# Liozou/CrystalEnergyGrids.jl

Hardware: AMD Instinct MI355X
Metric: grid-points/sec (higher is better)
Workload: dtype f64; 1 GPU; CHA_1.4_3b4eeb96 tiled 2x2x3 (11664 atoms) x 256^3 grid, Ar probe LJ + real-space Ewald; grid_points=16777216, framework_atoms=11664, lattice_images=37460, mode=fused, algo=culled, parallelism=x-slab sharding over 1 GPU(s)

## Files before the change

### crystalenergygrids.jl_amd/ceg_hip/_abi.py

```python
from __future__ import annotations

import ctypes as C
import os
import sys
from pathlib import Path

import numpy as np

RULE_DTYPE = np.dtype([('kind', '<i4'), ('_pad', '<i4'), ('p', '<f8', (3,)), ('shift', '<f8')],
                      align=True)
assert RULE_DTYPE.itemsize == 40

PKG_DIR = Path(__file__).resolve().parent.parent
REPO_DIR = PKG_DIR.parent
LIB_PATH = PKG_DIR / "csrc" / "libceg_hip.so"

class GridHeader(C.Structure):
    _fields_ = [("spacing", C.c_double), ("dims", C.c_int32 * 3), ("has_mat", C.c_int32),
                ("size", C.c_double * 3), ("shift", C.c_double * 3), ("delta", C.c_double * 3), ("unitcell", C.c_double * 3),
                ("num_unitcell", C.c_int32 * 3), ("_pad", C.c_int32), ("ewald_precision", C.c_double), ("mat", C.c_double * 9)]


class SweepParams(C.Structure):
    _fields_ = [("seed", C.c_uint64), ("first_step", C.c_uint64), ("stream_id", C.c_void_p), ("temperature", C.c_void_p),
                ("dmax", C.c_void_p), ("thetamax", C.c_void_p), ("p_rotation", C.c_void_p), ("bead", C.c_void_p)]


SWEEP_STATS_DTYPE = np.dtype([('translation_trials', '<i8'), ('translation_accepted', '<i8'), ('rotation_trials', '<i8'),
                              ('rotation_accepted', '<i8'), ('blocked', '<i8'), ('delta', '<f8')], align=True)
SWEEP_RECORD_DTYPE = np.dtype([('molecule', '<i4'), ('kind', '<i4'), ('accepted', '<i4'), ('_pad', '<i4'), ('u', '<f8'),
                               ('rows', '<f8', (2, 4)), ('positions', '<f8', (16, 3))], align=True)
assert SWEEP_STATS_DTYPE.itemsize == 48 and SWEEP_RECORD_DTYPE.itemsize == 472

GCMC_MAX_SPECIES = 8


class GcmcParams(C.Structure):
    _fields_ = [("seed", C.c_uint64), ("first_step", C.c_uint64), ("stream_id", C.c_void_p), ("temperature", C.c_void_p),
                ("dmax", C.c_void_p), ("thetamax", C.c_void_p), ("nspecies", C.c_int32), ("_pad", C.c_int32), ("species", C.c_void_p),
                ("molecule_species", C.c_void_p), ("max_molecules", C.c_void_p), ("molecule_species_out", C.c_void_p)]


GCMC_SPECIES_DTYPE = np.dtype([('m', '<i4'), ('bead', '<i4'), ('kinds', '<i4', (16,)), ('model', '<f8', (16, 3)), ('cumulative', '<f8', (5,)),
                               ('phiPV_div_k', '<f8'), ('self_reciprocal', '<f8'), ('tail_framework', '<f8'),
                               ('tail_cross', '<f8', (GCMC_MAX_SPECIES,))], align=True)
GCMC_STATS_DTYPE = np.dtype([('trials', '<i8', (7,)), ('accepted', '<i8', (7,)), ('blocked', '<i8'), ('capacity', '<i8'), ('spent', '<i8'),
                             ('delta_moves', '<f8'), ('delta_swaps', '<f8'), ('count', '<i4', (GCMC_MAX_SPECIES,)), ('nmol', '<i4'),
                             ('_pad', '<i4')], align=True)
GCMC_RECORD_DTYPE = np.dtype([('species', '<i4'), ('molecule', '<i4'), ('kind', '<i4'), ('accepted', '<i4'), ('n_species', '<i4'),
                              ('flags', '<i4'), ('u', '<f8'), ('tc', '<f8'), ('rows', '<f8', (2, 4)), ('positions', '<f8', (16, 3))], align=True)
assert (C.sizeof(GcmcParams), GCMC_SPECIES_DTYPE.itemsize, GCMC_STATS_DTYPE.itemsize, GCMC_RECORD_DTYPE.itemsize) == (88, 584, 192, 488)

c_double_p = C.POINTER(C.c_double)
c_float_p = C.POINTER(C.c_float)
c_int32_p = C.POINTER(C.c_int32)
c_int64_p = C.POINTER(C.c_int64)

PROTOTYPES = {
    "ceg_abi_version": (C.c_int, []),
    "ceg_device_count": (C.c_int, []),
    "ceg_last_error": (C.c_char_p, []),
    "ceg_grid_vdw": (C.c_int, [
        c_double_p, c_int64_p, C.c_int64, c_double_p, c_double_p,
        C.c_int32, C.c_double, C.c_double,
        C.c_void_p, c_int32_p, C.c_int32,
        c_int32_p, c_double_p, c_double_p, c_double_p,
        C.c_double, C.c_double, c_float_p, C.c_int32]),
    "ceg_grid_coulomb": (C.c_int, [
        c_double_p, c_double_p, C.c_int64, c_double_p, c_double_p,
        C.c_int32, C.c_double, C.c_double, C.c_double,
        c_int32_p, c_double_p, c_double_p, c_double_p,
        C.c_double, C.c_double, c_float_p, C.c_int32]),
    "ceg_grid_vdw_device": (C.c_int, [
        c_double_p, c_int64_p, C.c_int64, c_double_p, c_double_p,
        C.c_int32, C.c_double, C.c_double,
        C.c_void_p, c_int32_p, C.c_int32,
        c_int32_p, c_double_p, c_double_p, c_double_p,
        C.c_double, C.c_double, C.c_void_p, C.c_int32, C.c_int32]),
    "ceg_grid_coulomb_device": (C.c_int, [
        c_double_p, c_double_p, C.c_int64, c_double_p, c_double_p,
        C.c_int32, C.c_double, C.c_double, C.c_double,
        c_int32_p, c_double_p, c_double_p, c_double_p,
        C.c_double, C.c_double, C.c_void_p, C.c_int32, C.c_int32]),
    "ceg_grid_vdw_file": (C.c_int, [
        c_double_p, c_int64_p, C.c_int64, c_double_p, c_double_p,
        C.c_int32, C.c_double, C.c_double,
        C.c_void_p, c_int32_p, C.c_int32,
        c_int32_p, c_double_p, c_double_p, c_double_p,
        C.c_double, C.c_double, c_float_p, C.c_int32,
        C.c_char_p, C.c_char_p, C.c_int64, C.c_char_p, C.c_int64]),
    "ceg_grid_coulomb_file": (C.c_int, [
        c_double_p, c_double_p, C.c_int64, c_double_p, c_double_p,
        C.c_int32, C.c_double, C.c_double, C.c_double,
        c_int32_p, c_double_p, c_double_p, c_double_p,
        C.c_double, C.c_double, c_float_p, C.c_int32,
        C.c_char_p, C.c_char_p, C.c_int64, C.c_char_p, C.c_int64]),
    "ceg_release_cached_buffers": (C.c_int, []),
    "ceg_host_grid_alloc": (c_float_p, [c_int32_p]),
    "ceg_host_grid_free": (C.c_int, [c_float_p]),
    "ceg_plan_create": (C.c_int, [
        C.POINTER(C.c_void_p), C.c_int32,
        c_double_p, c_int64_p, c_double_p, C.c_int64,
        c_double_p, c_double_p, C.c_int32, C.c_double, C.c_double,
        C.c_void_p, c_int32_p, C.c_int32, C.c_double,
        c_int32_p, c_double_p, c_double_p, c_double_p]),
    "ceg_plan_destroy": (C.c_int, [C.c_void_p]),
    "ceg_image_cache_stats": (C.c_int, [c_int64_p, c_int64_p, c_int64_p]),
    "ceg_plan_can_cull": (C.c_int, [C.c_void_p]),
    "ceg_plan_num_images": (C.c_int64, [C.c_void_p]),
    "ceg_plan_copy_images": (C.c_int, [C.c_void_p, c_double_p, c_int32_p, c_int32_p, c_int32_p, c_int32_p]),
    "ceg_plan_build_vdw": (C.c_int, [
        C.c_void_p, C.c_double, C.c_double, C.c_int32, C.c_int32,
        C.c_void_p, C.c_int64, C.c_int32, C.c_int32, C.c_void_p]),
    "ceg_plan_build_coulomb": (C.c_int, [
        C.c_void_p, C.c_double, C.c_double, C.c_int32, C.c_int32,
        C.c_void_p, C.c_int64, C.c_int32, C.c_int32, C.c_void_p]),
    "ceg_plan_build_fused": (C.c_int, [
        C.c_void_p, C.c_double, C.c_double, C.c_double, C.c_double,
        C.c_int32, C.c_int32, C.c_void_p, C.c_void_p, C.c_int64, C.c_int32,
        C.c_int32, C.c_void_p]),
    "ceg_plan_create_multi": (C.c_int, [
        C.POINTER(C.c_void_p), C.c_int32,
        c_double_p, c_int64_p, c_double_p, C.c_int64,
        c_double_p, c_double_p, C.c_int32, C.c_double, C.c_double,
        C.c_int32, C.POINTER(C.c_void_p), C.POINTER(C.c_void_p), C.c_int32, C.c_double,
        c_int32_p, c_double_p, c_double_p, c_double_p]),
    "ceg_plan_num_probes": (C.c_int, [C.c_void_p]),
    "ceg_grids_multi": (C.c_int, [
        c_double_p, c_int64_p, c_double_p, C.c_int64, c_double_p, c_double_p, C.c_int32, C.c_double, C.c_double,
        C.c_int32, C.POINTER(C.c_void_p), C.POINTER(C.c_void_p), C.c_int32, C.c_double,
        c_int32_p, c_double_p, c_double_p, c_double_p,
        C.c_double, C.c_double, C.c_double, C.c_double, C.POINTER(C.c_void_p), c_float_p, C.c_int32]),
    "ceg_plan_build_multi": (C.c_int, [
        C.c_void_p, C.c_double, C.c_double, C.c_double, C.c_double,
        C.c_int32, C.c_int32, C.POINTER(C.c_void_p), C.c_void_p, C.c_int64, C.c_int32, C.c_void_p]),
    "ceg_plan_eval_points": (C.c_int, [
        C.c_void_p, C.c_int32, C.c_int32, c_double_p, C.c_int64, c_double_p]),
    "ceg_interp_create": (C.c_int, [
        C.POINTER(C.c_void_p), C.c_int32, C.c_void_p, C.c_int32,
        c_int32_p, c_double_p, c_double_p, c_double_p, c_double_p, C.c_int32]),
    "ceg_interp_create_from_file": (C.c_int, [C.POINTER(C.c_void_p), C.c_int32, C.c_char_p, C.c_int32, C.c_double, c_double_p, c_double_p, C.c_void_p]),
    "ceg_interp_set_higherorder": (C.c_int, [C.c_void_p, C.c_int32]),
    "ceg_interp_destroy": (C.c_int, [C.c_void_p]),
    "ceg_interp_points": (C.c_int, [C.c_void_p, c_double_p, C.c_int64, c_double_p]),
    "ceg_interp_points_device": (C.c_int, [C.c_void_p, C.c_void_p, C.c_int64, C.c_void_p, C.c_void_p]),
    "ceg_scale_grid_device": (C.c_int, [C.c_void_p, C.c_int64, C.c_double, C.c_int32, C.c_void_p]),
    "ceg_recip_create": (C.c_int, [
        C.POINTER(C.c_void_p), C.c_int32, c_int32_p, c_double_p, c_double_p, c_double_p, C.c_int64,
        c_int32_p, c_double_p]),
    "ceg_recip_destroy": (C.c_int, [C.c_void_p]),
    "ceg_recip_layout": (C.c_int, [c_int32_p, C.c_int64, c_int32_p, c_int32_p, c_int32_p, C.c_void_p, C.c_void_p]),
    "ceg_recip_energy": (C.c_int, [C.c_void_p, c_double_p, c_double_p, C.c_int32, C.c_int64, C.c_double, C.c_double, c_double_p]),
    "ceg_block_from_grid": (C.c_int, [C.c_int32, C.c_void_p, C.c_int32, c_int32_p, C.c_double, C.c_void_p]),
    "ceg_block_spheres": (C.c_int, [C.c_int32, c_int32_p, c_double_p, c_double_p, c_double_p, c_double_p, C.c_int32, C.c_double,
                                    c_double_p, c_double_p, C.c_int32, C.c_void_p]),
    "ceg_recip_set_structure_factor": (C.c_int, [C.c_void_p, c_double_p, c_double_p]),
    "ceg_pairs_create": (C.c_int, [C.POINTER(C.c_void_p), C.c_int32, c_double_p, c_double_p, C.c_double, C.c_void_p, c_int32_p,
                                   C.c_int32, C.c_double]),
    "ceg_pairs_destroy": (C.c_int, [C.c_void_p]),
    "ceg_pairs_set_atoms": (C.c_int, [C.c_void_p, c_double_p, c_int32_p, c_int32_p, C.c_int64]),
    "ceg_pairs_energy": (C.c_int, [C.c_void_p, c_double_p, c_int32_p, C.c_int32, C.c_int64, C.c_int32, c_double_p]),
    "ceg_pairs_energy_device": (C.c_int, [C.c_void_p, C.c_void_p, c_int32_p, C.c_int32, C.c_int64, C.c_int32, C.c_void_p, C.c_void_p]),
    "ceg_pairs_neighbour_cells": (C.c_int, [C.c_void_p, c_int32_p]),
    "ceg_mc_create": (C.c_int, [C.POINTER(C.c_void_p), C.c_int32, C.POINTER(C.c_void_p), C.c_void_p, c_double_p, C.c_int32, c_double_p,
                                c_double_p, C.c_double, C.c_void_p, c_int32_p, C.c_double, c_int32_p, c_double_p, c_double_p, c_double_p,
                                C.c_int64, c_int32_p, c_double_p]),
    "ceg_mc_destroy": (C.c_int, [C.c_void_p]),
    "ceg_mc_set_guests": (C.c_int, [C.c_void_p, c_double_p, c_int32_p, c_int32_p, C.c_int32]),
    "ceg_mc_trial": (C.c_int, [C.c_void_p, C.c_int32, c_double_p, C.c_int64, c_double_p]),
    "ceg_mc_trial_device": (C.c_int, [C.c_void_p, C.c_int32, C.c_void_p, C.c_int64, C.c_void_p, C.c_void_p]),
    "ceg_mc_trial_insert_device": (C.c_int, [C.c_void_p, c_int32_p, C.c_int32, C.c_void_p, C.c_int64, C.c_void_p, C.c_void_p]),
    "ceg_mc_accept": (C.c_int, [C.c_void_p, C.c_int32, c_double_p]),
    "ceg_mc_get_state": (C.c_int, [C.c_void_p, c_double_p, c_double_p, c_double_p]),
    "ceg_mc_neighbour_cells": (C.c_int, [C.c_void_p, c_int32_p, c_int32_p]),
    "ceg_mc_trial_insert": (C.c_int, [C.c_void_p, c_int32_p, C.c_int32, c_double_p, C.c_int64, c_double_p]),
    "ceg_mc_insert": (C.c_int, [C.c_void_p, c_int32_p, C.c_int32, c_double_p, c_int32_p]),
    "ceg_mc_remove": (C.c_int, [C.c_void_p, C.c_int32, c_int32_p]),
    "ceg_mc_group_create": (C.c_int, [C.POINTER(C.c_void_p), C.POINTER(C.c_void_p), C.c_int32]),
    "ceg_mc_group_destroy": (C.c_int, [C.c_void_p]),
    "ceg_mc_group_trial": (C.c_int, [C.c_void_p, c_int32_p, c_int32_p, c_int32_p, C.c_int32, c_double_p, c_double_p]),
    "ceg_mc_group_accept": (C.c_int, [C.c_void_p, c_int32_p, c_double_p]),
    "ceg_mc_group_sweep": (C.c_int, [C.c_void_p, C.c_void_p, C.c_int64, C.c_void_p, C.c_void_p]),
    "ceg_mc_group_sweep_gcmc": (C.c_int, [C.c_void_p, C.c_void_p, C.c_int64, C.c_void_p, C.c_void_p]),
    "ceg_energy_grid": (C.c_int, [C.POINTER(C.c_void_p), C.c_void_p, C.c_void_p, c_double_p, c_double_p, C.c_int32,
                                  c_double_p, C.c_int32, c_double_p, c_int32_p,
                                  C.c_void_p, c_int32_p, c_double_p, c_double_p, c_double_p, c_double_p,
                                  C.c_double, C.c_double, C.c_void_p, C.c_int32, C.c_void_p]),
    "ceg_energy_grid_reduced": (C.c_int, [C.POINTER(C.c_void_p), C.c_void_p, C.c_void_p, c_double_p, c_double_p, C.c_int32,
                                          c_double_p, C.c_int32, c_double_p, c_int32_p,
                                          C.c_void_p, c_int32_p, c_double_p, c_double_p, c_double_p, c_double_p,
                                          C.c_double, C.c_double, c_double_p, C.c_int32, c_double_p,
                                          C.c_void_p, C.c_void_p, C.c_void_p, C.c_int32, C.c_void_p]),
    "ceg_recip_energy_device": (C.c_int, [C.c_void_p, C.c_void_p, c_double_p, C.c_int32, C.c_int64, C.c_double, C.c_double,
                                          C.c_void_p, C.c_void_p]),
}

ALGO_AUTO, ALGO_BRUTEFORCE, ALGO_CULLED = 0, 1, 2
EGRID_MAX_TEMPS = 8


class CegError(RuntimeError):

    def __init__(self, code: int, msg: str):
        super().__init__(f"libceg_hip error {code}: {msg}")
        self.code = code


_lib = None


def load_library(path: os.PathLike | None = None) -> C.CDLL:
    global _lib
    if _lib is not None and path is None:
        return _lib
    p = Path(path) if path is not None else Path(os.environ.get("CEG_HIP_LIB", LIB_PATH))
    if not p.exists():
        raise ImportError(
            f"{p} is missing: build it with `python -c 'import __graft_entry__ as g; g.build()'` "
            "(hipcc --offload-arch=gfx950).  There is no CPU fallback for the grid build.")
    if "torch" not in sys.modules and not os.environ.get("CEG_HIP_NO_TORCH"):
        try:
            import torch
        except ImportError:
            pass
    lib = C.CDLL(str(p))
    for name, (restype, argtypes) in PROTOTYPES.items():
        fn = getattr(lib, name)
        fn.restype = restype
        fn.argtypes = argtypes
    if lib.ceg_abi_version() != 1:
        raise ImportError("libceg_hip.so ABI version mismatch")
    if path is None:
        _lib = lib
    return lib


def check(lib: C.CDLL, code: int) -> None:
    if code != 0:
        raise CegError(code, (lib.ceg_last_error() or b"").decode())


def dptr(a: np.ndarray):
    assert a.dtype == np.float64 and a.flags.c_contiguous
    return a.ctypes.data_as(c_double_p)


def i32ptr(a: np.ndarray):
    assert a.dtype == np.int32 and a.flags.c_contiguous
    return a.ctypes.data_as(c_int32_p)


def i64ptr(a: np.ndarray):
    assert a.dtype == np.int64 and a.flags.c_contiguous
    return a.ctypes.data_as(c_int64_p)


def fptr(a: np.ndarray):
    assert a.dtype == np.float32
    return a.ctypes.data_as(c_float_p)
```

### crystalenergygrids.jl_amd/ceg_hip/plan.py

```python
from __future__ import annotations

import ctypes as C
from typing import Optional

import numpy as np

from . import _abi
from .hostmirror.coordinates import GridCoordinatesSetup
from .grids import _grid_args, _matT, coulomb_scaling, vdw_scaling
from .hostmirror.probes import ProbeSystem


class _PlainBuilds:

    def build_vdw(self, d_out: int, channel_stride: int, i_begin: int, i_end: int, i_origin: int = 0,
                  algo: int = _abi.ALGO_AUTO, stream: int = 0) -> None:
        lam, thr = vdw_scaling()
        _abi.check(self._lib, self._lib.ceg_plan_build_vdw(self._h, lam, thr, i_begin, i_end, d_out, channel_stride,
                                                           i_origin, algo, stream))

    def build_coulomb(self, d_out: int, channel_stride: int, i_begin: int, i_end: int, i_origin: int = 0,
                      algo: int = _abi.ALGO_AUTO, stream: int = 0) -> None:
        lam, thr = coulomb_scaling()
        _abi.check(self._lib, self._lib.ceg_plan_build_coulomb(self._h, lam, thr, i_begin, i_end, d_out,
                                                               channel_stride, i_origin, algo, stream))

    def build_fused(self, d_vdw: int, d_coulomb: int, channel_stride: int, i_begin: int, i_end: int,
                    i_origin: int = 0, algo: int = _abi.ALGO_AUTO, stream: int = 0) -> None:
        lv, tv = vdw_scaling()
        lc, tc = coulomb_scaling()
        _abi.check(self._lib, self._lib.ceg_plan_build_fused(self._h, lv, tv, lc, tc, i_begin, i_end, d_vdw,
                                                             d_coulomb, channel_stride, i_origin, algo, stream))

    def eval_points(self, which: str, points, algo: int = _abi.ALGO_AUTO) -> np.ndarray:
        pts = np.ascontiguousarray(points, dtype=np.float64).reshape(-1, 3)
        out = np.empty((len(pts), 8), dtype=np.float64)
        w = {"vdw": 0, "coulomb": 1}[which]
        _abi.check(self._lib, self._lib.ceg_plan_eval_points(self._h, w, algo, _abi.dptr(pts), len(pts), _abi.dptr(out)))
        return out


class GridPlan(_PlainBuilds):
    def __init__(self, cset: GridCoordinatesSetup, vdw: Optional[ProbeSystem] = None,
                 coulomb: Optional[ProbeSystem] = None, alpha: float = 0.0, device: int = 0):
        if vdw is None and coulomb is None:
            raise ValueError("GridPlan needs a VdW probe and/or a Coulomb probe")
        ref = vdw if vdw is not None else coulomb
        if vdw is not None and coulomb is not None:
            if vdw.positions.shape != coulomb.positions.shape or not np.array_equal(vdw.positions, coulomb.positions):
                raise ValueError("VdW and Coulomb probes must share the same framework")
        self._lib = _abi.load_library()
        self.cset = cset
        self.device = device
        self.has_vdw = vdw is not None
        self.has_coulomb = coulomb is not None
        pos = np.ascontiguousarray(ref.positions, dtype=np.float64)
        mat, invmat = _matT(ref.mat), _matT(ref.invmat)
        ortho, safemin2 = ref.periodic_setup()
        dims, size, shift, delta = _grid_args(cset)
        kinds_p = rules_p = offs_p = None
        nkinds = 0
        keep = [pos, mat, invmat, dims, size, shift, delta]
        if vdw is not None:
            ff = vdw.forcefield
            ff.check_vdw_grid(vdw.probe, np.unique(vdw.atomkinds))
            rules, offsets = ff.rule_table(vdw.probe)
            kinds = np.ascontiguousarray(vdw.atomkinds, dtype=np.int64)
            kinds_p, rules_p, offs_p, nkinds = _abi.i64ptr(kinds), rules.ctypes.data, _abi.i32ptr(offsets), ff.nkinds
            keep += [rules, offsets, kinds]
        q_p = None
        if coulomb is not None:
            q = np.ascontiguousarray(coulomb.charges, dtype=np.float64)
            q_p = _abi.dptr(q)
            keep.append(q)
        handle = C.c_void_p()
        rc = self._lib.ceg_plan_create(C.byref(handle), device, _abi.dptr(pos), kinds_p, q_p, len(pos),
                                       _abi.dptr(mat), _abi.dptr(invmat), int(ortho), safemin2, ref.cutoff2,
                                       rules_p, offs_p, nkinds, float(alpha),
                                       _abi.i32ptr(dims), _abi.dptr(size), _abi.dptr(shift), _abi.dptr(delta))
        _abi.check(self._lib, rc)
        self._h = handle
        self.npoints = cset.npoints
        self.plane = self.npoints[1] * self.npoints[2]

    @property
    def can_cull(self) -> bool:
        return bool(self._lib.ceg_plan_can_cull(self._h))

    @property
    def num_images(self) -> int:
        return int(self._lib.ceg_plan_num_images(self._h))

    def close(self) -> None:
        if getattr(self, "_h", None):
            self._lib.ceg_plan_destroy(self._h)
            self._h = None

    def __del__(self):
        try:
            self.close()
        except Exception:
            pass


class MultiGridPlan(_PlainBuilds):
    MAX_PROBES = 4

    def __init__(self, cset: GridCoordinatesSetup, probes, coulomb: Optional[ProbeSystem] = None, alpha: float = 0.0,
                 device: int = 0):
        probes = list(probes)
        if not 1 <= len(probes) <= self.MAX_PROBES:
            raise ValueError(f"1..{self.MAX_PROBES} probes per multi-probe plan")
        ref = probes[0]
        for other in probes[1:] + ([coulomb] if coulomb is not None else []):
            if other.positions.shape != ref.positions.shape or not np.array_equal(other.positions, ref.positions):
                raise ValueError("all probes of a multi-probe plan must share the same framework")
        for other in probes[1:]:
            if not np.array_equal(other.atomkinds, ref.atomkinds) or other.cutoff2 != ref.cutoff2:
                raise ValueError("all probes of a multi-probe plan must share atom kinds and cutoff")
        self._lib = _abi.load_library()
        self.cset, self.device = cset, device
        self.nprobes = len(probes)
        self.has_coulomb = coulomb is not None
        pos = np.ascontiguousarray(ref.positions, dtype=np.float64)
        mat, invmat = _matT(ref.mat), _matT(ref.invmat)
        ortho, safemin2 = ref.periodic_setup()
        dims, size, shift, delta = _grid_args(cset)
        kinds = np.ascontiguousarray(ref.atomkinds, dtype=np.int64)
        tables = []
        for pr in probes:
            pr.forcefield.check_vdw_grid(pr.probe, np.unique(pr.atomkinds))
            tables.append(pr.forcefield.rule_table(pr.probe))
        rules_pp = (C.c_void_p * self.nprobes)(*[t[0].ctypes.data for t in tables])
        offs_pp = (C.c_void_p * self.nprobes)(*[t[1].ctypes.data for t in tables])
        q = np.ascontiguousarray(coulomb.charges, dtype=np.float64) if coulomb is not None else None
        handle = C.c_void_p()
        rc = self._lib.ceg_plan_create_multi(C.byref(handle), device, _abi.dptr(pos), _abi.i64ptr(kinds), _abi.dptr(q) if q is not None else None,
                                             len(pos), _abi.dptr(mat), _abi.dptr(invmat), int(ortho), safemin2, ref.cutoff2,
                                             self.nprobes, rules_pp, offs_pp, ref.forcefield.nkinds, float(alpha),
                                             _abi.i32ptr(dims), _abi.dptr(size), _abi.dptr(shift), _abi.dptr(delta))
        _abi.check(self._lib, rc)
        self._h = handle
        self.npoints = cset.npoints
        self.plane = self.npoints[1] * self.npoints[2]

    @property
    def num_images(self) -> int:
        return int(self._lib.ceg_plan_num_images(self._h))

    def close(self) -> None:
        if getattr(self, "_h", None):
            self._lib.ceg_plan_destroy(self._h)
            self._h = None

    def __del__(self):
        try:
            self.close()
        except Exception:
            pass

    def build(self, d_vdw, d_coulomb: int, channel_stride: int, i_begin: int, i_end: int, i_origin: int = 0, stream: int = 0) -> None:
        d_vdw = list(d_vdw) + [0] * (self.nprobes - len(d_vdw))
        ptrs = (C.c_void_p * self.nprobes)(*[int(x) if x else None for x in d_vdw])
        lv, tv = vdw_scaling()
        lc, tc = coulomb_scaling()
        _abi.check(self._lib, self._lib.ceg_plan_build_multi(self._h, lv, tv, lc, tc, i_begin, i_end, ptrs, int(d_coulomb) if d_coulomb else None,
                                                             channel_stride, i_origin, stream))
```

### crystalenergygrids.jl_amd/csrc/ceg_api.hip

```cpp
#include "ceg_internal.h"
#include "ceg_host.h"

#include <algorithm>
#include <atomic>
#include <chrono>
#include <cmath>
#include <cstdarg>
#include <cstdio>
#include <cstring>
#include <limits>
#include <map>
#include <memory>
#include <mutex>
#include <unordered_map>
#include <string>
#include <vector>

using namespace ceg;
using ceg_host::check_common;
using ceg_host::DeviceGuard;
using ceg_host::fail;

static thread_local std::string g_err = "";

int ceg_host::fail(int code, const char* fmt, ...)
{
    char buf[512];
    va_list ap;
    va_start(ap, fmt);
    vsnprintf(buf, sizeof buf, fmt, ap);
    va_end(ap);
    g_err = buf;
    return code;
}

extern "C" void ceg_set_last_error_(const char* msg) { g_err = msg ? msg : ""; }

extern "C" int ceg_abi_version(void) { return CEG_ABI_VERSION; }

extern "C" const char* ceg_last_error(void) { return g_err.c_str(); }

extern "C" int ceg_device_count(void)
{
    int n = 0;
    if (hipGetDeviceCount(&n) != hipSuccess) {
        (void)hipGetLastError();
        return 0;
    }
    return n;
}

struct ceg_plan {
    int device = 0;
    Geom g{};
    int64_t natoms = 0;
    bool has_rules = false, has_charge = false;
    bool can_cull = false;
    std::vector<double> h_pos, h_charge;
    std::vector<int32_t> h_kind;
    std::vector<DevRule> h_rules;
    std::vector<int32_t> h_offset;
    std::vector<int32_t> h_offset_union;
    int32_t nkinds = 0;
    double4* d_atoms = nullptr;
    int32_t* d_kind = nullptr;
    DevRule* d_rules = nullptr;
    int32_t* d_offset = nullptr;
    double4* d_images = nullptr;
    int32_t* d_imgkind = nullptr;
    int32_t* d_imgatom = nullptr;
    int32_t* d_binstart = nullptr;
    std::shared_ptr<void> images;
    ImageBins ib{};
    bool images_built = false;
    bool images_from_cache = false;
    PlanConst* d_pc = nullptr;
    double* d_erfcx = nullptr;
    double* d_exp2 = nullptr;
    int vdwk = 0;
    bool single_buck = false;
    double bk[4] = {0, 0, 0, 0};
    double* d_bk2 = nullptr;
    double r_exact2 = CEG_R_EXACT2;
    std::vector<FastVdw> h_fast;
    FastVdw* d_fast = nullptr;
    bool fast_ewald = false;
    bool ew2 = false;
    double* d_ew2 = nullptr;
    struct ProbeTab {
        std::vector<DevRule> rules;
        std::vector<int32_t> offset;
        std::vector<FastVdw> fast;
        DevRule* d_rules = nullptr;
        int32_t* d_offset = nullptr;
        FastVdw* d_fast = nullptr;
        PlanConst* d_pc = nullptr;
        int vdwk = 0;
        bool single_buck = false;
        double bk[4] = {0, 0, 0, 0};
        double* d_bk2 = nullptr;
        int32_t* d_imgkind = nullptr;
    };
    int nprobes = 0;
    std::vector<ProbeTab> probes;
};

namespace {

inline void matvec(const double* m, const double v[3], double o[3])
{
    for (int i = 0; i < 3; ++i) o[i] = m[i] * v[0] + m[i + 3] * v[1] + m[i + 6] * v[2];
}

void perpendicular_widths(const double* m, double w[3])
{
    const double* a = m;
    const double* b = m + 3;
    const double* c = m + 6;
    auto cross = [](const double* u, const double* v, double* o) {
        o[0] = u[1] * v[2] - u[2] * v[1];
        o[1] = u[2] * v[0] - u[0] * v[2];
        o[2] = u[0] * v[1] - u[1] * v[0];
    };
    auto norm = [](const double* u) { return std::sqrt(u[0] * u[0] + u[1] * u[1] + u[2] * u[2]); };
    double axb[3], bxc[3], cxa[3];
    cross(a, b, axb);
    cross(b, c, bxc);
    cross(c, a, cxa);
    const double vol = std::fabs(a[0] * bxc[0] + a[1] * bxc[1] + a[2] * bxc[2]);
    w[0] = vol / norm(bxc);
    w[1] = vol / norm(cxa);
    w[2] = vol / norm(axb);
}

int convert_rules(ceg_plan* p, const ceg_rule_t* rules, const int32_t* rule_offset, int32_t nkinds)
{
    std::vector<char> present(nkinds, 0);
    for (int64_t a = 0; a < p->natoms; ++a) present[p->h_kind[a]] = 1;
    p->h_offset.assign(nkinds + 1, 0);
    p->h_rules.clear();
    for (int32_t k = 0; k < nkinds; ++k) {
        p->h_offset[k] = (int32_t)p->h_rules.size();
        for (int32_t t = rule_offset[k]; t < rule_offset[k + 1]; ++t) {
            const ceg_rule_t& r = rules[t];
            DevRule d{};
            d.kind = r.kind;
            d.shift = r.shift;
            switch (r.kind) {
            case CEG_NOINTERACTION:
            case CEG_COULOMB_EWALD_DIRECT:
                continue;
            case CEG_LENNARDJONES:
                d.p0 = r.p[0];
                d.p1 = r.p[1] * r.p[1];
                break;
            case CEG_BUCKINGHAM:
                d.p0 = r.p[0];
                d.p1 = r.p[1];
                d.p2 = r.p[2];
                break;
            case CEG_HARDSPHERE: {
                const double rr = r.p[0] + r.p[1];
                d.p0 = rr * rr;
                break;
            }
            default:
                if (present[k])
                    return fail(CEG_ERR_RULE,
                                "interaction kind %d (force-field index %d) is not valid in a VdW grid "
                                "(src/interactions.jl:442-467)", r.kind, k + 1);
                continue;
            }
            p->h_rules.push_back(d);
        }
    }
    p->h_offset[nkinds] = (int32_t)p->h_rules.size();
    p->nkinds = nkinds;
    p->h_fast.assign(nkinds, FastVdw{});
    bool all_lj = true, all_fast = true;
    double hs_max2 = 0.0;
    for (int32_t k = 0; k < nkinds; ++k) {
        const int32_t b = p->h_offset[k], e = p->h_offset[k + 1];
        FastVdw f{};
        int nlj = 0, nbuck = 0, nhs = 0, nother = 0;
        for (int32_t t = b; t < e; ++t) {
            const DevRule& r = p->h_rules[t];
            if (r.kind == CEG_LENNARDJONES) { ++nlj; f.p0 = 4.0 * r.p0; f.p1 = r.p1; f.p2 = r.p1 * r.p1 * r.p1; f.shift += r.shift; }
            else if (r.kind == CEG_BUCKINGHAM) { ++nbuck; f.p0 = r.p0; f.p1 = r.p1; f.p2 = r.p2; f.shift += r.shift; }
            else if (r.kind == CEG_HARDSPHERE) { ++nhs; f.shift += r.shift; if (present[k]) hs_max2 = std::max(hs_max2, r.p0); }
            else ++nother;
        }
        if (e == b) f.cls = 0;
        else if (nlj == 1 && nbuck == 0 && nhs == 0 && nother == 0) f.cls = 1;
        else if (nbuck == 1 && nlj == 0 && nother == 0) f.cls = 2;
        else f.cls = 3;
        p->h_fast[k] = f;
        if (!present[k]) continue;
        if (f.cls > 1) all_lj = false;
        if (f.cls > 2) all_fast = false;
    }
    p->vdwk = all_lj ? 1 : (all_fast ? 2 : 0);
    if (p->vdwk == 2) {
        bool first = true, same = true;
        for (int32_t k = 0; k < nkinds && same; ++k) {
            const FastVdw& f = p->h_fast[k];
            if (!present[k] || f.cls == 0) continue;
            if (f.cls != 2) { same = false; break; }
            if (first) { p->bk[0] = f.p0; p->bk[1] = f.p1; p->bk[2] = f.p2; p->bk[3] = f.shift; first = false; }
            else same = f.p0 == p->bk[0] && f.p1 == p->bk[1] && f.p2 == p->bk[2] && f.shift == p->bk[3];
        }
        p->single_buck = same && !first && p->bk[1] > 0.0 && p->bk[2] != 0.0 && std::isfinite(1.0 / p->bk[2]);
    }
    p->r_exact2 = std::max(CEG_R_EXACT2, hs_max2 * (1.0 + 1e-9) + 1e-9);
    if (p->r_exact2 >= p->g.cutoff2) p->vdwk = 0, p->r_exact2 = CEG_R_EXACT2;
    return CEG_OK;
}

struct BlockCache {
    std::mutex m;
    std::map<std::pair<int, size_t>, std::vector<void*>> idle;
    std::unordered_map<void*, std::pair<int, size_t>> owner;
    size_t idle_bytes = 0;
};
BlockCache g_blocks;
constexpr size_t BLOCK_CACHE_LIMIT = 256ull << 20;

hipError_t cached_malloc(void** out, size_t bytes)
{
    int dev = 0;
    if (hipError_t e = hipGetDevice(&dev); e != hipSuccess) return e;
    size_t cls = 512;
    while (cls < bytes) cls <<= 1;
    std::lock_guard<std::mutex> lock(g_blocks.m);
    auto& list = g_blocks.idle[{dev, cls}];
    if (!list.empty()) {
        *out = list.back();
        list.pop_back();
        g_blocks.idle_bytes -= cls;
        return hipSuccess;
    }
    if (hipError_t e = hipMalloc(out, cls); e != hipSuccess) return e;
    g_blocks.owner[*out] = {dev, cls};
    return hipSuccess;
}

void cached_free(void* ptr)
{
    if (!ptr) return;
    std::lock_guard<std::mutex> lock(g_blocks.m);
    auto it = g_blocks.owner.find(ptr);
    if (it == g_blocks.owner.end()) { (void)hipFree(ptr); return; }
    const size_t cls = it->second.second;
    if (g_blocks.idle_bytes + cls > BLOCK_CACHE_LIMIT) {
        g_blocks.owner.erase(it);
        (void)hipFree(ptr);
        return;
    }
    g_blocks.idle[it->second].push_back(ptr);
    g_blocks.idle_bytes += cls;
}

void block_cache_release()
{
    std::lock_guard<std::mutex> lock(g_blocks.m);
    int prev = -1;
    (void)hipGetDevice(&prev);
    for (auto& kv : g_blocks.idle) {
        if (hipSetDevice(kv.first.first) != hipSuccess) continue;
        for (void* ptr : kv.second) {
            g_blocks.owner.erase(ptr);
            (void)hipFree(ptr);
        }
        kv.second.clear();
    }
    g_blocks.idle_bytes = 0;
    if (prev >= 0) (void)hipSetDevice(prev);
}

}

namespace ceg_host {
hipError_t pool_malloc(void** out, size_t bytes) { return cached_malloc(out, bytes); }
void pool_free(void* ptr) { cached_free(ptr); }
}

namespace ceg {
struct ImgBox {
    double mat[9], invmat[9];
    double lo[3], hi[3], bin[3];
    int32_t nb[3];
    int32_t has_rules, has_charge, vdw_only;
    int32_t nkinds;
    uint64_t hasbits[16];
};
hipError_t build_images_device(const ImgBox& B, const double4* d_atoms, const int32_t* d_kind, const int32_t* d_has, int64_t natoms,
                               double4** out_xyzq, int32_t** out_kind, int32_t** out_atom, int32_t** out_binstart, int64_t* out_n);
}

namespace {

struct UploadStaging {
    char* h = nullptr;
    size_t cap = 0, used = 0;
    bool pending = false;
};
constexpr size_t UPLOAD_STAGING_BYTES = 4u << 20, UPLOAD_STAGED_MAX = 1u << 20;
struct StagingPool {
    std::mutex m;
    std::vector<char*> idle;
};
StagingPool g_staging_pool;
thread_local UploadStaging* g_staging = nullptr;

struct StagingLease {
    UploadStaging st;
    UploadStaging* outer;
    StagingLease() : outer(g_staging)
    {
        if (!std::getenv("CEG_HIP_SYNC_UPLOADS")) {
            {
                std::lock_guard<std::mutex> lock(g_staging_pool.m);
                if (!g_staging_pool.idle.empty()) { st.h = g_staging_pool.idle.back(); g_staging_pool.idle.pop_back(); }
            }
            if (!st.h && hipHostMalloc((void**)&st.h, UPLOAD_STAGING_BYTES, hipHostMallocPortable) != hipSuccess) { st.h = nullptr; (void)hipGetLastError(); }
            if (st.h) st.cap = UPLOAD_STAGING_BYTES;
        }
        g_staging = &st;
    }
    ~StagingLease()
    {
        if (st.pending) (void)hipStreamSynchronize(nullptr);
        g_staging = outer;
        if (st.h) {
            std::lock_guard<std::mutex> lock(g_staging_pool.m);
            if (g_staging_pool.idle.size() < 8) g_staging_pool.idle.push_back(st.h);
            else (void)hipHostFree(st.h);
        }
    }
};

inline hipError_t flush_uploads()
{
    UploadStaging* st = g_staging;
    if (!st || !st->pending) return hipSuccess;
    st->pending = false;
    st->used = 0;
    return hipStreamSynchronize(nullptr);
}

template <class T>
int upload(T** dst, const T* src, size_t n)
{
    *dst = nullptr;
    if (n == 0) n = 1;
    HIP_TRY(cached_malloc((void**)dst, n * sizeof(T)));
    if (!src) return CEG_OK;
    const size_t bytes = n * sizeof(T);
    UploadStaging* st = g_staging;
    if (st && st->h && bytes <= UPLOAD_STAGED_MAX) {
        if (st->used + bytes > st->cap) HIP_TRY(flush_uploads());
        memcpy(st->h + st->used, src, bytes);
        HIP_TRY(hipMemcpyAsync(*dst, st->h + st->used, bytes, hipMemcpyHostToDevice, nullptr));
        st->used += (bytes + 255) & ~(size_t)255;
        st->pending = true;
        return CEG_OK;
    }
    HIP_TRY(hipMemcpy(*dst, src, bytes, hipMemcpyHostToDevice));
    return CEG_OK;
}

struct ImageSet {
    int device = 0;
    uint64_t key[2] = {0, 0};
    int64_t natoms = 0;
    double cutoff2 = 0.0;
    double lo[3] = {0, 0, 0}, hi[3] = {0, 0, 0};
    double4* d_images = nullptr;
    int32_t* d_imgkind = nullptr;
    int32_t* d_imgatom = nullptr;
    int32_t* d_binstart = nullptr;
    ImageBins ib{};
    size_t bytes = 0;
    ~ImageSet()
    {
        DeviceGuard guard(device);
        (void)hipDeviceSynchronize();
        for (void* ptr : {(void*)d_images, (void*)d_imgkind, (void*)d_imgatom, (void*)d_binstart}) cached_free(ptr);
    }
};
std::mutex g_image_mutex;
std::vector<std::shared_ptr<ImageSet>>& g_image_cache = *new std::vector<std::shared_ptr<ImageSet>>();
std::atomic<long> g_image_hits{0}, g_image_misses{0};

struct Hash128 {
    uint64_t a = 0x243F6A8885A308D3ull, b = 0x13198A2E03707344ull;
    void word(uint64_t w)
    {
        a = (a ^ w) * 0x9E3779B97F4A7C15ull; a ^= a >> 29;
        b = (b + w) * 0xC2B2AE3D27D4EB4Full; b ^= b >> 31; b += a;
    }
    void bytes(const void* ptr, size_t n)
    {
        const unsigned char* c = static_cast<const unsigned char*>(ptr);
        size_t i = 0;
        for (; i + 8 <= n; i += 8) { uint64_t w; memcpy(&w, c + i, 8); word(w); }
        uint64_t w = 0;
        if (i < n) memcpy(&w, c + i, n - i);
        word(w ^ ((uint64_t)n << 56));
    }
    template <class T> void pod(const T& v) { bytes(&v, sizeof v); }
};

int image_cache_capacity()
{
    if (const char* e = std::getenv("CEG_HIP_IMAGE_CACHE")) return std::max(0, atoi(e));
    return 6;
}

void image_cache_release()
{
    std::lock_guard<std::mutex> lock(g_image_mutex);
    g_image_cache.clear();
}

#ifndef CEG_BIN_Z
#define CEG_BIN_Z 1.5
#endif
int build_images(ceg_plan* p)
{
    const Geom& g = p->g;
    const double cutoff = std::sqrt(g.cutoff2);
    const double margin = cutoff * (1.0 + 1e-6) + 1e-6;
    double lo[3], hi[3];
    for (int a = 0; a < 3; ++a) {
        lo[a] = g.shift[a] - margin;
        hi[a] = g.shift[a] + g.size[a] + margin;
    }
    double target[3] = {4.5, 4.5, CEG_BIN_Z};
    if (const char* e = std::getenv("CEG_HIP_BIN_XY")) target[0] = target[1] = std::max(0.5, atof(e));
    if (const char* e = std::getenv("CEG_HIP_BIN_Z")) target[2] = std::max(0.25, atof(e));
    int nb[3];
    double bin[3];
    for (int a = 0; a < 3; ++a) {
        nb[a] = std::max(1, (int)std::floor((hi[a] - lo[a]) / target[a]));
        bin[a] = (hi[a] - lo[a]) / nb[a];
    }
    const std::vector<int32_t>& off = p->nprobes > 0 ? p->h_offset_union : p->h_offset;
    auto kind_has_rule = [&](int32_t k) { return k >= 0 && k + 1 < (int32_t)off.size() && off[k + 1] > off[k]; };
    Hash128 hk;
    std::shared_ptr<ImageSet> hit;
    const int cap = image_cache_capacity();
    if (cap > 0) {
        hk.pod(p->device); hk.pod(p->natoms);
        hk.bytes(g.mat, sizeof g.mat); hk.bytes(g.invmat, sizeof g.invmat);
        hk.bytes(lo, sizeof lo); hk.bytes(hi, sizeof hi); hk.bytes(target, sizeof target);
        hk.bytes(p->h_pos.data(), p->h_pos.size() * sizeof(double));
        const int32_t mode = (p->has_rules ? 1 : 0) | (p->has_charge ? 2 : 0);
        hk.pod(mode);
        if (p->has_charge) hk.bytes(p->h_charge.data(), p->h_charge.size() * sizeof(double));
        if (p->has_rules)
            for (int64_t a = 0; a < p->natoms; ++a) {
                const int32_t k = p->h_kind[a];
                hk.pod((int32_t)(k < 0 ? -1 : (k | (kind_has_rule(k) ? (1 << 25) : 0))));
            }
        std::lock_guard<std::mutex> lock(g_image_mutex);
        for (size_t t = 0; t < g_image_cache.size(); ++t) {
            const std::shared_ptr<ImageSet> c = g_image_cache[t];
            if (c->device == p->device && c->key[0] == hk.a && c->key[1] == hk.b && c->natoms == p->natoms && c->cutoff2 == g.cutoff2 &&
                memcmp(c->lo, lo, sizeof lo) == 0 && memcmp(c->hi, hi, sizeof hi) == 0) {
                hit = c;
                std::rotate(g_image_cache.begin() + t, g_image_cache.begin() + t + 1, g_image_cache.end());
                break;
            }
        }
    }
    if (hit) {
        g_image_hits.fetch_add(1);
        p->images = hit;
        const ImageSet& c = *hit;
        p->d_images = c.d_images; p->d_imgkind = c.d_imgkind; p->d_imgatom = c.d_imgatom; p->d_binstart = c.d_binstart;
        p->ib = c.ib;
        p->ib.kind = p->has_rules ? p->d_imgkind : nullptr;
        p->ib.atoms = p->d_atoms;
        p->images_built = true;
        p->images_from_cache = true;
        return CEG_OK;
    }
    if (cap > 0) g_image_misses.fetch_add(1);
    if (!std::getenv("CEG_HIP_IMAGES_ON_HOST")) {
        ceg::ImgBox B{};
        memcpy(B.mat, g.mat, sizeof B.mat);
        memcpy(B.invmat, g.invmat, sizeof B.invmat);
        for (int a = 0; a < 3; ++a) { B.lo[a] = lo[a]; B.hi[a] = hi[a]; B.bin[a] = bin[a]; B.nb[a] = nb[a]; }
        B.has_rules = p->has_rules ? 1 : 0;
        B.has_charge = p->has_charge ? 1 : 0;
        B.vdw_only = (p->has_rules && !p->has_charge) ? 1 : 0;
        B.nkinds = p->nkinds;
        int32_t* d_has = nullptr;
        if (p->has_rules && p->nkinds <= 1024) {
            for (int32_t k = 0; k < p->nkinds; ++k)
                if (kind_has_rule(k)) B.hasbits[k >> 6] |= 1ull << (k & 63);
        } else if (p->has_rules) {
            std::vector<int32_t> has((size_t)std::max(p->nkinds, 1), 0);
            for (int32_t k = 0; k < p->nkinds; ++k) has[k] = kind_has_rule(k) ? 1 : 0;
            if (int rc = upload(&d_has, has.data(), has.size())) return rc;
        }
        auto set = std::make_shared<ImageSet>();
        set->device = p->device;
        set->key[0] = hk.a; set->key[1] = hk.b;
        set->natoms = p->natoms; set->cutoff2 = g.cutoff2;
        memcpy(set->lo, lo, sizeof lo); memcpy(set->hi, hi, sizeof hi);
        int64_t n = 0;
        const hipError_t e = ceg::build_images_device(B, p->d_atoms, p->has_rules ? p->d_kind : nullptr, d_has, p->natoms, &set->d_images, &set->d_imgkind,
                                                      &set->d_imgatom, &set->d_binstart, &n);
        if (d_has) cached_free(d_has);
        if (e != hipSuccess) return fail(CEG_ERR_HIP, "building the lattice-image list on the device failed: %s", hipGetErrorString(e));
        set->bytes = (size_t)n * (sizeof(double4) + 2 * sizeof(int32_t)) + (size_t)(nb[0] * nb[1] * nb[2] + 1) * sizeof(int32_t);
        p->images = set;
        p->d_images = set->d_images; p->d_imgkind = set->d_imgkind; p->d_imgatom = set->d_imgatom; p->d_binstart = set->d_binstart;
        ImageBins& ib = p->ib;
        ib.xyzq = p->d_images;
        ib.kind = p->has_rules ? p->d_imgkind : nullptr;
        ib.atom = p->d_imgatom;
        ib.atoms = p->d_atoms;
        ib.bin_start = p->d_binstart;
        for (int a = 0; a < 3; ++a) {
            ib.lo[a] = lo[a];
            ib.bin[a] = bin[a];
            ib.inv_bin[a] = 1.0 / bin[a];
            ib.nb[a] = nb[a];
        }
        ib.nimages = (int32_t)n;
        p->images_built = true;
        set->ib = ib;
        if (cap > 0) {
            std::lock_guard<std::mutex> lock(g_image_mutex);
            g_image_cache.push_back(set);
            while ((int)g_image_cache.size() > cap) g_image_cache.erase(g_image_cache.begin());
        }
        return CEG_OK;
    }
    struct Img { double x, y, z, q; int32_t kind; int32_t bin; int32_t atom; };
    std::vector<Img> imgs;
    imgs.reserve((size_t)p->natoms * 8);
    const double* M = g.mat;
    const double* I = g.invmat;
    for (int64_t a = 0; a < p->natoms; ++a) {
        if (p->has_rules && !p->has_charge) {
            if (!kind_has_rule(p->h_kind[a])) continue;
        }
        const double pa[3] = {p->h_pos[3 * a], p->h_pos[3 * a + 1], p->h_pos[3 * a + 2]};
        double fmin[3] = {1e300, 1e300, 1e300}, fmax[3] = {-1e300, -1e300, -1e300};
        for (int c = 0; c < 8; ++c) {
            const double d[3] = {((c & 1) ? hi[0] : lo[0]) - pa[0], ((c & 2) ? hi[1] : lo[1]) - pa[1],
                                 ((c & 4) ? hi[2] : lo[2]) - pa[2]};
            double f[3];
            matvec(I, d, f);
            for (int q = 0; q < 3; ++q) {
                fmin[q] = std::min(fmin[q], f[q]);
                fmax[q] = std::max(fmax[q], f[q]);
            }
        }
        int n0[3], n1[3];
        for (int q = 0; q < 3; ++q) {
            n0[q] = (int)std::ceil(fmin[q] - 1e-9);
            n1[q] = (int)std::floor(fmax[q] + 1e-9);
        }
        for (int nx = n0[0]; nx <= n1[0]; ++nx)
            for (int ny = n0[1]; ny <= n1[1]; ++ny)
                for (int nz = n0[2]; nz <= n1[2]; ++nz) {
                    const double P[3] = {pa[0] + (nx * M[0] + ny * M[3] + nz * M[6]),
                                         pa[1] + (nx * M[1] + ny * M[4] + nz * M[7]),
                                         pa[2] + (nx * M[2] + ny * M[5] + nz * M[8])};
                    if (P[0] < lo[0] || P[0] > hi[0] || P[1] < lo[1] || P[1] > hi[1] || P[2] < lo[2] ||
                        P[2] > hi[2])
                        continue;
                    int b[3];
                    for (int q = 0; q < 3; ++q) {
                        b[q] = (int)std::floor((P[q] - lo[q]) / bin[q]);
                        b[q] = std::min(std::max(b[q], 0), nb[q] - 1);
                    }
                    Img im;
                    im.x = P[0]; im.y = P[1]; im.z = P[2];
                    im.q = p->has_charge ? p->h_charge[a] : 0.0;
                    im.kind = -1;
                    if (p->has_rules) {
                        const int32_t k = p->h_kind[a];
                        im.kind = k < 0 ? -1 : (k | (kind_has_rule(k) ? (1 << 25) : 0));
                    }
                    im.bin = (b[0] * nb[1] + b[1]) * nb[2] + b[2];
                    im.atom = (int32_t)a;
                    imgs.push_back(im);
                }
    }
    if (imgs.size() > 0x7ffffff0ull) return fail(CEG_ERR_UNSUPPORTED, "too many lattice images");
    const size_t nbins = (size_t)nb[0] * nb[1] * nb[2];
    std::vector<int32_t> start(nbins + 1, 0);
    for (const Img& im : imgs) start[im.bin + 1]++;
    for (size_t b = 0; b < nbins; ++b) start[b + 1] += start[b];
    std::vector<int32_t> cursor(start.begin(), start.end() - 1);
    std::vector<double4> xyzq(imgs.size());
    std::vector<int32_t> kind(imgs.size());
    std::vector<int32_t> atom(imgs.size());
    for (const Img& im : imgs) {
        const int32_t s = cursor[im.bin]++;
        xyzq[s] = make_double4(im.x, im.y, im.z, im.q);
        kind[s] = im.kind;
        atom[s] = im.atom;
    }
    auto set = std::make_shared<ImageSet>();
    set->device = p->device;
    set->key[0] = hk.a; set->key[1] = hk.b;
    set->natoms = p->natoms; set->cutoff2 = g.cutoff2;
    memcpy(set->lo, lo, sizeof lo); memcpy(set->hi, hi, sizeof hi);
    if (int rc = upload(&set->d_images, xyzq.data(), xyzq.size())) return rc;
    if (int rc = upload(&set->d_imgkind, kind.data(), kind.size())) return rc;
    if (int rc = upload(&set->d_imgatom, atom.data(), atom.size())) return rc;
    if (int rc = upload(&set->d_binstart, start.data(), start.size())) return rc;
    set->bytes = xyzq.size() * sizeof(double4) + (kind.size() + atom.size() + start.size()) * sizeof(int32_t);
    p->images = set;
    p->d_images = set->d_images; p->d_imgkind = set->d_imgkind; p->d_imgatom = set->d_imgatom; p->d_binstart = set->d_binstart;
    ImageBins& ib = p->ib;
    ib.xyzq = p->d_images;
    ib.kind = p->has_rules ? p->d_imgkind : nullptr;
    ib.atom = p->d_imgatom;
    ib.atoms = p->d_atoms;
    ib.bin_start = p->d_binstart;
    for (int a = 0; a < 3; ++a) {
        ib.lo[a] = lo[a];
        ib.bin[a] = bin[a];
        ib.inv_bin[a] = 1.0 / bin[a];
        ib.nb[a] = nb[a];
    }
    ib.nimages = (int32_t)imgs.size();
    p->images_built = true;
    set->ib = ib;
    if (cap > 0) {
        std::lock_guard<std::mutex> lock(g_image_mutex);
        g_image_cache.push_back(set);
        while ((int)g_image_cache.size() > cap) g_image_cache.erase(g_image_cache.begin());
    }
    return CEG_OK;
}

bool build_ewald_tables_uncached(double alpha, double cutoff2, std::vector<double>& tab, std::vector<double>& exp2_tab,
                                 double* inv_h_out, double* mx0_inv_h_out);

bool build_ewald_tables(double alpha, double cutoff2, std::vector<double>& tab, std::vector<double>& exp2_tab,
                        double* inv_h_out, double* mx0_inv_h_out)
{
    struct Memo { bool valid = false, ok = false; double alpha = 0, cutoff2 = 0, inv_h = 0, mx0 = 0; std::vector<double> tab, e2; };
    static std::mutex m;
    static Memo memo;
    std::lock_guard<std::mutex> lock(m);
    if (!(memo.valid && memo.alpha == alpha && memo.cutoff2 == cutoff2)) {
        memo.tab.clear(); memo.e2.clear();
        memo.ok = build_ewald_tables_uncached(alpha, cutoff2, memo.tab, memo.e2, &memo.inv_h, &memo.mx0);
        memo.alpha = alpha; memo.cutoff2 = cutoff2; memo.valid = true;
    }
    tab = memo.tab; exp2_tab = memo.e2; *inv_h_out = memo.inv_h; *mx0_inv_h_out = memo.mx0;
    return memo.ok;
}

bool build_ewald_tables_uncached(double alpha, double cutoff2, std::vector<double>& tab, std::vector<double>& exp2_tab,
                                 double* inv_h_out, double* mx0_inv_h_out)
{
    const int N = CEG_ERFCX_TAB_N;
    const long double x0 = (long double)alpha * std::sqrt((long double)CEG_R_EXACT2) * (1.0L - 1e-6L);
    const long double x1 = (long double)alpha * std::sqrt((long double)cutoff2 * (1.0L + 2e-9L)) * (1.0L + 1e-6L);
    if (!(x1 > x0) || x1 > 5.0L * (1.0L - 1e-9L)) return false;
    const long double h = (x1 - x0) / N;
    auto erfcx = [](long double x) { return expl(x * x) * erfcl(x); };
    tab.assign((size_t)N * 6, 0.0);
    const long double PI = 3.14159265358979323846264338327950288L;
    long double node[6];
    for (int k = 0; k < 6; ++k) node[k] = 0.5L + 0.5L * cosl(PI * (k + 0.5L) / 6.0L);
    double worst = 0.0;
    for (int i = 0; i < N; ++i) {
        const long double lo = x0 + i * h;
        long double V[6][7];
        for (int r = 0; r < 6; ++r) {
            long double pw = 1.0L;
            for (int c = 0; c < 6; ++c) { V[r][c] = pw; pw *= node[r]; }
            V[r][6] = erfcx(lo + node[r] * h);
        }
        for (int c = 0; c < 6; ++c) {
            int piv = c;
            for (int r = c + 1; r < 6; ++r) if (fabsl(V[r][c]) > fabsl(V[piv][c])) piv = r;
            for (int q = 0; q < 7; ++q) std::swap(V[c][q], V[piv][q]);
            const long double d = V[c][c];
            for (int q = 0; q < 7; ++q) V[c][q] /= d;
            for (int r = 0; r < 6; ++r) if (r != c) {
                const long double f = V[r][c];
                for (int q = 0; q < 7; ++q) V[r][q] -= f * V[c][q];
            }
        }
        for (int c = 0; c < 6; ++c) tab[(size_t)i * 6 + c] = (double)V[c][6];
        for (int t = 0; t <= 8; ++t) {
            const double sl = t / 8.0;
            double pv = tab[(size_t)i * 6 + 5];
            for (int c = 4; c >= 0; --c) pv = pv * sl + tab[(size_t)i * 6 + c];
            const long double ref = erfcx(lo + (long double)sl * h);
            worst = std::max(worst, (double)fabsl(((long double)pv - ref) / ref));
        }
    }
    if (!(worst < 1e-14)) return false;
    exp2_tab.resize(64);
    for (int j = 0; j < 64; ++j) exp2_tab[j] = (double)exp2l((long double)j / 64.0L);
    *inv_h_out = (double)(1.0L / h);
    *mx0_inv_h_out = (double)(-x0 / h);
    return true;
}

bool build_ew2_table_uncached(double alpha, double r_exact2, double cutoff2, std::vector<double>& tab, int32_t* base_out,
                              int32_t* ni_out, double* worst_out, int which = 0, double bkA = 0.0, double bkC = 0.0)
{
    const int SHIFT = which == 0 ? CEG_EW2_SHIFT : CEG_BK2_SHIFT, ni_max = which == 0 ? CEG_EW2_NI_MAX : CEG_BK2_NI_MAX;
    auto key_of = [SHIFT](double s) { uint64_t b; memcpy(&b, &s, 8); return (int32_t)((uint32_t)(b >> 32) >> SHIFT); };
    if (!(alpha > 0.0) || !(r_exact2 >= 1.0) || !(cutoff2 > r_exact2)) return false;
    const int32_t base = key_of(r_exact2), last = key_of(cutoff2 * (1.0 + 4e-9) + 4e-9);
    const int32_t ni = last - base + 1;
    if (ni < 1 || ni > ni_max) return false;
    const long double a = alpha, ka = 2.0L * a / sqrtl(3.14159265358979323846264338327950288L);
    auto B0 = [&](long double s) { const long double r = sqrtl(s); return which == 0 ? erfcl(a * r) / r : (long double)bkA * expl(-a * r); };
    auto Cf = [&](long double s) { return ka * expl(-a * a * s); };
    const int nf = which == 0 ? 2 : 1, stride = which == 0 ? CEG_EW2_STRIDE : CEG_BK2_STRIDE;
    const int ND = which == 0 ? 7 : CEG_BK2_ND;
    const long double PI = 3.14159265358979323846264338327950288L;
    long double node[8];
    for (int k = 0; k < ND; ++k) node[k] = cosl(PI * (k + 0.5L) / (long double)ND);
    tab.assign((size_t)ni * stride, 0.0);
    double worst = 0.0;
    for (int32_t i = 0; i < ni; ++i) {
        const uint64_t lo_bits = (uint64_t)(uint32_t)((base + i) << SHIFT) << 32;
        const uint64_t mid_bits = lo_bits | ((uint64_t)1 << (32 + SHIFT - 1));
        const uint64_t hi_bits = (uint64_t)(uint32_t)((base + i + 1) << SHIFT) << 32;
        double s_lo, s_mid, s_hi;
        memcpy(&s_lo, &lo_bits, 8); memcpy(&s_mid, &mid_bits, 8); memcpy(&s_hi, &hi_bits, 8);
        const long double hh = 0.5L * ((long double)s_hi - (long double)s_lo);
        for (int f = 0; f < nf; ++f) {
            long double V[8][9];
            for (int r = 0; r < ND; ++r) {
                long double pw = 1.0L;
                for (int c = 0; c < ND; ++c) { V[r][c] = pw; pw *= node[r]; }
                const long double s = (long double)s_mid + node[r] * hh;
                V[r][ND] = f == 0 ? B0(s) : Cf(s);
            }
            for (int c = 0; c < ND; ++c) {
                int piv = c;
                for (int r = c + 1; r < ND; ++r) if (fabsl(V[r][c]) > fabsl(V[piv][c])) piv = r;
                for (int q = 0; q <= ND; ++q) std::swap(V[c][q], V[piv][q]);
                const long double d = V[c][c];
                for (int q = 0; q <= ND; ++q) V[c][q] /= d;
                for (int r = 0; r < ND; ++r) if (r != c) {
                    const long double g = V[r][c];
                    for (int q = 0; q <= ND; ++q) V[r][q] -= g * V[c][q];
                }
            }
            long double cu[8], ct[8] = {0, 0, 0, 0, 0, 0, 0, 0};
            long double sc = 1.0L;
            for (int c = 0; c < ND; ++c) { cu[c] = V[c][ND] * sc; sc /= hh; }
            for (int c = 0; c < ND; ++c) {
                long double binom = 1.0L;
                for (int k = 0; k <= c; ++k) {
                    ct[k] += cu[c] * binom * powl(-hh, c - k);
                    binom = binom * (c - k) / (k + 1);
                }
            }
            double* co = &tab[(size_t)i * stride + ND * f];
            for (int c = 0; c < ND; ++c) co[c] = (double)ct[c];
            for (int q = 0; q <= 16; ++q) {
                const double t = (double)(((long double)q / 16.0L) * 2.0L * hh * (1.0L - 1e-12L));
                double pv = co[ND - 1];
                for (int c = ND - 2; c >= 0; --c) pv = __builtin_fma(pv, t, co[c]);
                const long double s = (long double)s_lo + (long double)t;
                const long double ref = f == 0 ? B0(s) : Cf(s);
                const long double scale = which == 0 ? fabsl(ref) : fabsl(ref) + fabsl((long double)bkC) / (s * s * s);
                worst = std::max(worst, (double)fabsl(((long double)pv - ref) / scale));
            }
        }
    }
    *base_out = base; *ni_out = ni; *worst_out = worst;
    return worst < 5e-11;
}

bool build_ew2_table(double alpha, double r_exact2, double cutoff2, std::vector<double>& tab, int32_t* base_out, int32_t* ni_out)
{
    struct Memo { bool valid = false, ok = false; double alpha = 0, r_exact2 = 0, cutoff2 = 0; int32_t base = 0, ni = 0; std::vector<double> tab; };
    static std::mutex m;
    static Memo memo;
    std::lock_guard<std::mutex> lock(m);
    if (!(memo.valid && memo.alpha == alpha && memo.r_exact2 == r_exact2 && memo.cutoff2 == cutoff2)) {
        memo.tab.clear();
        double worst = 0.0;
        memo.ok = build_ew2_table_uncached(alpha, r_exact2, cutoff2, memo.tab, &memo.base, &memo.ni, &worst);
        memo.alpha = alpha; memo.r_exact2 = r_exact2; memo.cutoff2 = cutoff2; memo.valid = true;
        if (std::getenv("CEG_HIP_TRACE"))
            fprintf(stderr, "[ceg_hip] r^2-indexed Ewald table: %d intervals, worst relative error %.2e -> %s\n", memo.ni, worst,
                    memo.ok ? "used" : "not used");
    }
    tab = memo.tab; *base_out = memo.base; *ni_out = memo.ni;
    return memo.ok;
}

bool build_bk2_table(double A, double B, double C, double r_exact2, double cutoff2, std::vector<double>& tab, int32_t* base_out, int32_t* ni_out)
{
    struct Memo { bool valid = false, ok = false; double A = 0, B = 0, C = 0, r_exact2 = 0, cutoff2 = 0; int32_t base = 0, ni = 0; std::vector<double> tab; };
    static std::mutex m;
    static Memo memo;
    std::lock_guard<std::mutex> lock(m);
    if (!(memo.valid && memo.A == A && memo.B == B && memo.C == C && memo.r_exact2 == r_exact2 && memo.cutoff2 == cutoff2)) {
        memo.tab.clear();
        double worst = 0.0;
        memo.ok = build_ew2_table_uncached(B, r_exact2, cutoff2, memo.tab, &memo.base, &memo.ni, &worst, 1, A, C) && worst < CEG_BK2_TOL;
        memo.A = A; memo.B = B; memo.C = C; memo.r_exact2 = r_exact2; memo.cutoff2 = cutoff2; memo.valid = true;
        if (std::getenv("CEG_HIP_TRACE"))
            fprintf(stderr, "[ceg_hip] r^2-indexed Buckingham table: %d intervals, worst error %.2e of the pair energy -> %s\n", memo.ni, worst,
                    memo.ok ? "used" : "not used");
    }
    tab = memo.tab; *base_out = memo.base; *ni_out = memo.ni;
    return memo.ok;
}

}

int ceg_host::check_common(const double* pos, int64_t natoms, const double* mat, const double* invmat,
                           const int32_t* dims, const double* size, const double* shift, const double* delta)
{
    if (!pos && natoms > 0) return fail(CEG_ERR_INVALID, "pos is NULL");
    if (natoms < 0) return fail(CEG_ERR_INVALID, "natoms < 0");
    if (!mat || !invmat || !dims || !size || !shift || !delta)
        return fail(CEG_ERR_INVALID, "NULL geometry argument");
    for (int a = 0; a < 3; ++a)
        if (dims[a] < 1) return fail(CEG_ERR_INVALID, "dims[%d] = %d < 1", a, dims[a]);
    return CEG_OK;
}

__global__ void k_probe_image_flags(const int32_t* __restrict__ kind_union, const int32_t* __restrict__ has, int32_t nkinds, int32_t* __restrict__ out, int64_t n)
{
    const int64_t i = (int64_t)blockIdx.x * blockDim.x + threadIdx.x;
    if (i >= n) return;
    const int32_t kw = kind_union[i];
    if (kw < 0) { out[i] = kw; return; }
    const int32_t k = kw & ((1 << 24) - 1);
    out[i] = k | ((k < nkinds && has[k]) ? (1 << 25) : 0);
}

static int probe_image_flags(const int32_t* d_union, const int32_t* d_has, int32_t nkinds, int32_t* d_out, int64_t n)
{
    if (n <= 0) return CEG_OK;
    hipLaunchKernelGGL(k_probe_image_flags, dim3((unsigned)((n + 255) / 256)), dim3(256), 0, nullptr, d_union, d_has, nkinds, d_out, n);
    return hipGetLastError() == hipSuccess ? CEG_OK : fail(CEG_ERR_HIP, "image-flag kernel launch failed");
}

static int create_impl(ceg_plan_t** plan, int32_t device,
                       const double* pos, const int64_t* atomkind, const double* charge,
                       int64_t natoms,
                       const double mat[9], const double invmat[9],
                       int32_t ortho, double safemin2, double cutoff2,
                       const ceg_rule_t* rules, const int32_t* rule_offset, int32_t nkinds,
                       int32_t nprobes, const ceg_rule_t* const* mrules, const int32_t* const* moffset,
                       double alpha,
                       const int32_t dims[3], const double size[3], const double shift[3],
                       const double delta[3])
{
    if (!plan) return fail(CEG_ERR_INVALID, "plan is NULL");
    *plan = nullptr;
    if (int rc = check_common(pos, natoms, mat, invmat, dims, size, shift, delta)) return rc;
    if (nprobes < 0 || nprobes > CEG_MAX_PROBES) return fail(CEG_ERR_INVALID, "nprobes = %d outside 1..%d", nprobes, CEG_MAX_PROBES);
    if (nprobes > 0) {
        if (!mrules || !moffset || !atomkind || nkinds <= 0) return fail(CEG_ERR_INVALID, "rule tables / atomkind missing");
        for (int q = 0; q < nprobes; ++q)
            if (!mrules[q] || !moffset[q]) return fail(CEG_ERR_INVALID, "rule table of probe %d is NULL", q);
        rules = mrules[0];
        rule_offset = moffset[0];
    }
    const bool trace = std::getenv("CEG_HIP_TRACE") != nullptr;
    const auto t0 = std::chrono::steady_clock::now();
    auto stamp = [&](const char* what) {
        if (trace)
            fprintf(stderr, "[ceg plan] %-28s %8.3f ms\n", what,
                    std::chrono::duration<double, std::milli>(std::chrono::steady_clock::now() - t0).count());
    };
    const int ndev = ceg_device_count();
    if (ndev <= 0) return fail(CEG_ERR_NO_DEVICE, "no HIP device available (this library has no CPU path)");
    if (device < 0 || device >= ndev) return fail(CEG_ERR_NO_DEVICE, "device %d not present (%d devices)", device, ndev);
    const bool has_rules = rules && rule_offset && atomkind && nkinds > 0;
    if (!has_rules && !charge) return fail(CEG_ERR_INVALID, "plan needs rules+atomkind and/or charges");

    ceg_plan* p = new ceg_plan();
    p->device = device;
    p->natoms = natoms;
    p->has_rules = has_rules;
    p->has_charge = charge != nullptr;
    Geom& g = p->g;
    memcpy(g.mat, mat, sizeof g.mat);
    memcpy(g.invmat, invmat, sizeof g.invmat);
    for (int a = 0; a < 3; ++a) {
        g.size[a] = size[a];
        g.shift[a] = shift[a];
        g.delta[a] = delta[a];
        g.dims[a] = dims[a];
    }
    g.ortho = ortho ? 1 : 0;
    g.safemin2 = safemin2;
    g.cutoff2 = cutoff2;
    g.alpha = alpha;
    g.diag = (mat[1] == 0 && mat[2] == 0 && mat[3] == 0 && mat[5] == 0 && mat[6] == 0 && mat[7] == 0) ? 1 : 0;

    p->h_pos.assign(pos, pos + 3 * natoms);
    if (charge) p->h_charge.assign(charge, charge + natoms);
    p->h_kind.assign(natoms, -1);
    if (has_rules) {
        for (int64_t a = 0; a < natoms; ++a) {
            const int64_t k = atomkind[a];
            if (k < 1 || k > nkinds) {
                delete p;
                return fail(CEG_ERR_INVALID, "atomkind[%lld] = %lld outside 1..%d", (long long)a, (long long)k, nkinds);
            }
            p->h_kind[a] = (int32_t)(k - 1);
        }
        if (int rc = convert_rules(p, rules, rule_offset, nkinds)) {
            delete p;
            return rc;
        }
        if (nprobes > 0) {
            p->nprobes = nprobes;
            p->probes.resize(nprobes);
            std::vector<int32_t> any(nkinds, 0);
            double r_exact2 = CEG_R_EXACT2;
            for (int q = 0; q < nprobes; ++q) {
                if (q > 0)
                    if (int rc = convert_rules(p, mrules[q], moffset[q], nkinds)) { delete p; return rc; }
                ceg_plan::ProbeTab& t = p->probes[q];
                t.rules = p->h_rules; t.offset = p->h_offset; t.fast = p->h_fast;
                t.vdwk = p->vdwk; t.single_buck = p->single_buck;
                for (int c = 0; c < 4; ++c) t.bk[c] = p->bk[c];
                r_exact2 = std::max(r_exact2, p->r_exact2);
                for (int32_t k = 0; k < nkinds; ++k) any[k] |= (t.offset[k + 1] > t.offset[k]) ? 1 : 0;
            }
            p->r_exact2 = r_exact2;
            if (!(r_exact2 < p->g.cutoff2)) {
                delete p;
                return fail(CEG_ERR_UNSUPPORTED, "a hard sphere of one of the probes reaches the cutoff: build that grid with a plan of its own");
            }
            p->h_rules = p->probes[0].rules; p->h_fast = p->probes[0].fast;
            p->vdwk = p->probes[0].vdwk; p->single_buck = p->probes[0].single_buck;
            for (int c = 0; c < 4; ++c) p->bk[c] = p->probes[0].bk[c];
            p->h_offset_union.assign(nkinds + 1, 0);
            for (int32_t k = 0; k < nkinds; ++k) p->h_offset_union[k + 1] = p->h_offset_union[k] + any[k];
            p->h_offset = p->probes[0].offset;
        }
    }
    double w[3];
    perpendicular_widths(g.mat, w);
    const double cutoff = std::sqrt(cutoff2);
    p->can_cull = std::isfinite(cutoff2) && cutoff2 > 0 &&
                  std::min(w[0], std::min(w[1], w[2])) >= 2.0 * cutoff * (1.0 - 1e-12);

    stamp("host: rules, geometry");
    DeviceGuard guard(device);
    if (!guard.ok) {
        delete p;
        return fail(CEG_ERR_HIP, "hipSetDevice(%d) failed", device);
    }
    StagingLease lease;
    std::vector<double4> xyzq((size_t)natoms);
    for (int64_t a = 0; a < natoms; ++a)
        xyzq[a] = make_double4(pos[3 * a], pos[3 * a + 1], pos[3 * a + 2], charge ? charge[a] : 0.0);
    int rc = upload(&p->d_atoms, xyzq.data(), xyzq.size());
    if (!rc) rc = upload(&p->d_kind, p->h_kind.data(), p->h_kind.size());
    if (!rc) rc = upload(&p->d_rules, p->h_rules.data(), p->h_rules.size());
    if (!rc) {
        if (p->h_offset.empty()) p->h_offset.assign(1, 0);
        rc = upload(&p->d_offset, p->h_offset.data(), p->h_offset.size());
    }
    stamp("atom / rule tables uploaded");
    if (!rc && p->can_cull) rc = build_images(p);
    stamp(p->images_from_cache ? "images: cache hit" : "images built + uploaded");
    if (!rc && p->can_cull) {
        PlanConst hc{};
        hc.g = p->g;
        hc.ib = p->ib;
        hc.rt = RuleTable{p->d_rules, p->d_offset, p->nkinds};
        hc.alpha2 = alpha * alpha;
        hc.r_exact2 = p->r_exact2;
        {
            const double hx = 1.5 * size[0] / dims[0], hy = 1.5 * size[1] / dims[1], hz = 1.5 * size[2] / dims[2];
            const double reach = std::sqrt(cutoff2 * (1.0 + 1e-9) + 1e-9) + std::sqrt(hx * hx + hy * hy + hz * hz);
            bool all = true;
            for (int k = 0; k < 3; ++k) {
                const double rown = std::sqrt(invmat[k] * invmat[k] + invmat[k + 3] * invmat[k + 3] + invmat[k + 6] * invmat[k + 6]);
                const double ek = std::fabs(invmat[k]) * hx + std::fabs(invmat[k + 3]) * hy + std::fabs(invmat[k + 6]) * hz + 1e-9;
                if (!(rown * reach + ek < 0.5 - 1e-6)) all = false;
            }
            hc.all_simple = all ? 1 : 0;
        }
        if (p->h_fast.empty()) p->h_fast.assign(1, FastVdw{});
        rc = upload(&p->d_fast, p->h_fast.data(), p->h_fast.size());
        hc.fastvdw = p->d_fast;
        p->fast_ewald = false;
        bool any_vdwk2 = p->vdwk == 2;
        for (const auto& t : p->probes) any_vdwk2 = any_vdwk2 || t.vdwk == 2;
        if (!rc && ((p->has_charge && std::isfinite(alpha) && alpha > 0) || any_vdwk2)) {
            std::vector<double> tab, e2;
            double inv_h = 0, mx0 = 0;
            const bool want_ewald = p->has_charge && std::isfinite(alpha) && alpha > 0;
            const bool ok = build_ewald_tables(want_ewald ? alpha : 0.25, cutoff2, tab, e2, &inv_h, &mx0);
            if (!ok && p->vdwk == 2) p->vdwk = 0;
            if (!ok)
                for (auto& t : p->probes)
                    if (t.vdwk == 2) t.vdwk = 0;
            if (ok) {
                rc = upload(&p->d_erfcx, tab.data(), tab.size());
                if (!rc) rc = upload(&p->d_exp2, e2.data(), e2.size());
                hc.erfcx_tab = p->d_erfcx;
                hc.exp2_tab = p->d_exp2;
                hc.erfcx_inv_h = inv_h;
                hc.erfcx_mx0_inv_h = mx0;
                p->fast_ewald = want_ewald;
            }
            hc.ew_k3 = 2.0 * alpha * alpha / 3.0;
            hc.ew_k15 = 4.0 * (alpha * alpha) * (alpha * alpha) / 15.0;
            if (ok && want_ewald && !rc && !std::getenv("CEG_HIP_NO_EW2")) {
                std::vector<double> t2;
                int32_t base = 0, ni = 0;
                if (build_ew2_table(alpha, p->r_exact2, cutoff2, t2, &base, &ni)) {
                    rc = upload(&p->d_ew2, t2.data(), t2.size());
                    hc.ew2_tab = p->d_ew2;
                    hc.ew2_ni = ni;
                    hc.ew2_base = base;
                    p->ew2 = !rc;
                }
            }
        }
        auto setup_bk2 = [&](int& vdwk, bool single_buck, const double bk[4], double** d_tab, PlanConst& target) {
            if (rc || vdwk != 2 || !single_buck || std::getenv("CEG_HIP_NO_BK2")) return;
            std::vector<double> tb;
            int32_t base = 0, ni = 0;
            if (!build_bk2_table(bk[0] / bk[2], bk[1], 1.0, p->r_exact2, cutoff2, tb, &base, &ni)) return;
            rc = upload(d_tab, tb.data(), tb.size());
            target.bk2_tab = *d_tab;
            target.bk2_ni = ni;
            target.bk2_base = base;
            const double B = bk[1], C = bk[2];
            target.bk_B = B; target.bk_C = C; target.bk_invC = 1.0 / C; target.bk_nshift = -bk[3] / C;
            target.bk_c1 = -B / 6.0; target.bk_c2 = -B / 48.0; target.bk_c3 = B * B / 3.0; target.bk_c4 = -B / 160.0;
            target.bk_s1 = 1.0 / (6.0 * C); target.bk_s2 = -1.0 / (48.0 * C); target.bk_s3 = 1.0 / (480.0 * C);
            if (!rc) vdwk = 3;
        };
        if (p->nprobes == 0) setup_bk2(p->vdwk, p->single_buck, p->bk, &p->d_bk2, hc);
        if (!rc && p->nprobes > 0) {
            hc.nprobes = p->nprobes;
            for (int q = 0; q < p->nprobes && !rc; ++q) {
                ceg_plan::ProbeTab& t = p->probes[q];
                rc = upload(&t.d_rules, t.rules.data(), t.rules.size());
                if (!rc) rc = upload(&t.d_offset, t.offset.data(), t.offset.size());
                if (!rc) rc = upload(&t.d_fast, t.fast.data(), t.fast.size());
                hc.rtm[q] = RuleTable{t.d_rules, t.d_offset, p->nkinds};
                hc.fastm[q] = t.d_fast;
            }
            for (int q = 0; q < p->nprobes && !rc; ++q) {
                ceg_plan::ProbeTab& t = p->probes[q];
                PlanConst hq = hc;
                hq.rt = hc.rtm[q];
                hq.fastvdw = hc.fastm[q];
                setup_bk2(t.vdwk, t.single_buck, t.bk, &t.d_bk2, hq);
                if (!rc && p->nprobes > 1) {
                    std::vector<int32_t> has((size_t)p->nkinds);
                    for (int32_t k = 0; k < p->nkinds; ++k) has[k] = t.offset[k + 1] > t.offset[k] ? 1 : 0;
                    int32_t* d_has = nullptr;
                    rc = upload(&d_has, has.data(), has.size());
                    if (!rc) {
                        void* raw = nullptr;
                        const int64_t n = p->ib.nimages;
                        if (cached_malloc(&raw, sizeof(int32_t) * (size_t)std::max<int64_t>(n, 1)) != hipSuccess) rc = fail(CEG_ERR_HIP, "hipMalloc failed");
                        else {
                            t.d_imgkind = (int32_t*)raw;
                            rc = probe_image_flags(p->d_imgkind, d_has, p->nkinds, t.d_imgkind, n);
                        }
                    }
                    if (d_has) { (void)hipDeviceSynchronize(); cached_free(d_has); }
                    hq.ib.kind = t.d_imgkind;
                }
                if (!rc) rc = upload(&t.d_pc, &hq, 1);
                if (q == 0) { p->vdwk = t.vdwk; }
            }
            hc.rt = hc.rtm[0];
            hc.fastvdw = hc.fastm[0];
        }
        if (!rc) rc = upload(&p->d_pc, &hc, 1);
    } else if (!rc && p->nprobes > 0) {
        rc = fail(CEG_ERR_UNSUPPORTED, "multi-probe plans need every perpendicular cell width >= 2*cutoff (what a ProbeSystem guarantees)");
    }
    if (flush_uploads() != hipSuccess && !rc) rc = fail(CEG_ERR_HIP, "uploading the plan's tables failed");
    stamp("function tables, constants");
    if (rc) {
        ceg_plan_destroy(p);
        return rc;
    }
    *plan = p;
    return CEG_OK;
}

extern "C" int ceg_plan_create(ceg_plan_t** plan, int32_t device,
                               const double* pos, const int64_t* atomkind, const double* charge,
                               int64_t natoms,
                               const double mat[9], const double invmat[9],
                               int32_t ortho, double safemin2, double cutoff2,
                               const ceg_rule_t* rules, const int32_t* rule_offset, int32_t nkinds,
                               double alpha,
                               const int32_t dims[3], const double size[3], const double shift[3],
                               const double delta[3])
{
    return create_impl(plan, device, pos, atomkind, charge, natoms, mat, invmat, ortho, safemin2, cutoff2, rules, rule_offset, nkinds, 0,
                       nullptr, nullptr, alpha, dims, size, shift, delta);
}

extern "C" int ceg_plan_create_multi(ceg_plan_t** plan, int32_t device, const double* pos, const int64_t* atomkind, const double* charge,
                                     int64_t natoms, const double mat[9], const double invmat[9], int32_t ortho, double safemin2,
                                     double cutoff2, int32_t nprobes, const ceg_rule_t* const* rules,
                                     const int32_t* const* rule_offset, int32_t nkinds, double alpha, const int32_t dims[3],
                                     const double size[3], const double shift[3], const double delta[3])
{
    if (nprobes < 1) return fail(CEG_ERR_INVALID, "nprobes = %d < 1", nprobes);
    return create_impl(plan, device, pos, atomkind, charge, natoms, mat, invmat, ortho, safemin2, cutoff2, nullptr, nullptr, nkinds, nprobes,
                       rules, rule_offset, alpha, dims, size, shift, delta);
}

extern "C" int ceg_plan_num_probes(const ceg_plan_t* p) { return p ? p->nprobes : 0; }

extern "C" int ceg_plan_destroy(ceg_plan_t* p)
{
    if (!p) return CEG_OK;
    DeviceGuard guard(p->device);
    (void)hipDeviceSynchronize();
    p->images.reset();
    for (void* ptr : {(void*)p->d_atoms, (void*)p->d_kind, (void*)p->d_rules, (void*)p->d_offset, (void*)p->d_pc, (void*)p->d_erfcx,
                      (void*)p->d_exp2, (void*)p->d_fast, (void*)p->d_ew2, (void*)p->d_bk2})
        cached_free(ptr);
    for (auto& t : p->probes)
        for (void* ptr : {(void*)t.d_rules, (void*)t.d_offset, (void*)t.d_fast, (void*)t.d_pc, (void*)t.d_bk2, (void*)t.d_imgkind}) cached_free(ptr);
    delete p;
    return CEG_OK;
}

extern "C" int ceg_image_cache_stats(int64_t* hits, int64_t* misses, int64_t* entries)
{
    std::lock_guard<std::mutex> lock(g_image_mutex);
    if (hits) *hits = g_image_hits.load();
    if (misses) *misses = g_image_misses.load();
    if (entries) *entries = (int64_t)g_image_cache.size();
    return CEG_OK;
}

extern "C" int ceg_plan_can_cull(const ceg_plan_t* p) { return (p && p->can_cull) ? 1 : 0; }

extern "C" int64_t ceg_plan_num_images(const ceg_plan_t* p) { return (p && p->images_built) ? p->ib.nimages : 0; }

extern "C" int ceg_plan_copy_images(const ceg_plan_t* p, double* xyzq, int32_t* kind, int32_t* atom, int32_t* bin_start, int32_t nb[3])
{
    if (!p || !p->images_built) return fail(CEG_ERR_INVALID, "the plan has no image list");
    DeviceGuard guard(p->device);
    if (!guard.ok) return fail(CEG_ERR_HIP, "hipSetDevice(%d) failed", p->device);
    const size_t n = (size_t)p->ib.nimages;
    const size_t nbins = (size_t)p->ib.nb[0] * p->ib.nb[1] * p->ib.nb[2];
    if (nb) for (int a = 0; a < 3; ++a) nb[a] = p->ib.nb[a];
    bool ok = hipDeviceSynchronize() == hipSuccess;
    if (ok && xyzq && n) ok = hipMemcpy(xyzq, p->d_images, n * sizeof(double4), hipMemcpyDeviceToHost) == hipSuccess;
    if (ok && kind && n && p->d_imgkind) ok = hipMemcpy(kind, p->d_imgkind, n * sizeof(int32_t), hipMemcpyDeviceToHost) == hipSuccess;
    if (ok && atom && n) ok = hipMemcpy(atom, p->d_imgatom, n * sizeof(int32_t), hipMemcpyDeviceToHost) == hipSuccess;
    if (ok && bin_start) ok = hipMemcpy(bin_start, p->d_binstart, (nbins + 1) * sizeof(int32_t), hipMemcpyDeviceToHost) == hipSuccess;
    return ok ? CEG_OK : fail(CEG_ERR_HIP, "copying the image list failed");
}

namespace {

int resolve_algo(const ceg_plan* p, int32_t algo, bool* culled)
{
    switch (algo) {
    case CEG_ALGO_AUTO: *culled = p->can_cull; return CEG_OK;
    case CEG_ALGO_BRUTEFORCE: *culled = false; return CEG_OK;
    case CEG_ALGO_CULLED:
        if (!p->can_cull)
            return fail(CEG_ERR_UNSUPPORTED,
                        "culled algorithm needs every perpendicular cell width >= 2*cutoff");
        *culled = true;
        return CEG_OK;
    default: return fail(CEG_ERR_INVALID, "unknown algo %d", algo);
    }
}

int run(ceg_plan* p, int mode, const Output& out, const Points& pts, bool culled, hipStream_t stream)
{
    if (mode != MODE_COULOMB && !p->has_rules) return fail(CEG_ERR_INVALID, "plan was created without rules");
    if (mode != MODE_VDW && !p->has_charge) return fail(CEG_ERR_INVALID, "plan was created without charges");
    RuleTable rt{p->d_rules, p->d_offset, p->nkinds};
    hipError_t e;
    if (culled) {
        const bool probe0 = p->nprobes > 0 && mode != MODE_COULOMB;
        e = launch_culled(mode, probe0 ? p->probes[0].d_pc : p->d_pc, p->g, probe0 ? p->probes[0].vdwk : p->vdwk,
                          p->ew2 ? 2 : (p->fast_ewald ? 1 : 0), out, pts, stream);
    } else {
        AtomTable at{p->d_atoms, p->has_rules ? p->d_kind : nullptr, p->natoms};
        e = launch_bruteforce(mode, p->g, at, rt, out, pts, stream);
    }
    if (e != hipSuccess) return fail(CEG_ERR_HIP, "kernel launch failed: %s", hipGetErrorString(e));
    return CEG_OK;
}

int build_common(ceg_plan* p, int mode, double lv, double tv, double lc, double tc, int32_t i_begin,
                 int32_t i_end, float* d_v, float* d_c, int64_t channel_stride, int32_t i_origin,
                 int32_t algo, void* stream)
{
    if (!p) return fail(CEG_ERR_INVALID, "plan is NULL");
    if (i_begin < 0 || i_end > p->g.dims[0] + 1 || i_begin > i_end)
        return fail(CEG_ERR_INVALID, "bad x-plane range [%d,%d) for dims[0]+1 = %d", i_begin, i_end, p->g.dims[0] + 1);
    if (i_origin > i_begin) return fail(CEG_ERR_INVALID, "i_origin %d > i_begin %d", i_origin, i_begin);
    if ((mode != MODE_COULOMB && !d_v) || (mode != MODE_VDW && !d_c)) return fail(CEG_ERR_INVALID, "output pointer is NULL");
    const int64_t plane = (int64_t)(p->g.dims[1] + 1) * (p->g.dims[2] + 1);
    if (channel_stride < (int64_t)(i_end - i_origin) * plane)
        return fail(CEG_ERR_INVALID, "channel_stride %lld too small", (long long)channel_stride);
    bool culled;
    if (int rc = resolve_algo(p, algo, &culled)) return rc;
    Output out{};
    out.vdw = d_v;
    out.coulomb = d_c;
    out.channel_stride = channel_stride;
    out.i_origin = i_origin;
    out.i_begin = i_begin;
    out.i_end = i_end;
    out.lambda_vdw = lv;
    out.thr_vdw = tv;
    out.lambda_coulomb = lc;
    out.thr_coulomb = tc;
    DeviceGuard guard(p->device);
    if (!guard.ok) return fail(CEG_ERR_HIP, "hipSetDevice(%d) failed", p->device);
    return run(p, mode, out, Points{nullptr, 0}, culled, (hipStream_t)stream);
}

}

extern "C" int ceg_plan_build_vdw(ceg_plan_t* plan, double lambda, double threshold, int32_t i_begin,
                                  int32_t i_end, float* d_out, int64_t channel_stride, int32_t i_origin,
                                  int32_t algo, void* stream)
{
    return build_common(plan, MODE_VDW, lambda, threshold, 0, 0, i_begin, i_end, d_out, nullptr, channel_stride,
                        i_origin, algo, stream);
}

extern "C" int ceg_plan_build_coulomb(ceg_plan_t* plan, double lambda, double threshold, int32_t i_begin,
                                      int32_t i_end, float* d_out, int64_t channel_stride, int32_t i_origin,
                                      int32_t algo, void* stream)
{
    return build_common(plan, MODE_COULOMB, 0, 0, lambda, threshold, i_begin, i_end, nullptr, d_out,
                        channel_stride, i_origin, algo, stream);
}

extern "C" int ceg_plan_build_fused(ceg_plan_t* plan, double lambda_vdw, double threshold_vdw,
                                    double lambda_coulomb, double threshold_coulomb, int32_t i_begin,
                                    int32_t i_end, float* d_out_vdw, float* d_out_coulomb,
                                    int64_t channel_stride, int32_t i_origin, int32_t algo, void* stream)
{
    return build_common(plan, MODE_FUSED, lambda_vdw, threshold_vdw, lambda_coulomb, threshold_coulomb, i_begin,
                        i_end, d_out_vdw, d_out_coulomb, channel_stride, i_origin, algo, stream);
}

extern "C" int ceg_plan_build_multi(ceg_plan_t* p, double lambda_vdw, double threshold_vdw, double lambda_coulomb, double threshold_coulomb,
                                    int32_t i_begin, int32_t i_end, float* const* d_out_vdw, float* d_out_coulomb,
                                    int64_t channel_stride, int32_t i_origin, void* stream)
{
    if (!p) return fail(CEG_ERR_INVALID, "plan is NULL");
    if (p->nprobes < 1) return fail(CEG_ERR_INVALID, "not a multi-probe plan (ceg_plan_create_multi)");
    if (i_begin < 0 || i_end > p->g.dims[0] + 1 || i_begin > i_end)
        return fail(CEG_ERR_INVALID, "bad x-plane range [%d,%d) for dims[0]+1 = %d", i_begin, i_end, p->g.dims[0] + 1);
    if (i_origin > i_begin) return fail(CEG_ERR_INVALID, "i_origin %d > i_begin %d", i_origin, i_begin);
    const int64_t plane = (int64_t)(p->g.dims[1] + 1) * (p->g.dims[2] + 1);
    if (channel_stride < (int64_t)(i_end - i_origin) * plane) return fail(CEG_ERR_INVALID, "channel_stride %lld too small", (long long)channel_stride);
    if (d_out_coulomb && !p->has_charge) return fail(CEG_ERR_INVALID, "plan was created without charges");
    std::vector<int> req;
    for (int q = 0; q < p->nprobes; ++q)
        if (d_out_vdw && d_out_vdw[q]) req.push_back(q);
    if (req.empty() && !d_out_coulomb) return CEG_OK;
    Output base{};
    base.channel_stride = channel_stride;
    base.i_origin = i_origin;
    base.i_begin = i_begin;
    base.i_end = i_end;
    base.lambda_vdw = lambda_vdw;
    base.thr_vdw = threshold_vdw;
    base.lambda_coulomb = lambda_coulomb;
    base.thr_coulomb = threshold_coulomb;
    DeviceGuard guard(p->device);
    if (!guard.ok) return fail(CEG_ERR_HIP, "hipSetDevice(%d) failed", p->device);
    hipStream_t st = (hipStream_t)stream;
    hipError_t e = hipSuccess;
    const int ewk = p->ew2 ? 2 : (p->fast_ewald ? 1 : 0);
    auto single = [&](int mode, int q) {
        Output o = base;
        o.vdw = q >= 0 ? d_out_vdw[q] : nullptr;
        o.coulomb = mode != MODE_VDW ? d_out_coulomb : nullptr;
        return launch_culled(mode, q >= 0 ? p->probes[q].d_pc : p->d_pc, p->g, q >= 0 ? p->probes[q].vdwk : 1, ewk, o, Points{nullptr, 0}, st);
    };
    auto multi = [&](int mode, const int* idx, int np) {
        Output o = base;
        for (int t = 0; t < np; ++t) { o.vdwm[t] = d_out_vdw[idx[t]]; o.probe_idx[t] = idx[t]; }
        o.coulomb = mode == MODE_FUSED ? d_out_coulomb : nullptr;
        return launch_culled_multi(mode, np, p->d_pc, p->g, o, st);
    };
    std::vector<int> lj, other;
    for (int q : req) (p->probes[q].vdwk == 1 ? lj : other).push_back(q);
    if (d_out_coulomb) {
        int fused_np = CEG_MAX_PROBES_FUSED;
        if (const char* env = std::getenv("CEG_HIP_MULTI_FUSED_NP")) fused_np = std::max(0, std::min(CEG_MAX_PROBES_FUSED, atoi(env)));
        if (!p->ew2 && p->nprobes > 1) fused_np = 0;
        if (fused_np >= 2 && lj.size() >= 2) {
            e = multi(MODE_FUSED, &lj[0], 2);
            lj.erase(lj.begin(), lj.begin() + 2);
        } else if (fused_np >= 1 && !other.empty()) {
            e = single(MODE_FUSED, other[0]);
            other.erase(other.begin());
        } else if (fused_np >= 1 && !lj.empty()) {
            e = single(MODE_FUSED, lj[0]);
            lj.erase(lj.begin());
        } else {
            e = single(MODE_COULOMB, -1);
        }
    }
    size_t at = 0;
    while (e == hipSuccess && at < lj.size()) {
        const int n = (int)std::min<size_t>(CEG_MAX_PROBES, lj.size() - at);
        e = n == 1 ? single(MODE_VDW, lj[at]) : multi(MODE_VDW, &lj[at], n);
        at += (size_t)n;
    }
    for (size_t t = 0; e == hipSuccess && t < other.size(); ++t) e = single(MODE_VDW, other[t]);
    if (e != hipSuccess) return fail(CEG_ERR_HIP, "kernel launch failed: %s", hipGetErrorString(e));
    return CEG_OK;
}

extern "C" int ceg_plan_eval_points(ceg_plan_t* p, int32_t which, int32_t algo, const double* points,
                                    int64_t npoints, double* out)
{
    if (!p) return fail(CEG_ERR_INVALID, "plan is NULL");
    if (npoints < 0 || (npoints > 0 && (!points || !out))) return fail(CEG_ERR_INVALID, "bad points/out");
    if (which != 0 && which != 1) return fail(CEG_ERR_INVALID, "which must be 0 (vdw) or 1 (coulomb)");
    if (npoints == 0) return CEG_OK;
    bool culled;
    if (int rc = resolve_algo(p, algo, &culled)) return rc;
    if (culled) {
        bool inside = true;
        for (int64_t q = 0; q < npoints && inside; ++q)
            for (int a = 0; a < 3; ++a) {
                const double x = points[3 * q + a];
                if (!(x >= p->g.shift[a] - 1e-9 && x <= p->g.shift[a] + p->g.size[a] + 1e-9)) inside = false;
            }
        if (!inside) {
            if (algo == CEG_ALGO_CULLED)
                return fail(CEG_ERR_UNSUPPORTED, "culled evaluation needs points inside the grid bounding box");
            culled = false;
        }
    }
    DeviceGuard guard(p->device);
    if (!guard.ok) return fail(CEG_ERR_HIP, "hipSetDevice(%d) failed", p->device);
    double* d_pts = nullptr;
    double* d_out = nullptr;
    HIP_TRY(hipMalloc((void**)&d_pts, sizeof(double) * 3 * npoints));
    if (hipMalloc((void**)&d_out, sizeof(double) * 8 * npoints) != hipSuccess) {
        (void)hipFree(d_pts);
        return fail(CEG_ERR_HIP, "hipMalloc failed");
    }
    int rc = CEG_OK;
    if (hipMemcpy(d_pts, points, sizeof(double) * 3 * npoints, hipMemcpyHostToDevice) != hipSuccess)
        rc = fail(CEG_ERR_HIP, "hipMemcpy H2D failed");
    if (!rc) {
        Output o{};
        if (which == 0) o.raw_vdw = d_out; else o.raw_coulomb = d_out;
        rc = run(p, which == 0 ? MODE_VDW : MODE_COULOMB, o, Points{d_pts, npoints}, culled, nullptr);
    }
    if (!rc && hipDeviceSynchronize() != hipSuccess) rc = fail(CEG_ERR_HIP, "kernel execution failed: %s", hipGetErrorString(hipGetLastError()));
    if (!rc && hipMemcpy(out, d_out, sizeof(double) * 8 * npoints, hipMemcpyDeviceToHost) != hipSuccess)
        rc = fail(CEG_ERR_HIP, "hipMemcpy D2H failed");
    (void)hipFree(d_pts);
    (void)hipFree(d_out);
    return rc;
}

extern "C" int ceg_release_cached_buffers(void)
{
    ceg_host::oneshot_pools_release();
    image_cache_release();
    block_cache_release();
    return CEG_OK;
}
```

### crystalenergygrids.jl_amd/csrc/ceg_internal.h

```cpp
#pragma once

#include <hip/hip_runtime.h>
#include <stdint.h>

#include "../../include/ceg_hip.h"

namespace ceg {

enum Mode : int { MODE_VDW = 0, MODE_COULOMB = 1, MODE_FUSED = 2 };

struct DevRule {
    int32_t kind;
    int32_t _pad;
    double  p0, p1, p2;
    double  shift;
};

struct Geom {
    double mat[9];
    double invmat[9];
    double size[3];
    double shift[3];
    double delta[3];
    int32_t dims[3];
    int32_t ortho;
    double safemin2;
    double cutoff2;
    double alpha;
    int32_t diag;
    int32_t _pad;
};


struct Output {
    float*  vdw;
    float*  coulomb;
    double* raw_vdw;
    double* raw_coulomb;
    int64_t channel_stride;
    int32_t i_origin;
    int32_t i_begin, i_end;
    double  lambda_vdw, thr_vdw;
    double  lambda_coulomb, thr_coulomb;
    float*  vdwm[CEG_MAX_PROBES];
    int32_t probe_idx[CEG_MAX_PROBES];
};

struct Points {
    const double* xyz;
    int64_t n;
};

struct AtomTable {
    const double4* xyzq;
    const int32_t* kind;
    int64_t n;
};

struct RuleTable {
    const DevRule* rules;
    const int32_t* offset;
    int32_t nkinds;
};

struct ImageBins {
    const double4* xyzq;
    const int32_t* kind;
    const int32_t* atom;
    const double4* atoms;
    const int32_t* bin_start;
    double lo[3];
    double inv_bin[3];
    double bin[3];
    int32_t nb[3];
    int32_t nimages;
};

struct FastVdw {
    double p0, p1, p2, shift;
    int32_t cls;
    int32_t _pad;
};

struct PlanConst {
    Geom g;
    ImageBins ib;
    RuleTable rt;
    const FastVdw* fastvdw;
    double r_exact2;
    const double* erfcx_tab;
    const double* exp2_tab;
    double erfcx_inv_h;
    double erfcx_mx0_inv_h;
    double alpha2;
    const double* ew2_tab;
    int32_t ew2_ni;
    int32_t ew2_base;
    double ew_k3, ew_k15;
    const double* bk2_tab;
    int32_t bk2_ni, bk2_base;
    double bk_B, bk_C, bk_invC;
    double bk_nshift, bk_c1, bk_c2, bk_c3, bk_c4;
    double bk_s1, bk_s2, bk_s3;
    int32_t all_simple;
    int32_t nprobes;
    RuleTable rtm[CEG_MAX_PROBES];
    const FastVdw* fastm[CEG_MAX_PROBES];
};

constexpr int CEG_ERFCX_TAB_N = 128;
#ifndef CEG_R_EXACT2_VALUE
#define CEG_R_EXACT2_VALUE 4.0
#endif
constexpr double CEG_R_EXACT2 = CEG_R_EXACT2_VALUE;

constexpr int CEG_EW2_LOGM = 5;
constexpr int CEG_EW2_SHIFT = 20 - CEG_EW2_LOGM;
constexpr int CEG_EW2_STRIDE = 14;
#ifndef CEG_EW2_LDS_STRIDE
#define CEG_EW2_LDS_STRIDE 14
#endif
constexpr int CEG_EW2_NI_MAX = 176;
constexpr int CEG_BK2_ND = 8;
constexpr int CEG_BK2_STRIDE = 10;
constexpr int CEG_BK2_LOGM = CEG_EW2_LOGM;
constexpr int CEG_BK2_SHIFT = 20 - CEG_BK2_LOGM;
constexpr int CEG_BK2_NI_MAX = CEG_EW2_NI_MAX;
constexpr double CEG_BK2_TOL = 2e-14;

hipError_t launch_bruteforce(int mode, const Geom& g, const AtomTable& atoms, const RuleTable& rt,
                             const Output& out, const Points& pts, hipStream_t stream);
hipError_t launch_culled(int mode, const PlanConst* d_pc, const Geom& g, int vdwk, int ewk,
                         const Output& out, const Points& pts, hipStream_t stream);
constexpr int CEG_MAX_PROBES_FUSED = 2;
hipError_t launch_culled_multi(int mode, int np, const PlanConst* d_pc, const Geom& g, const Output& out, hipStream_t stream);

}
```

### crystalenergygrids.jl_amd/csrc/ceg_kernels.hip

```cpp
#include <type_traits>

#include "ceg_internal.h"
#include "ceg_math.h"
#include "ceg_minimage.h"

namespace ceg {

struct Accum {
    double v, d1x, d1y, d1z, d2xy, d2xz, d2yz, d3;
};

__device__ __forceinline__ void accum_zero(Accum& a)
{
    a.v = a.d1x = a.d1y = a.d1z = a.d2xy = a.d2xz = a.d2yz = a.d3 = 0.0;
}

__device__ __forceinline__ void accum_add(Accum& a, double v, double p1, double p2, double p3,
                                          double dx, double dy, double dz)
{
    a.v += v;
    a.d1x += p1 * dx;
    a.d1y += p1 * dy;
    a.d1z += p1 * dz;
    const double d13 = dx * dz;
    a.d2xy += p2 * (dx * dy);
    a.d2xz += p2 * d13;
    a.d2yz += p2 * (dy * dz);
    a.d3 += p3 * d13 * dy;
}

__device__ __forceinline__ double grid_coord(int i, double size, int dims, double shift)
{
#pragma clang fp contract(off)
    return __dadd_rn(__ddiv_rn(__dmul_rn((double)i, size), (double)dims), shift);
}

__device__ __attribute__((noinline)) double exp_out_of_line(double x) { return exp(x); }

template <bool LJONLY = false, bool COLD = false>
__device__ __forceinline__ void vdw_terms(const DevRule* __restrict__ rules, int rb, int re, double r2,
                                          double& v_out, double& p1_out, double& p2_out, double& p3_out)
{
    double v = 0.0, p1 = 0.0, p2 = 0.0, p3 = 0.0;
    for (int t = rb; t < re; ++t) {
        const int kind = rules[t].kind;
        const double q0 = rules[t].p0, q1 = rules[t].p1, q2 = rules[t].p2, sh = rules[t].shift;
        double tv, t1 = 0.0, t2 = 0.0, t3 = 0.0;
        if (LJONLY || kind == CEG_LENNARDJONES) {
            const double inv = 1.0 / r2;
            const double s = q1 * inv;
            const double x6 = s * s * s;
            const double inv2 = inv * inv;
            tv = 4.0 * q0 * x6 * (x6 - 1.0);
            t1 = 24.0 * q0 * (x6 * (1.0 - 2.0 * x6)) * inv;
            t2 = 96.0 * q0 * (x6 * (7.0 * x6 - 2.0)) * inv2;
            t3 = 384.0 * q0 * (x6 * (5.0 - 28.0 * x6)) * (inv2 * inv2);
        } else if (kind == CEG_BUCKINGHAM) {
            const double A = q0, B = q1, C = q2;
            const double r4 = r2 * r2;
            const double r = sqrt(r2);
            const double r6 = r4 * r2;
            const double x6 = C / r6;
            const double xe = A * (COLD ? exp_out_of_line(-B * r) : exp(-B * r));
            tv = xe - x6;
            t1 = -B * xe / r + 6.0 * x6 / r2;
            t2 = -48.0 * x6 / r4 + B * xe * (1.0 + B * r) / (r2 * r);
            t3 = -(3.0 * B * r + B * B * r2 + 3.0) * B * xe * r / r6 + 480.0 * C / (r6 * r6);
        } else {
            tv = (r2 < q0) ? __builtin_huge_val() : 0.0;
        }
        v += tv - sh;
        p1 += t1;
        p2 += t2;
        p3 += t3;
    }
    v_out = v; p1_out = p1; p2_out = p2; p3_out = p3;
}

__device__ __forceinline__ void ewald_terms(double alpha, double charge, double r2,
                                            double& v, double& p1, double& p2, double& p3)
{
    const double inv_sqrtpi = 0.56418958354775628695;
    const double r = sqrt(r2);
    const double r3 = r2 * r;
    const double r5 = r3 * r2;
    const double r2a2 = r2 * (alpha * alpha);
    const double er2a2 = 2.0 * alpha * r * exp(-r2a2) * inv_sqrtpi;
    const double erfar = erfc(alpha * r);
    v = charge * erfar / r;
    p1 = -charge * (er2a2 + erfar) / r3;
    p2 = charge * (er2a2 * (3.0 + 2.0 * r2a2) + 3.0 * erfar) / r5;
    p3 = charge * (-er2a2 * (15.0 + 10.0 * r2a2 + 4.0 * (r2a2 * r2a2)) - 15.0 * erfar) / (r5 * r2);
}

__device__ __forceinline__ void ewald_terms_poly(double alpha, double charge, double r2,
                                                 double& v, double& p1, double& p2, double& p3)
{
    const double inv_sqrtpi = 0.56418958354775628695;
    const double r = sqrt(r2);
    const double r3 = r2 * r;
    const double r5 = r3 * r2;
    const double r2a2 = r2 * (alpha * alpha);
    const double E = fast_exp_neg(-r2a2);
    const double er2a2 = 2.0 * alpha * r * E * inv_sqrtpi;
    const double erfar = E * erfcx_poly(alpha * r);
    v = charge * erfar / r;
    p1 = -charge * (er2a2 + erfar) / r3;
    p2 = charge * (er2a2 * (3.0 + 2.0 * r2a2) + 3.0 * erfar) / r5;
    p3 = charge * (-er2a2 * (15.0 + 10.0 * r2a2 + 4.0 * (r2a2 * r2a2)) - 15.0 * erfar) / (r5 * r2);
}

__device__ __attribute__((noinline)) double4 ewald_terms_poly_call(double alpha, double charge, double r2)
{
    double v, p1, p2, p3;
    ewald_terms_poly(alpha, charge, r2, v, p1, p2, p3);
    return make_double4(v, p1, p2, p3);
}
__device__ __attribute__((noinline)) double4 lj_terms_call(const DevRule* __restrict__ rules, int rb, int re, double r2)
{
    double v, p1, p2, p3;
    vdw_terms<true, true>(rules, rb, re, r2, v, p1, p2, p3);
    return make_double4(v, p1, p2, p3);
}

__device__ __forceinline__ double clamp_julia(double x, double lo, double hi)
{
    return (x > hi) ? hi : ((x < lo) ? lo : x);
}

__device__ __forceinline__ void store_gridpoint(float* __restrict__ out, int64_t idx, int64_t cs,
                                                const double* delta, double lambda, double thr, Accum a)
{
#pragma clang fp contract(off)
    if (a.v > thr) {
        a.v = 2.0 * thr;
        a.d1x = clamp_julia(a.d1x, -thr, thr);
        a.d1y = clamp_julia(a.d1y, -thr, thr);
        a.d1z = clamp_julia(a.d1z, -thr, thr);
        a.d2xy = a.d2xz = a.d2yz = 0.0;
        a.d3 = 0.0;
    }
    const double D1 = delta[0], D2 = delta[1], D3 = delta[2];
    out[idx] = (float)__dmul_rn(a.v, lambda);
    out[idx + cs] = (float)__dmul_rn(__dmul_rn(a.d1x, D1), lambda);
    out[idx + 2 * cs] = (float)__dmul_rn(__dmul_rn(a.d1y, D2), lambda);
    out[idx + 3 * cs] = (float)__dmul_rn(__dmul_rn(a.d1z, D3), lambda);
    out[idx + 4 * cs] = (float)__dmul_rn(__dmul_rn(a.d2xy, __dmul_rn(D1, D2)), lambda);
    out[idx + 5 * cs] = (float)__dmul_rn(__dmul_rn(a.d2xz, __dmul_rn(D1, D3)), lambda);
    out[idx + 6 * cs] = (float)__dmul_rn(__dmul_rn(a.d2yz, __dmul_rn(D2, D3)), lambda);
    out[idx + 7 * cs] = (float)__dmul_rn(__dmul_rn(a.d3, __dmul_rn(__dmul_rn(D1, D2), D3)), lambda);
}

__device__ __forceinline__ void gridpoint8(float r[8], const double* delta, double lambda, double thr, Accum a)
{
#pragma clang fp contract(off)
    if (a.v > thr) {
        a.v = 2.0 * thr;
        a.d1x = clamp_julia(a.d1x, -thr, thr);
        a.d1y = clamp_julia(a.d1y, -thr, thr);
        a.d1z = clamp_julia(a.d1z, -thr, thr);
        a.d2xy = a.d2xz = a.d2yz = 0.0;
        a.d3 = 0.0;
    }
    const double D1 = delta[0], D2 = delta[1], D3 = delta[2];
    r[0] = (float)__dmul_rn(a.v, lambda);
    r[1] = (float)__dmul_rn(__dmul_rn(a.d1x, D1), lambda);
    r[2] = (float)__dmul_rn(__dmul_rn(a.d1y, D2), lambda);
    r[3] = (float)__dmul_rn(__dmul_rn(a.d1z, D3), lambda);
    r[4] = (float)__dmul_rn(__dmul_rn(a.d2xy, __dmul_rn(D1, D2)), lambda);
    r[5] = (float)__dmul_rn(__dmul_rn(a.d2xz, __dmul_rn(D1, D3)), lambda);
    r[6] = (float)__dmul_rn(__dmul_rn(a.d2yz, __dmul_rn(D2, D3)), lambda);
    r[7] = (float)__dmul_rn(__dmul_rn(a.d3, __dmul_rn(__dmul_rn(D1, D2), D3)), lambda);
}

typedef float ceg_v4f __attribute__((ext_vector_type(4)));
__device__ __forceinline__ void store_float4_unaligned(float* dst, float4 v)
{
    const ceg_v4f u = {v.x, v.y, v.z, v.w};
    asm volatile("global_store_dwordx4 %0, %1, off" : : "v"(dst), "v"(u) : "memory");
}

__device__ __forceinline__ void store_raw(double* __restrict__ out, int64_t p, const Accum& a)
{
    double* o = out + 8 * p;
    o[0] = a.v;  o[1] = a.d1x;  o[2] = a.d1y;  o[3] = a.d1z;
    o[4] = a.d2xy;  o[5] = a.d2xz;  o[6] = a.d2yz;  o[7] = a.d3;
}

template <int MODE>
__device__ __forceinline__ void write_results(const Geom& g, const Output& out, bool points_mode,
                                              int64_t pidx, int i, int j, int k,
                                              Accum av, Accum ac, double smallest_d2)
{
    if (MODE != MODE_VDW) {
        ac.v = (smallest_d2 < 1.0) ? __builtin_huge_val() : ac.v;
    }
    if (points_mode) {
        if (MODE != MODE_COULOMB && out.raw_vdw) store_raw(out.raw_vdw, pidx, av);
        if (MODE != MODE_VDW && out.raw_coulomb) store_raw(out.raw_coulomb, pidx, ac);
        return;
    }
    const int64_t nz = g.dims[2] + 1, ny = g.dims[1] + 1;
    const int64_t idx = (int64_t)k + nz * ((int64_t)j + ny * (int64_t)(i - out.i_origin));
    if (MODE != MODE_COULOMB && out.vdw)
        store_gridpoint(out.vdw, idx, out.channel_stride, g.delta, out.lambda_vdw, out.thr_vdw, av);
    if (MODE != MODE_VDW && out.coulomb)
        store_gridpoint(out.coulomb, idx, out.channel_stride, g.delta, out.lambda_coulomb, out.thr_coulomb, ac);
}

__device__ __forceinline__ double periodic_distance2_literal(const Geom& g, double& dx, double& dy, double& dz)
{
    return periodic_distance2_literal_m(g.mat, g.invmat, g.ortho, g.safemin2, dx, dy, dz);
}

template <int MODE, bool POINTS>
__global__ __launch_bounds__(256) void k_bruteforce(Geom g, AtomTable atoms, RuleTable rt, Output out,
                                                     Points pts, int64_t total)
{
    __shared__ double4 s_xyzq[256];
    __shared__ int32_t s_kind[256];

    const int tid = threadIdx.x;
    const int64_t t = (int64_t)blockIdx.x * 256 + tid;
    const bool valid = t < total;
    int i = 0, j = 0, k = 0;
    double px, py, pz;
    if (POINTS) {
        const int64_t tt = valid ? t : 0;
        px = pts.xyz[3 * tt]; py = pts.xyz[3 * tt + 1]; pz = pts.xyz[3 * tt + 2];
    } else {
        const int64_t nz = g.dims[2] + 1, ny = g.dims[1] + 1;
        const int64_t tt = valid ? t : 0;
        k = (int)(tt % nz);
        j = (int)((tt / nz) % ny);
        i = out.i_begin + (int)(tt / (nz * ny));
        px = grid_coord(i, g.size[0], g.dims[0], g.shift[0]);
        py = grid_coord(j, g.size[1], g.dims[1], g.shift[1]);
        pz = grid_coord(k, g.size[2], g.dims[2], g.shift[2]);
    }

    Accum av, ac;
    accum_zero(av);
    accum_zero(ac);
    double smallest_d2 = __builtin_huge_val();

    for (int64_t base = 0; base < atoms.n; base += 256) {
        __syncthreads();
        const int64_t a = base + tid;
        if (a < atoms.n) {
            s_xyzq[tid] = atoms.xyzq[a];
            s_kind[tid] = atoms.kind ? atoms.kind[a] : -1;
        }
        __syncthreads();
        const int m = (int)((atoms.n - base < 256) ? (atoms.n - base) : 256);
        for (int q = 0; q < m; ++q) {
            const double4 A = s_xyzq[q];
            double dx = px - A.x, dy = py - A.y, dz = pz - A.z;
            const double d2 = periodic_distance2_literal(g, dx, dy, dz);
            if (d2 >= g.cutoff2) continue;
            if (MODE != MODE_COULOMB) {
                const int kd = __builtin_amdgcn_readfirstlane(s_kind[q]);
                if (kd >= 0) {
                    const int rb = rt.offset[kd], re = rt.offset[kd + 1];
                    if (re > rb) {
                        double v, p1, p2, p3;
                        vdw_terms(rt.rules, rb, re, d2, v, p1, p2, p3);
                        accum_add(av, v, p1, p2, p3, dx, dy, dz);
                    }
                }
            }
            if (MODE != MODE_VDW) {
                smallest_d2 = fmin(smallest_d2, d2);
                double v, p1, p2, p3;
                ewald_terms(g.alpha, A.w, d2, v, p1, p2, p3);
                accum_add(ac, v, p1, p2, p3, dx, dy, dz);
            }
        }
    }
    if (valid) write_results<MODE>(g, out, POINTS, t, i, j, k, av, ac, smallest_d2);
}

#ifndef CEG_WAVES_FUSED_BUCK
#define CEG_WAVES_FUSED_BUCK CEG_WAVES
#endif
#ifndef CEG_WAVES_FUSED_LJ
#define CEG_WAVES_FUSED_LJ CEG_WAVES
#endif
#ifndef CEG_WAVES_VDW_LJ
#define CEG_WAVES_VDW_LJ CEG_WAVES
#endif
#ifndef CEG_WAVES_VDW_BUCK
#define CEG_WAVES_VDW_BUCK CEG_WAVES
#endif
#ifndef CEG_WAVES_COULOMB
#define CEG_WAVES_COULOMB CEG_WAVES
#endif
#ifndef CEG_WAVES
#define CEG_WAVES 4
#endif
#ifndef CEG_WG
#define CEG_WG 256
#endif
#ifndef CEG_WAVES_MULTI_FUSED
#define CEG_WAVES_MULTI_FUSED 4
#endif
#ifndef CEG_WAVES_MULTI_VDW
#define CEG_WAVES_MULTI_VDW 4
#endif
#ifndef CEG_NW_MULTI_FUSED
#define CEG_NW_MULTI_FUSED 8
#endif
constexpr int culled_waves(int mode, int vdwk, int ewk, int np = 1)
{
    return np > 1 ? (mode == 2 ? CEG_WAVES_MULTI_FUSED : (np == 2 ? CEG_WAVES_MULTI_VDW : 3))
           : (mode == 2 && vdwk >= 2 && ewk) ? CEG_WAVES_FUSED_BUCK
           : (mode == 2 && vdwk == 1 && ewk) ? CEG_WAVES_FUSED_LJ
           : (mode == 0 && vdwk == 1)      ? CEG_WAVES_VDW_LJ
           : (mode == 0 && vdwk >= 2)      ? CEG_WAVES_VDW_BUCK
           : (mode == 1 && ewk)            ? CEG_WAVES_COULOMB
                                           : CEG_WAVES;
}
#ifndef CEG_NW_EW2
#define CEG_NW_EW2 8
#endif
constexpr int culled_nw(int mode, int vdwk, int ewk, int np = 1)
{
    return np > 1 ? (mode == 2 ? CEG_NW_MULTI_FUSED : CEG_WG / 64)
                  : ((mode != 0 && ewk == 2) || (mode != 1 && vdwk == 3)) ? CEG_NW_EW2 : CEG_WG / 64;
}
[[maybe_unused]] constexpr double R_EXACT2 = CEG_R_EXACT2;
static_assert(ERFCX_TAB_N == CEG_ERFCX_TAB_N, "table size mismatch");
constexpr int META_SIMPLE = 1 << 24;
constexpr int META_HASVDW = 1 << 25;
constexpr int META_BUCK = 1 << 26;
constexpr int META_KINDMASK = (1 << 24) - 1;

struct __attribute__((aligned(16))) Quad { double x, y, z, w; };
struct __attribute__((aligned(16))) CandRec {
    Quad xyzq;
    Quad lj;
    int32_t meta;
    int32_t atom;
    int32_t _pad[2];
};

template <int MODE, bool FASTEW, bool LJSLOW, bool EWSCALED, bool BKSCALED, int NP, bool DOV = true, bool DOC = true, typename Rec>
__device__ __forceinline__ void slow_pairs(const PlanConst* __restrict__ pc, unsigned long long cands, int lane,
                                           double px, double py, double pz,
                                           const Rec* s_rec,
                                           const unsigned long long* s_odd,
                                           Accum* avm, const int32_t* probe_idx, Accum& ac, double& smallest_d2)
{
    Accum& av = avm[0];
    const Geom& g = pc->g;
    while (cands != 0ull) {
        const int q = __builtin_ctzll(cands);
        cands &= cands - 1ull;
        const unsigned long long lanes = s_odd[q];
        if (!((lanes >> lane) & 1ull)) continue;
        const int mt = s_rec[q].meta;
        const double4 O = pc->ib.atoms[s_rec[q].atom];
        double dx = px - O.x, dy = py - O.y, dz = pz - O.z;
        const double r2 = periodic_distance2_literal(g, dx, dy, dz);
        if (r2 >= g.cutoff2) continue;
        if constexpr (NP > 1) {
            if (DOV && (mt & META_HASVDW)) {
                const int kd = mt & META_KINDMASK;
#pragma unroll
                for (int p = 0; p < NP; ++p) {
                    const RuleTable& rtp = pc->rtm[probe_idx[p]];
                    const int rb = rtp.offset[kd], re = rtp.offset[kd + 1];
                    if (re == rb) continue;
                    const double4 T = lj_terms_call(rtp.rules, rb, re, r2);
                    accum_add(avm[p], T.x, T.y * (-1.0 / 6.0), T.z * (1.0 / 48.0), T.w * (-1.0 / 480.0), dx, dy, dz);
                }
            }
        } else if (MODE != MODE_COULOMB && (mt & META_HASVDW)) {
            const int kd = mt & META_KINDMASK;
            double v, p1, p2, p3;
            vdw_terms<LJSLOW, true>(pc->rt.rules, pc->rt.offset[kd], pc->rt.offset[kd + 1], r2, v, p1, p2, p3);
            if (LJSLOW) {
                p1 *= -1.0 / 6.0; p2 *= 1.0 / 48.0; p3 *= -1.0 / 480.0;
            }
            if (BKSCALED) {
                v *= pc->bk_invC; p1 *= pc->bk_s1; p2 *= pc->bk_s2; p3 *= pc->bk_s3;
            }
            accum_add(av, v, p1, p2, p3, dx, dy, dz);
        }
        if (MODE != MODE_VDW && DOC) {
            smallest_d2 = fmin(smallest_d2, r2);
            double v, p1, p2, p3;
            if constexpr (NP > 1) {
                const double4 T = ewald_terms_poly_call(g.alpha, O.w, r2);
                v = T.x; p1 = T.y; p2 = T.z; p3 = T.w;
            } else if (FASTEW)
                ewald_terms_poly(g.alpha, O.w, r2, v, p1, p2, p3);
            else
                ewald_terms(g.alpha, O.w, r2, v, p1, p2, p3);
            if (EWSCALED) {
                p2 *= 1.0 / 3.0; p3 *= 1.0 / 15.0;
            }
            accum_add(ac, v, p1, p2, p3, dx, dy, dz);
        }
    }
}

__device__ __forceinline__ int mad_u24(int a, int b, int c)
{
    int r;
    asm("v_mad_u32_u24 %0, %1, %2, %3" : "=v"(r) : "v"(a), "v"(b), "s"(c));
    return r;
}

__device__ __forceinline__ double uniform(double x)
{
    int lo = __double2loint(x), hi = __double2hiint(x);
    asm("" : "+v"(lo));
    asm("" : "+v"(hi));
    return __hiloint2double(__builtin_amdgcn_readfirstlane(hi), __builtin_amdgcn_readfirstlane(lo));
}

__device__ __forceinline__ double wave_min(double x)
{
#pragma unroll
    for (int o = 32; o > 0; o >>= 1) x = fmin(x, __shfl_xor(x, o));
    return x;
}
__device__ __forceinline__ double wave_max(double x)
{
#pragma unroll
    for (int o = 32; o > 0; o >>= 1) x = fmax(x, __shfl_xor(x, o));
    return x;
}

static_assert(sizeof(CandRec) == 80, "candidate record layout");
struct __attribute__((aligned(16))) CandRecS {
    Quad xyzq;
    int32_t meta;
    int32_t atom;
    int32_t _pad[2];
};
static_assert(sizeof(CandRecS) == 48, "candidate record layout");
template <int NP>
struct __attribute__((aligned(16))) CandRecM {
    Quad xyzq;
    double ljm[3 * NP + (NP & 1)];
    int32_t meta;
    int32_t atom;
    int32_t _pad[2];
};
static_assert(sizeof(CandRecM<2>) == 96 && sizeof(CandRecM<3>) == 128 && sizeof(CandRecM<4>) == 144, "candidate record layout");
template <int NP> __device__ __forceinline__ Quad lj_record(const CandRecM<NP>& r, int p) { return Quad{r.ljm[3 * p], 0.0, r.ljm[3 * p + 1], r.ljm[3 * p + 2]}; }
__device__ __forceinline__ Quad lj_record(const CandRec& r, int) { return r.lj; }
__device__ __forceinline__ Quad lj_record(const CandRecS&, int) { return Quad{0.0, 0.0, 0.0, 0.0}; }
template <int NP> __device__ __forceinline__ void set_lj_record(CandRecM<NP>& r, int p, Quad q) { r.ljm[3 * p] = q.x; r.ljm[3 * p + 1] = q.z; r.ljm[3 * p + 2] = q.w; }
__device__ __forceinline__ void set_lj_record(CandRec& r, int, Quad q) { r.lj = q; }
__device__ __forceinline__ void set_lj_record(CandRecS&, int, Quad) {}

template <int MODE, bool POINTS, int VDWK, int EWK, int NP = 1>
__global__ __launch_bounds__(64 * culled_nw(MODE, VDWK, EWK, NP), culled_waves(MODE, VDWK, EWK, NP)) void k_culled(const PlanConst* __restrict__ pc, Output out, Points pts,
                                                              int tiles_j, int tiles_k, int64_t ntiles)
{
    static_assert(NP >= 1 && NP <= CEG_MAX_PROBES && (NP == 1 || (VDWK == 1 && !POINTS && EWK == 2 && MODE != MODE_COULOMB)), "multi-probe variant");
    constexpr bool MULTI = NP > 1;
    constexpr bool FASTEW = EWK != 0;
    constexpr bool EW2 = EWK == 2 && MODE != MODE_VDW;
    constexpr int WG = 64 * culled_nw(MODE, VDWK, EWK, NP);
    constexpr bool BK2 = VDWK == 3 && MODE != MODE_COULOMB;
    constexpr int NW = WG / 64;
    constexpr bool HAS_LJ = !MULTI && (VDWK == 1 || VDWK == 2) && MODE != MODE_COULOMB;
    using Rec = std::conditional_t<MULTI, CandRecM<NP>, std::conditional_t<HAS_LJ, CandRec, CandRecS>>;
    __shared__ __attribute__((aligned(16))) Rec s_rec_all[NW][64];
    __shared__ int32_t s_rowstart_all[NW][64];
    __shared__ int32_t s_rowprefix_all[NW][66];
    __shared__ unsigned long long s_odd_all[NW][64];
    __shared__ __attribute__((aligned(16))) double s_erfcx[EW2 ? 2 : ERFCX_TAB_N * 6];
    constexpr int EW2_LS = (NP == 1) ? CEG_EW2_LDS_STRIDE : CEG_EW2_STRIDE;
    __shared__ __attribute__((aligned(16))) double s_ew2[EW2 ? CEG_EW2_NI_MAX * EW2_LS : 2];
    __shared__ __attribute__((aligned(16))) double s_bk2[BK2 ? CEG_BK2_NI_MAX * CEG_BK2_STRIDE : 2];
    __shared__ double s_exp2[64];
    __shared__ int32_t s_org[NW][4];

    const int wave = __builtin_amdgcn_readfirstlane(threadIdx.x >> 6);
    Rec* s_rec = s_rec_all[wave];
    int32_t* s_rowstart = s_rowstart_all[wave];
    int32_t* s_rowprefix = s_rowprefix_all[wave];
    unsigned long long* s_odd = s_odd_all[wave];

    constexpr bool FASTVDW = VDWK != 0;
    if (EW2) {
        const int nt = pc->ew2_ni * CEG_EW2_STRIDE;
        for (int t = threadIdx.x; t < nt; t += WG) s_ew2[(t / CEG_EW2_STRIDE) * EW2_LS + t % CEG_EW2_STRIDE] = pc->ew2_tab[t];
    } else if (FASTEW && MODE != MODE_VDW) {
        for (int t = threadIdx.x; t < ERFCX_TAB_N * 6; t += WG) s_erfcx[t] = pc->erfcx_tab[t];
    }
    if (BK2) {
        const int nt = pc->bk2_ni * CEG_BK2_STRIDE;
        for (int t = threadIdx.x; t < nt; t += WG) s_bk2[t] = pc->bk2_tab[t];
    }
    if ((FASTEW && !EW2 && MODE != MODE_VDW) || (VDWK == 2 && MODE != MODE_COULOMB))
        if (threadIdx.x < 64) s_exp2[threadIdx.x] = pc->exp2_tab[threadIdx.x];
    __syncthreads();
    const int64_t tile_raw = (int64_t)blockIdx.x * NW + wave;
    const bool active = tile_raw < ntiles;
    const int64_t tile = active ? tile_raw : ntiles - 1;

    const Geom& g = pc->g;
    const ImageBins& ib = pc->ib;
    const RuleTable& rt = pc->rt;
    const int lane = threadIdx.x & 63;
    const double cutoff2 = g.cutoff2;
    const double r_exact2 = pc->r_exact2;
    const double alpha = g.alpha;
    const int32_t ortho = g.ortho;
    const double safemin2 = g.safemin2;

    int i = 0, j = 0, k = 0;
    int i0 = 0, j0 = 0, k0 = 0;
    int64_t pidx = 0;
    bool valid;
    double px, py, pz;
    if (POINTS) {
        pidx = tile * 64 + lane;
        valid = active && pidx < pts.n;
        const int64_t tt = valid ? pidx : (pts.n - 1);
        px = pts.xyz[3 * tt]; py = pts.xyz[3 * tt + 1]; pz = pts.xyz[3 * tt + 2];
    } else {
        const int tj = (int)((tile / tiles_k) % tiles_j);
        const int ti = (int)(tile / ((int64_t)tiles_k * tiles_j));
        const int nq = (tiles_k + NW - 1) / NW;
        const int tk = (int)((tile % tiles_k + (int64_t)NW * ((ti + (out.i_begin >> 2) + tj) % nq)) % tiles_k);
        i0 = out.i_begin + 4 * ti; j0 = 4 * tj; k0 = 4 * tk;
        if (lane == 0) {
            s_org[wave][0] = active ? i0 : -1;
            s_org[wave][1] = j0;
            s_org[wave][2] = k0;
        }
        i = i0 + (lane >> 4);
        j = j0 + ((lane >> 2) & 3);
        k = k0 + (lane & 3);
        valid = active && (i < out.i_end) && (j <= g.dims[1]) && (k <= g.dims[2]);
        const int ci = i < out.i_end ? i : out.i_end - 1;
        const int cj = j <= g.dims[1] ? j : g.dims[1];
        const int ck = k <= g.dims[2] ? k : g.dims[2];
        px = grid_coord(ci, g.size[0], g.dims[0], g.shift[0]);
        py = grid_coord(cj, g.size[1], g.dims[1], g.shift[1]);
        pz = grid_coord(ck, g.size[2], g.dims[2], g.shift[2]);
    }

    const double blx = uniform(wave_min(px)), bhx = uniform(wave_max(px));
    const double bly = uniform(wave_min(py)), bhy = uniform(wave_max(py));
    const double blz = uniform(wave_min(pz)), bhz = uniform(wave_max(pz));
    const double cx = uniform(0.5 * (blx + bhx)), cy = uniform(0.5 * (bly + bhy)), cz = uniform(0.5 * (blz + bhz));
    const double hx = uniform(0.5 * (bhx - blx)), hy = uniform(0.5 * (bhy - bly)), hz = uniform(0.5 * (bhz - blz));
    const double rc2 = uniform(cutoff2 * (1.0 + 1e-9) + 1e-9);
    const double rc = uniform(sqrt(rc2));

    auto bin_of = [&](double x, int ax) -> int {
        int b = (int)floor((x - ib.lo[ax]) * ib.inv_bin[ax]);
        b = b < 0 ? 0 : b;
        return b >= ib.nb[ax] ? ib.nb[ax] - 1 : b;
    };
    const int bx0 = bin_of(blx - rc, 0), bx1 = bin_of(bhx + rc, 0);
    const int by0 = bin_of(bly - rc, 1), by1 = bin_of(bhy + rc, 1);
    const int nry = by1 - by0 + 1;
    const int nrows = active ? (bx1 - bx0 + 1) * nry : 0;
    const float inv_nry = __int_as_float(__builtin_amdgcn_readfirstlane(__float_as_int(1.0f / (float)nry)));

    Accum avm[NP], ac;
#pragma unroll
    for (int p = 0; p < NP; ++p) accum_zero(avm[p]);
    Accum& av = avm[0];
    accum_zero(ac);
    double smallest_d2 = __builtin_huge_val();
    const double band_cut = 1e-9 * cutoff2;
    const double alpha2 = pc->alpha2;
    const bool stale_possible = !ortho && safemin2 < cutoff2;
    const double cut_hi = uniform(cutoff2 + band_cut);
    const double reg_hi = uniform(stale_possible ? fmin(cutoff2 - band_cut, safemin2 * (1.0 - 1e-9)) : cutoff2 - band_cut);
    const double erf_inv_h = pc->erfcx_inv_h, erf_mx0 = pc->erfcx_mx0_inv_h;
    const int hi_lo = __builtin_amdgcn_readfirstlane(__double2hiint(r_exact2) + (__double2loint(r_exact2) != 0 ? 1 : 0));
    const int hi_top = __builtin_amdgcn_readfirstlane(__double2hiint(reg_hi));
    const unsigned hi_span = hi_top > hi_lo ? (unsigned)(hi_top - hi_lo) : 0u;
    const int hi_cut = __builtin_amdgcn_readfirstlane(__double2hiint(cut_hi));
    const double int_lo = uniform(r_exact2 * (1.0 + 4e-6)), int_hi = uniform(reg_hi * (1.0 - 4e-6));
    const int ew2_off = EW2 ? __builtin_amdgcn_readfirstlane(-pc->ew2_base * (EW2_LS * 8)) : 0;
    int ew2_stride = EW2_LS * 8;
    asm volatile("" : "+v"(ew2_stride));
    const double ew_k3 = pc->ew_k3, ew_k15 = pc->ew_k15;
    const bool all_simple = __builtin_amdgcn_readfirstlane(pc->all_simple) != 0;
    const int bk2_off = BK2 ? __builtin_amdgcn_readfirstlane(-pc->bk2_base * (CEG_BK2_STRIDE * 8)) : 0;
    int bk2_stride = CEG_BK2_STRIDE * 8;
    asm volatile("" : "+v"(bk2_stride));
    const double bk_B = pc->bk_B, bk_nshift = pc->bk_nshift, bk_c1 = pc->bk_c1, bk_c2 = pc->bk_c2, bk_c3 = pc->bk_c3, bk_c4 = pc->bk_c4;

    for (int rbase = 0; rbase < nrows; rbase += 64) {
        int count = 0, start = 0;
        const int r = rbase + lane;
        if (r < nrows) {
            const int rq = (int)(((float)r + 0.5f) * inv_nry);
            const int bx = bx0 + rq, by = by0 + (r - rq * nry);
            const double colx0 = ib.lo[0] + bx * ib.bin[0], colx1 = colx0 + ib.bin[0];
            const double coly0 = ib.lo[1] + by * ib.bin[1], coly1 = coly0 + ib.bin[1];
            const double gx = fmax(0.0, fmax(blx - colx1, colx0 - bhx));
            const double gy = fmax(0.0, fmax(bly - coly1, coly0 - bhy));
            const double dxy2 = gx * gx + gy * gy;
            if (dxy2 < rc2) {
                const double zr = sqrt(rc2 - dxy2);
                const int bz0 = bin_of(blz - zr, 2), bz1 = bin_of(bhz + zr, 2);
                const int64_t rowbase = ((int64_t)bx * ib.nb[1] + by) * ib.nb[2];
                start = ib.bin_start[rowbase + bz0];
                count = ib.bin_start[rowbase + bz1 + 1] - start;
            }
        }
        int ln = lane;
        asm volatile("" : "+v"(ln));
        int incl = count;
#pragma unroll
        for (int o = 1; o < 64; o <<= 1) {
            const int up = __builtin_amdgcn_ds_bpermute((ln - o) << 2, incl);
            if (ln >= o) incl += up;
        }
        __builtin_amdgcn_wave_barrier();
        s_rowstart[ln] = start;
        s_rowprefix[ln + 1] = incl;
        if (ln == 0) s_rowprefix[0] = 0;
        __builtin_amdgcn_wave_barrier();
        const int total = __builtin_amdgcn_readfirstlane(s_rowprefix[64]);

        for (int cbase = 0; cbase < total; cbase += 64) {
            const int t = cbase + lane;
            bool keep = false, interior = false;
            double4 P = make_double4(0, 0, 0, 0);
            double4 LJ = make_double4(0, 0, 0, 0);
            double4 LJM[NP];
#pragma unroll
            for (int p = 0; p < NP; ++p) LJM[p] = make_double4(0, 0, 0, 0);
            int meta = 0, aidx = 0;
            if (t < total) {
                int lo = 0, hi = 64;
#pragma unroll
                for (int s = 0; s < 6; ++s) {
                    const int mid = (lo + hi) >> 1;
                    if (s_rowprefix[mid] <= t) lo = mid; else hi = mid;
                }
                const int img = s_rowstart[lo] + (t - s_rowprefix[lo]);
                P = ib.xyzq[img];
                aidx = ib.atom[img];
                const int kw = ib.kind ? ib.kind[img] : -1;
                const int kd = kw < 0 ? -1 : (kw & META_KINDMASK);
                const double qx = fmax(0.0, fabs(cx - P.x) - hx);
                const double qy = fmax(0.0, fabs(cy - P.y) - hy);
                const double qz = fmax(0.0, fabs(cz - P.z) - hz);
                const double dmin2 = qx * qx + qy * qy + qz * qz;
                keep = dmin2 < rc2;
                const double fx = fabs(cx - P.x) + hx, fy = fabs(cy - P.y) + hy, fz = fabs(cz - P.z) + hz;
                interior = dmin2 > int_lo && (fx * fx + fy * fy + fz * fz) < int_hi;
                bool hasvdw = false;
                int vclass = 0;
                if (MODE != MODE_COULOMB && kd >= 0) {
                    hasvdw = (kw & META_HASVDW) != 0;
                    if constexpr (MULTI) {
                        if (hasvdw && keep) {
#pragma unroll
                            for (int p = 0; p < NP; ++p) {
                                const FastVdw F = pc->fastm[out.probe_idx[p]][kd];
                                LJM[p] = make_double4(F.p0, F.p1, F.p2, F.shift);
                            }
                        }
                    } else if (FASTVDW && VDWK != 3 && hasvdw && keep) {
                        const FastVdw F = pc->fastvdw[kd];
                        LJ = make_double4(F.p0, F.p1, F.p2, F.shift);
                        vclass = F.cls;
                    }
                }
                if (MODE == MODE_VDW) keep = keep && hasvdw;
                bool simple = g.diag != 0 || (!POINTS && all_simple);
                if (!simple && keep) {
                    const double* I = g.invmat;
                    const double ux = cx - P.x, uy = cy - P.y, uz = cz - P.z;
                    const double f0 = I[0] * ux + I[3] * uy + I[6] * uz;
                    const double f1 = I[1] * ux + I[4] * uy + I[7] * uz;
                    const double f2 = I[2] * ux + I[5] * uy + I[8] * uz;
                    const double e0 = fabs(I[0]) * hx + fabs(I[3]) * hy + fabs(I[6]) * hz + 1e-9;
                    const double e1 = fabs(I[1]) * hx + fabs(I[4]) * hy + fabs(I[7]) * hz + 1e-9;
                    const double e2 = fabs(I[2]) * hx + fabs(I[5]) * hy + fabs(I[8]) * hz + 1e-9;
                    simple = (fabs(f0) + e0 < 0.5) && (fabs(f1) + e1 < 0.5) && (fabs(f2) + e2 < 0.5);
                }
                meta = (kd & META_KINDMASK) | (simple ? META_SIMPLE : 0) | (hasvdw ? META_HASVDW : 0) |
                       (vclass == 2 ? META_BUCK : 0);
            }
#ifdef CEG_SKIP_TESTS
            keep = keep && (P.x == 12345.678);
#endif
            const bool simple_c = (meta & META_SIMPLE) != 0;
            const bool withv = MODE != MODE_COULOMB && (meta & META_HASVDW) != 0;
            const bool ks = keep && simple_c;
            const unsigned long long mask_vi = __builtin_amdgcn_ballot_w64(ks && withv && interior);
            const unsigned long long mask_vb = __builtin_amdgcn_ballot_w64(ks && withv && !interior);
            const unsigned long long mask_ni = __builtin_amdgcn_ballot_w64(ks && !withv && interior);
            const unsigned long long mask_nb = __builtin_amdgcn_ballot_w64(ks && !withv && !interior);
            const unsigned long long mask_x = __builtin_amdgcn_ballot_w64(keep && !simple_c);
            const int nvi = __popcll(mask_vi), nv = nvi + __popcll(mask_vb), nni = nv + __popcll(mask_ni), nreg = nni + __popcll(mask_nb),
                      nkeep = nreg + __popcll(mask_x);
            __builtin_amdgcn_wave_barrier();
            if (keep) {
                const unsigned long long mine = !simple_c ? mask_x : (withv ? (interior ? mask_vi : mask_vb) : (interior ? mask_ni : mask_nb));
                const int first = !simple_c ? nreg : (withv ? (interior ? 0 : nvi) : (interior ? nv : nni));
                const int slot = first + __builtin_amdgcn_mbcnt_hi((unsigned)(mine >> 32), __builtin_amdgcn_mbcnt_lo((unsigned)mine, 0));
                s_rec[slot].xyzq = Quad{P.x, P.y, P.z, P.w};
                if constexpr (MULTI) {
#pragma unroll
                    for (int p = 0; p < NP; ++p) set_lj_record(s_rec[slot], p, Quad{LJM[p].x, LJM[p].y, LJM[p].z, LJM[p].w});
                } else if constexpr (HAS_LJ) s_rec[slot].lj = Quad{LJ.x, LJ.y, LJ.z, LJ.w};
                s_rec[slot].meta = meta;
                s_rec[slot].atom = aidx;
            }
            __builtin_amdgcn_wave_barrier();

            unsigned long long slow = 0ull;
            auto pair_body = [&](const int q, auto with_vdw_tag, auto interior_tag) __attribute__((always_inline)) {
                constexpr bool WITH_VDW = decltype(with_vdw_tag)::value;
                constexpr bool INTERIOR = decltype(interior_tag)::value;
                const Quad A = s_rec[q].xyzq;
                double dx = px - A.x, dy = py - A.y, dz = pz - A.z;
                const double r2 = dx * dx + dy * dy + dz * dz;
                const int hi = __double2hiint(r2);
                if constexpr (!INTERIOR) {
                    const unsigned long long m_in = __builtin_amdgcn_uicmp((unsigned)(hi - hi_lo), hi_span, 36);
                    const unsigned long long oddlanes = __builtin_amdgcn_sicmp(hi, hi_cut, 41) & ~m_in;
                    if (oddlanes != 0ull) {
                        slow |= 1ull << q;
                        if (lane == 0) s_odd[q] = oddlanes;
                    }
                    if (!((unsigned)(hi - hi_lo) < hi_span)) return;
                }

                const double dxy = dx * dy, dxz = dx * dz, dyz = dy * dz;
                const double dxyz = dxz * dy;
                double rr = 0.0, rinv = 0.0, inv = 0.0;
                constexpr bool NEED_SQRT = (VDWK >= 2 && MODE != MODE_COULOMB) || (EWK == 1 && MODE != MODE_VDW);
                if (NEED_SQRT) {
                    fast_sqrt_rsqrt(r2, rr, rinv);
                    inv = rinv * rinv;
                } else if (FASTVDW || EW2) {
                    inv = fast_rcp(r2);
                }
                int key = 0;
                double t = 0.0;
                static_assert(CEG_BK2_SHIFT == CEG_EW2_SHIFT, "the Buckingham table shares the interval key of the Ewald tables");
                if (EW2 || (BK2 && WITH_VDW)) {
                    key = (int)((unsigned)hi >> CEG_EW2_SHIFT);
                    t = r2 - __hiloint2double(hi & (int)(0xffffffffu << CEG_EW2_SHIFT), 0);
                }
                if constexpr (WITH_VDW && MULTI) {
                    const double inv2 = inv * inv;
                    const double y3 = inv2 * inv;
                    const double inv4 = inv2 * inv2;
#pragma unroll
                    for (int p = 0; p < NP; ++p) {
                        const Quad L = lj_record(s_rec[q], p);
                        const double x6 = L.z * y3;
                        const double w = L.x * x6;
                        const double u = w * x6;
                        const double v = (u - w) - L.w;
                        const double p1 = __builtin_fma(u, 2.0, -w) * inv;
                        const double p2 = fms_vsv(u, 3.5, w) * inv2;
                        const double p3 = fms_vsv(u, 5.6, w) * inv4;
                        Accum& a = avm[p];
                        a.v += v;
                        a.d1x = __builtin_fma(p1, dx, a.d1x);
                        a.d1y = __builtin_fma(p1, dy, a.d1y);
                        a.d1z = __builtin_fma(p1, dz, a.d1z);
                        a.d2xy = __builtin_fma(p2, dxy, a.d2xy);
                        a.d2xz = __builtin_fma(p2, dxz, a.d2xz);
                        a.d2yz = __builtin_fma(p2, dyz, a.d2yz);
                        a.d3 = __builtin_fma(p3, dxyz, a.d3);
                    }
                } else if constexpr (WITH_VDW) {
                    double v, p1, p2, p3;
                    if constexpr (VDWK == 3) {
                        const double2* rec = reinterpret_cast<const double2*>(
                            reinterpret_cast<const char*>(s_bk2) + mad_u24(key, bk2_stride, bk2_off));
                        const double2 g01 = rec[0], g23 = rec[1], g45 = rec[2], g67 = rec[3];
                        double g0 = __builtin_fma(g67.y, t, g67.x);
                        g0 = __builtin_fma(g0, t, g45.y);
                        g0 = __builtin_fma(g0, t, g45.x);
                        g0 = __builtin_fma(g0, t, g23.y);
                        g0 = __builtin_fma(g0, t, g23.x);
                        g0 = __builtin_fma(g0, t, g01.y);
                        g0 = __builtin_fma(g0, t, g01.x);
                        const double u = g0 * rinv;
                        const double inv2 = inv * inv, y3 = inv2 * inv;
                        const double w = fma_vsv(g0, bk_B, u);
                        const double wi = w * inv;
                        v = add_sc(g0 - y3, bk_nshift);
                        p1 = fma_vsv(u, bk_c1, y3 * inv);
                        p2 = fma_vsv(wi, bk_c2, y3 * inv2);
                        p3 = fma_vsv(fma_vsv(u, bk_c3, wi) * inv, bk_c4, y3 * y3);
                    } else if constexpr (HAS_LJ) {
                      if (VDWK == 2 && (__builtin_amdgcn_readfirstlane(s_rec[q].meta) & META_BUCK)) {
                        const Quad L = lj_record(s_rec[q], 0);
                        const double Br = L.y * rr;
                        const double xe = L.x * exp_neg_tab(s_exp2, -Br);
                        const double inv2 = inv * inv;
                        const double x6 = L.z * (inv2 * inv);
                        const double Bxe = L.y * xe;
                        const double rinv3 = rinv * inv;
                        v = (xe - x6) - L.w;
                        p1 = __builtin_fma(mul_sc(x6, 6.0), inv, -Bxe * rinv);
                        p2 = __builtin_fma(mul_sc(x6, -48.0), inv2, (Bxe * rinv3) * (1.0 + Br));
                        p3 = __builtin_fma(mul_sc(x6, 480.0), inv2 * inv,
                                           -((Bxe * rinv3) * inv) * __builtin_fma(Br, add_sc(Br, 3.0), 3.0));
                      } else {
                        const Quad L = lj_record(s_rec[q], 0);
                        const double inv2 = inv * inv;
                        const double x6 = L.z * (inv2 * inv);
                        const double w = L.x * x6;
                        const double u = w * x6;
                        v = (u - w) - L.w;
                        p1 = __builtin_fma(u, 2.0, -w) * inv;
                        p2 = fms_vsv(u, 3.5, w) * inv2;
                        p3 = fms_vsv(u, 5.6, w) * (inv2 * inv2);
                        if (VDWK != 1) {
                            p1 = mul_sc(p1, -6.0); p2 = mul_sc(p2, 48.0); p3 = mul_sc(p3, -480.0);
                        }
                      }
                    } else {
                        const int kd = __builtin_amdgcn_readfirstlane(s_rec[q].meta) & META_KINDMASK;
                        vdw_terms(rt.rules, rt.offset[kd], rt.offset[kd + 1], r2, v, p1, p2, p3);
                    }
                    av.v += v;
                    av.d1x = __builtin_fma(p1, dx, av.d1x);
                    av.d1y = __builtin_fma(p1, dy, av.d1y);
                    av.d1z = __builtin_fma(p1, dz, av.d1z);
                    av.d2xy = __builtin_fma(p2, dxy, av.d2xy);
                    av.d2xz = __builtin_fma(p2, dxz, av.d2xz);
                    av.d2yz = __builtin_fma(p2, dyz, av.d2yz);
                    av.d3 = __builtin_fma(p3, dxyz, av.d3);
                }
                if (MODE != MODE_VDW) {
                    double v, p1, p2, p3;
                    if (EW2) {
                        const char* recp = reinterpret_cast<const char*>(s_ew2) + mad_u24(key, ew2_stride, ew2_off);
                        double2 a01, a23, a45, a6c0, c12, c34, c56;
                        if (EW2_LS % 2 == 0) {
                            const double2* rec = reinterpret_cast<const double2*>(recp);
                            a01 = rec[0]; a23 = rec[1]; a45 = rec[2]; a6c0 = rec[3]; c12 = rec[4]; c34 = rec[5]; c56 = rec[6];
                        } else {
                            const double* rec = reinterpret_cast<const double*>(recp);
                            a01 = make_double2(rec[0], rec[1]); a23 = make_double2(rec[2], rec[3]); a45 = make_double2(rec[4], rec[5]);
                            a6c0 = make_double2(rec[6], rec[7]); c12 = make_double2(rec[8], rec[9]); c34 = make_double2(rec[10], rec[11]);
                            c56 = make_double2(rec[12], rec[13]);
                        }
                        double b0 = __builtin_fma(a6c0.x, t, a45.y);
                        double cc = __builtin_fma(c56.y, t, c56.x);
                        b0 = __builtin_fma(b0, t, a45.x);
                        cc = __builtin_fma(cc, t, c34.y);
                        b0 = __builtin_fma(b0, t, a23.y);
                        cc = __builtin_fma(cc, t, c34.x);
                        b0 = __builtin_fma(b0, t, a23.x);
                        cc = __builtin_fma(cc, t, c12.y);
                        b0 = __builtin_fma(b0, t, a01.y);
                        cc = __builtin_fma(cc, t, c12.x);
                        b0 = __builtin_fma(b0, t, a01.x);
                        cc = __builtin_fma(cc, t, a6c0.y);
                        const double qb0 = A.w * b0, qc = A.w * cc;
                        const double b1 = (qb0 + qc) * inv;
                        const double b2 = fma_vsv(qc, ew_k3, b1) * inv;
                        const double b3 = fma_vsv(qc, ew_k15, b2) * inv;
                        v = qb0; p1 = -b1; p2 = b2; p3 = -b3;
                    } else if (FASTEW) {
                        const double x = alpha * rr;
                        const double x2 = alpha2 * r2;
                        const double E = exp_neg_tab(s_exp2, -x2);
                        const double gx = erfcx_tab(s_erfcx, x, erf_inv_h, erf_mx0);
                        const double kx = mul_sc(x, 1.1283791670955125739);
                        const double qe1 = (A.w * rinv) * E;
                        const double qe3 = qe1 * inv, qe5 = qe3 * inv, qe7 = qe5 * inv;
                        v = qe1 * gx;
                        p1 = -qe3 * (kx + gx);
                        p2 = qe5 * __builtin_fma(kx, fma2_sc(x2, 3.0), mul_sc(gx, 3.0));
                        p3 = -qe7 * __builtin_fma(kx, fma_sc(fma4_sc(x2, 10.0), x2, 15.0), mul_sc(gx, 15.0));
                    } else {
                        smallest_d2 = min_nonan(smallest_d2, r2);
                        ewald_terms(alpha, A.w, r2, v, p1, p2, p3);
                    }
                    ac.v += v;
                    ac.d1x = __builtin_fma(p1, dx, ac.d1x);
                    ac.d1y = __builtin_fma(p1, dy, ac.d1y);
                    ac.d1z = __builtin_fma(p1, dz, ac.d1z);
                    ac.d2xy = __builtin_fma(p2, dxy, ac.d2xy);
                    ac.d2xz = __builtin_fma(p2, dxz, ac.d2xz);
                    ac.d2yz = __builtin_fma(p2, dyz, ac.d2yz);
                    ac.d3 = __builtin_fma(p3, dxyz, ac.d3);
                }
            };
#ifdef CEG_STAGING_ONLY
            if (nkeep == 12345) { av.v += s_rec[0].xyzq.x; ac.v += s_rec[1].xyzq.y; }
            continue;
#endif
            if (MODE != MODE_COULOMB) {
                for (int q = 0; q < nvi; ++q) pair_body(q, std::true_type{}, std::true_type{});
                for (int q = nvi; q < nv; ++q) pair_body(q, std::true_type{}, std::false_type{});
            }
            if (MODE != MODE_VDW) {
                for (int q = (MODE == MODE_COULOMB ? 0 : nv); q < nni; ++q) pair_body(q, std::false_type{}, std::true_type{});
                for (int q = nni; q < nreg; ++q) pair_body(q, std::false_type{}, std::false_type{});
            }
            for (int q = nreg; q < nkeep; ++q) {
                const Quad A = s_rec[q].xyzq;
                const double dx = px - A.x, dy = py - A.y, dz = pz - A.z;
                const double r2 = dx * dx + dy * dy + dz * dz;
                const unsigned long long lanes = __builtin_amdgcn_sicmp(__double2hiint(r2), hi_cut, 41);
                if (lanes != 0ull) {
                    slow |= 1ull << q;
                    if (lane == 0) s_odd[q] = lanes;
                }
            }
#ifdef CEG_NO_EXACT_PATH
            slow = 0ull;
#endif
            if (slow != 0ull) {
                __builtin_amdgcn_wave_barrier();
                if constexpr (MULTI && MODE == MODE_FUSED) {
                    slow_pairs<MODE, FASTEW, true, EW2, false, NP, true, false>(pc, slow, lane, px, py, pz, s_rec, s_odd, avm, out.probe_idx, ac, smallest_d2);
                    slow_pairs<MODE, FASTEW, true, EW2, false, NP, false, true>(pc, slow, lane, px, py, pz, s_rec, s_odd, avm, out.probe_idx, ac, smallest_d2);
                } else
                    slow_pairs<MODE, FASTEW, VDWK == 1, EW2, VDWK == 3 && MODE != MODE_COULOMB, NP>(pc, slow, lane, px, py, pz, s_rec, s_odd, avm, out.probe_idx, ac, smallest_d2);
            }
        }
    }
    if (VDWK == 1 && MODE != MODE_COULOMB) {
#pragma unroll
        for (int p = 0; p < NP; ++p) {
            Accum& a = avm[p];
            a.d1x *= -6.0; a.d1y *= -6.0; a.d1z *= -6.0;
            a.d2xy *= 48.0; a.d2xz *= 48.0; a.d2yz *= 48.0;
            a.d3 *= -480.0;
        }
    }
    if (VDWK == 3 && MODE != MODE_COULOMB) {
        const double C = pc->bk_C;
        av.v *= C;
        av.d1x *= 6.0 * C; av.d1y *= 6.0 * C; av.d1z *= 6.0 * C;
        av.d2xy *= -48.0 * C; av.d2xz *= -48.0 * C; av.d2yz *= -48.0 * C;
        av.d3 *= 480.0 * C;
    }
    if (EW2) {
        ac.d2xy *= 3.0; ac.d2xz *= 3.0; ac.d2yz *= 3.0;
        ac.d3 *= 15.0;
    }
    if (POINTS) {
        if (valid) write_results<MODE>(g, out, true, pidx, i, j, k, av, ac, smallest_d2);
        return;
    }
#ifdef CEG_SKIP_OUTPUT
    if (av.v + ac.v == 12345.678 && lane == 0) out.vdw[0] = 1.0f;
    return;
#endif
    constexpr bool TWO_PASS = MODE == MODE_FUSED && sizeof(Rec) * 64 < 2 * 512 * sizeof(float);
    const int64_t nz = g.dims[2] + 1, ny = g.dims[1] + 1;
    constexpr int NSEG = 8 * 16 * NW;
    if (MODE != MODE_VDW) ac.v = (smallest_d2 < 1.0) ? __builtin_huge_val() : ac.v;
    if constexpr (MULTI) {
        constexpr int NGRID = NP + (MODE == MODE_FUSED ? 1 : 0);
        float* sm = reinterpret_cast<float*>(s_rec_all[wave]);
#pragma unroll
        for (int gi = 0; gi < NGRID; ++gi) {
            if (gi == 0) __builtin_amdgcn_wave_barrier(); else __syncthreads();
            float r[8];
            if (gi < NP) gridpoint8(r, g.delta, out.lambda_vdw, out.thr_vdw, avm[gi < NP ? gi : 0]);
            else gridpoint8(r, g.delta, out.lambda_coulomb, out.thr_coulomb, ac);
#pragma unroll
            for (int c = 0; c < 8; ++c) sm[c * 64 + lane] = r[c];
            __syncthreads();
            float* base = gi < NP ? out.vdwm[gi < NP ? gi : 0] : out.coulomb;
            for (int seg = threadIdx.x; seg < NSEG; seg += WG) {
                const int w = seg % NW;
                const int row = seg / NW;
                const int c = row >> 4, li = (row >> 2) & 3, lj = row & 3;
                const int oi = s_org[w][0];
                if (oi < 0) continue;
                const int gi_ = oi + li, gj = s_org[w][1] + lj, gk = s_org[w][2];
                if (gi_ >= out.i_end || gj > g.dims[1] || gk > g.dims[2]) continue;
                const int64_t idx = (int64_t)gk + nz * ((int64_t)gj + ny * (int64_t)(gi_ - out.i_origin)) + (int64_t)c * out.channel_stride;
                const int so = c * 64 + li * 16 + lj * 4;
                const int nvalid = (g.dims[2] + 1 - gk) < 4 ? (g.dims[2] + 1 - gk) : 4;
                const float4 v = *reinterpret_cast<const float4*>(reinterpret_cast<const float*>(s_rec_all[w]) + so);
                float* dst = base + idx;
                if (nvalid == 4) store_float4_unaligned(dst, v);
                else { dst[0] = v.x; if (nvalid > 1) dst[1] = v.y; if (nvalid > 2) dst[2] = v.z; }
            }
        }
        return;
    }
#pragma unroll
    for (int pass = 0; pass < (TWO_PASS ? 2 : 1); ++pass) {
        const bool do_v = MODE != MODE_COULOMB && (!TWO_PASS || pass == 0);
        const bool do_c = MODE != MODE_VDW && (!TWO_PASS || pass == 1);
        const int off_c = (MODE == MODE_FUSED && !TWO_PASS) ? 512 : 0;
        float* sm = reinterpret_cast<float*>(s_rec_all[wave]);
        if (pass == 0) __builtin_amdgcn_wave_barrier(); else __syncthreads();
        if (do_v) {
            float r[8];
            gridpoint8(r, g.delta, out.lambda_vdw, out.thr_vdw, av);
#pragma unroll
            for (int c = 0; c < 8; ++c) sm[c * 64 + lane] = r[c];
        }
        if (do_c) {
            float r[8];
            gridpoint8(r, g.delta, out.lambda_coulomb, out.thr_coulomb, ac);
#pragma unroll
            for (int c = 0; c < 8; ++c) sm[off_c + c * 64 + lane] = r[c];
        }
        __syncthreads();
        for (int seg = threadIdx.x; seg < NSEG; seg += WG) {
            const int w = seg % NW;
            const int row = seg / NW;
            const int c = row >> 4, li = (row >> 2) & 3, lj = row & 3;
            const int oi = s_org[w][0];
            if (oi < 0) continue;
            const int gi = oi + li, gj = s_org[w][1] + lj, gk = s_org[w][2];
            if (gi >= out.i_end || gj > g.dims[1] || gk > g.dims[2]) continue;
            const int64_t idx = (int64_t)gk + nz * ((int64_t)gj + ny * (int64_t)(gi - out.i_origin)) + (int64_t)c * out.channel_stride;
            const int so = c * 64 + li * 16 + lj * 4;
            const int nvalid = (g.dims[2] + 1 - gk) < 4 ? (g.dims[2] + 1 - gk) : 4;
            if (do_v) {
                const float4 v = *reinterpret_cast<const float4*>(reinterpret_cast<const float*>(s_rec_all[w]) + so);
                float* dst = out.vdw + idx;
                if (nvalid == 4) store_float4_unaligned(dst, v);
                else { dst[0] = v.x; if (nvalid > 1) dst[1] = v.y; if (nvalid > 2) dst[2] = v.z; }
            }
            if (do_c) {
                const float4 v = *reinterpret_cast<const float4*>(reinterpret_cast<const float*>(s_rec_all[w]) + off_c + so);
                float* dst = out.coulomb + idx;
                if (nvalid == 4) store_float4_unaligned(dst, v);
                else { dst[0] = v.x; if (nvalid > 1) dst[1] = v.y; if (nvalid > 2) dst[2] = v.z; }
            }
        }
    }
}

template <bool POINTS>
static hipError_t launch_bf_t(int mode, const Geom& g, const AtomTable& atoms, const RuleTable& rt,
                              const Output& out, const Points& pts, int64_t total, hipStream_t stream)
{
    if (total <= 0) return hipSuccess;
    const int64_t nblocks = (total + 255) / 256;
    if (nblocks > 0x7fffffffLL) return hipErrorInvalidValue;
    dim3 grid((unsigned)nblocks), block(256);
    switch (mode) {
    case MODE_VDW:
        hipLaunchKernelGGL((k_bruteforce<MODE_VDW, POINTS>), grid, block, 0, stream, g, atoms, rt, out, pts, total);
        break;
    case MODE_COULOMB:
        hipLaunchKernelGGL((k_bruteforce<MODE_COULOMB, POINTS>), grid, block, 0, stream, g, atoms, rt, out, pts, total);
        break;
    default:
        hipLaunchKernelGGL((k_bruteforce<MODE_FUSED, POINTS>), grid, block, 0, stream, g, atoms, rt, out, pts, total);
        break;
    }
    return hipGetLastError();
}

hipError_t launch_bruteforce(int mode, const Geom& g, const AtomTable& atoms, const RuleTable& rt,
                             const Output& out, const Points& pts, hipStream_t stream)
{
    if (pts.xyz) return launch_bf_t<true>(mode, g, atoms, rt, out, pts, pts.n, stream);
    const int64_t total = (int64_t)(out.i_end - out.i_begin) * (g.dims[1] + 1) * (g.dims[2] + 1);
    return launch_bf_t<false>(mode, g, atoms, rt, out, pts, total, stream);
}

template <int MODE, bool POINTS>
static hipError_t launch_cull_flags(int vdwk, int ewk, hipStream_t stream, const PlanConst* pc, const Output& out, const Points& pts,
                                    int tj, int tk, int64_t ntiles)
{
    if (MODE == MODE_VDW) ewk = 1;
    if (MODE == MODE_COULOMB) vdwk = 1;
    if (ewk == 2 && vdwk == 0) ewk = 1;
    if (vdwk == 3 && MODE == MODE_FUSED && ewk != 2) vdwk = 2;
    const int nw = culled_nw(MODE, vdwk, ewk);
    const int64_t nblocks = (ntiles + nw - 1) / nw;
    if (nblocks > 0x7fffffffLL) return hipErrorInvalidValue;
    const dim3 grid((unsigned)nblocks), block(64 * nw);
#define CEG_LAUNCH(V, F) hipLaunchKernelGGL((k_culled<MODE, POINTS, V, F>), grid, block, 0, stream, pc, out, pts, tj, tk, ntiles)
    if (ewk == 2 && MODE != MODE_VDW) {
        if (vdwk == 1) CEG_LAUNCH(1, 2); else if (vdwk == 3) CEG_LAUNCH(3, 2); else CEG_LAUNCH(2, 2);
    } else if (ewk) {
        if (vdwk == 1) CEG_LAUNCH(1, 1); else if (vdwk == 2) CEG_LAUNCH(2, 1); else if (vdwk == 3) CEG_LAUNCH(3, 1); else CEG_LAUNCH(0, 1);
    } else {
        if (vdwk == 1) CEG_LAUNCH(1, 0); else if (vdwk == 2) CEG_LAUNCH(2, 0); else if (vdwk == 3) CEG_LAUNCH(2, 0); else CEG_LAUNCH(0, 0);
    }
#undef CEG_LAUNCH
    return hipGetLastError();
}

template <bool POINTS>
static hipError_t launch_cull_t(int mode, const PlanConst* pc, int vdwk, int ewk, const Output& out,
                                const Points& pts, int64_t ntiles, int tj, int tk, hipStream_t stream)
{
    if (ntiles <= 0) return hipSuccess;
    switch (mode) {
    case MODE_VDW: return launch_cull_flags<MODE_VDW, POINTS>(vdwk, ewk, stream, pc, out, pts, tj, tk, ntiles);
    case MODE_COULOMB: return launch_cull_flags<MODE_COULOMB, POINTS>(vdwk, ewk, stream, pc, out, pts, tj, tk, ntiles);
    default: return launch_cull_flags<MODE_FUSED, POINTS>(vdwk, ewk, stream, pc, out, pts, tj, tk, ntiles);
    }
}

template <int MODE, int NP>
static hipError_t launch_multi_t(const PlanConst* pc, const Output& out, int tj, int tk, int64_t ntiles, hipStream_t stream)
{
    const int nw = culled_nw(MODE, 1, 2, NP);
    const int64_t nblocks = (ntiles + nw - 1) / nw;
    if (nblocks > 0x7fffffffLL) return hipErrorInvalidValue;
    hipLaunchKernelGGL((k_culled<MODE, false, 1, 2, NP>), dim3((unsigned)nblocks), dim3(64 * nw), 0, stream, pc, out, Points{nullptr, 0}, tj, tk, ntiles);
    return hipGetLastError();
}

hipError_t launch_culled_multi(int mode, int np, const PlanConst* d_pc, const Geom& g, const Output& out, hipStream_t stream)
{
    const int ni = out.i_end - out.i_begin;
    const int ti = (ni + 3) / 4, tj = (g.dims[1] + 1 + 3) / 4, tk = (g.dims[2] + 1 + 3) / 4;
    const int64_t ntiles = (int64_t)ti * tj * tk;
    if (ntiles <= 0) return hipSuccess;
    if (mode == MODE_FUSED) {
        static_assert(CEG_MAX_PROBES_FUSED == 2, "fused multi-probe variants");
        if (np == 2) return launch_multi_t<MODE_FUSED, 2>(d_pc, out, tj, tk, ntiles, stream);
        return hipErrorInvalidValue;
    }
    if (mode != MODE_VDW) return hipErrorInvalidValue;
    switch (np) {
    case 2: return launch_multi_t<MODE_VDW, 2>(d_pc, out, tj, tk, ntiles, stream);
    case 3: return launch_multi_t<MODE_VDW, 3>(d_pc, out, tj, tk, ntiles, stream);
    case 4: return launch_multi_t<MODE_VDW, 4>(d_pc, out, tj, tk, ntiles, stream);
    default: return hipErrorInvalidValue;
    }
}

hipError_t launch_culled(int mode, const PlanConst* d_pc, const Geom& g, int vdwk, int ewk,
                         const Output& out, const Points& pts, hipStream_t stream)
{
    if (pts.xyz) return launch_cull_t<true>(mode, d_pc, vdwk, ewk, out, pts, (pts.n + 63) / 64, 1, 1, stream);
    const int ni = out.i_end - out.i_begin;
    const int ti = (ni + 3) / 4, tj = (g.dims[1] + 1 + 3) / 4, tk = (g.dims[2] + 1 + 3) / 4;
    return launch_cull_t<false>(mode, d_pc, vdwk, ewk, out, pts, (int64_t)ti * tj * tk, tj, tk, stream);
}

}
```

### include/ceg_hip.h

```cpp
#ifndef CEG_HIP_H
#define CEG_HIP_H

#include <stdint.h>

#ifdef __cplusplus
extern "C" {
#endif

#define CEG_ABI_VERSION 1

#if defined(__GNUC__)
#define CEG_API __attribute__((visibility("default")))
#else
#define CEG_API
#endif

#define CEG_OK                 0
#define CEG_ERR_INVALID       -1
#define CEG_ERR_NO_DEVICE     -2
#define CEG_ERR_HIP           -3
#define CEG_ERR_RULE          -4
#define CEG_ERR_UNSUPPORTED   -5

enum ceg_kind {
    CEG_HARDSPHERE            = 0,
    CEG_COULOMB_EWALD_DIRECT  = 1,
    CEG_COULOMB               = 2,
    CEG_LENNARDJONES          = 3,
    CEG_BUCKINGHAM            = 4,
    CEG_MONOMIAL              = 5,
    CEG_EXPONENTIAL           = 6,
    CEG_UNDEFINED_INTERACTION = 7,
    CEG_NOINTERACTION         = 8
};

typedef struct ceg_rule {
    int32_t kind;
    int32_t _pad;
    double  p[3];
    double  shift;
} ceg_rule_t;

enum ceg_algo {
    CEG_ALGO_AUTO       = 0,
    CEG_ALGO_BRUTEFORCE = 1,
    CEG_ALGO_CULLED     = 2
};

CEG_API int         ceg_abi_version(void);
CEG_API int         ceg_device_count(void);
CEG_API const char* ceg_last_error(void);

CEG_API int ceg_grid_vdw(const double* pos, const int64_t* atomkind, int64_t natoms,
                 const double mat[9], const double invmat[9],
                 int32_t ortho, double safemin2, double cutoff2,
                 const ceg_rule_t* rules, const int32_t* rule_offset, int32_t nkinds,
                 const int32_t dims[3], const double size[3], const double shift[3],
                 const double delta[3],
                 double lambda, double threshold,
                 float* grid, int32_t ngpus);

CEG_API int ceg_grid_coulomb(const double* pos, const double* charge, int64_t natoms,
                     const double mat[9], const double invmat[9],
                     int32_t ortho, double safemin2, double cutoff2, double alpha,
                     const int32_t dims[3], const double size[3], const double shift[3],
                     const double delta[3],
                     double lambda, double threshold,
                     float* grid, int32_t ngpus);

CEG_API int ceg_grid_vdw_file(const double* pos, const int64_t* atomkind, int64_t natoms,
                 const double mat[9], const double invmat[9],
                 int32_t ortho, double safemin2, double cutoff2,
                 const ceg_rule_t* rules, const int32_t* rule_offset, int32_t nkinds,
                 const int32_t dims[3], const double size[3], const double shift[3],
                 const double delta[3], double lambda, double threshold,
                 float* grid, int32_t ngpus,
                 const char* path, const void* header, int64_t header_bytes,
                 const void* trailer, int64_t trailer_bytes);
CEG_API int ceg_grid_coulomb_file(const double* pos, const double* charge, int64_t natoms,
                     const double mat[9], const double invmat[9],
                     int32_t ortho, double safemin2, double cutoff2, double alpha,
                     const int32_t dims[3], const double size[3], const double shift[3],
                     const double delta[3], double lambda, double threshold,
                     float* grid, int32_t ngpus,
                     const char* path, const void* header, int64_t header_bytes,
                     const void* trailer, int64_t trailer_bytes);

CEG_API float* ceg_host_grid_alloc(const int32_t dims[3]);
CEG_API int    ceg_host_grid_free(float* grid);

CEG_API int ceg_release_cached_buffers(void);

CEG_API int ceg_grid_vdw_device(const double* pos, const int64_t* atomkind, int64_t natoms,
                                const double mat[9], const double invmat[9], int32_t ortho, double safemin2, double cutoff2,
                                const ceg_rule_t* rules, const int32_t* rule_offset, int32_t nkinds,
                                const int32_t dims[3], const double size[3], const double shift[3], const double delta[3],
                                double lambda, double threshold, float* d_grid, int32_t target_device, int32_t ngpus);
CEG_API int ceg_grid_coulomb_device(const double* pos, const double* charge, int64_t natoms,
                                    const double mat[9], const double invmat[9], int32_t ortho, double safemin2, double cutoff2,
                                    double alpha,
                                    const int32_t dims[3], const double size[3], const double shift[3], const double delta[3],
                                    double lambda, double threshold, float* d_grid, int32_t target_device, int32_t ngpus);

typedef struct ceg_plan ceg_plan_t;

CEG_API int ceg_plan_create(ceg_plan_t** plan, int32_t device,
                    const double* pos, const int64_t* atomkind, const double* charge,
                    int64_t natoms,
                    const double mat[9], const double invmat[9],
                    int32_t ortho, double safemin2, double cutoff2,
                    const ceg_rule_t* rules, const int32_t* rule_offset, int32_t nkinds,
                    double alpha,
                    const int32_t dims[3], const double size[3], const double shift[3],
                    const double delta[3]);
CEG_API int ceg_plan_destroy(ceg_plan_t* plan);
CEG_API int ceg_image_cache_stats(int64_t* hits, int64_t* misses, int64_t* entries);

CEG_API int ceg_plan_can_cull(const ceg_plan_t* plan);

CEG_API int64_t ceg_plan_num_images(const ceg_plan_t* plan);
CEG_API int ceg_plan_copy_images(const ceg_plan_t* plan, double* xyzq, int32_t* kind, int32_t* atom, int32_t* bin_start, int32_t nb[3]);

CEG_API int ceg_plan_build_vdw(ceg_plan_t* plan, double lambda, double threshold,
                       int32_t i_begin, int32_t i_end,
                       float* d_out, int64_t channel_stride, int32_t i_origin,
                       int32_t algo, void* stream);
CEG_API int ceg_plan_build_coulomb(ceg_plan_t* plan, double lambda, double threshold,
                           int32_t i_begin, int32_t i_end,
                           float* d_out, int64_t channel_stride, int32_t i_origin,
                           int32_t algo, void* stream);
CEG_API int ceg_plan_build_fused(ceg_plan_t* plan,
                         double lambda_vdw, double threshold_vdw,
                         double lambda_coulomb, double threshold_coulomb,
                         int32_t i_begin, int32_t i_end,
                         float* d_out_vdw, float* d_out_coulomb,
                         int64_t channel_stride, int32_t i_origin,
                         int32_t algo, void* stream);

#define CEG_MAX_PROBES 4
CEG_API int ceg_plan_create_multi(ceg_plan_t** plan, int32_t device,
                          const double* pos, const int64_t* atomkind, const double* charge, int64_t natoms,
                          const double mat[9], const double invmat[9],
                          int32_t ortho, double safemin2, double cutoff2,
                          int32_t nprobes, const ceg_rule_t* const* rules, const int32_t* const* rule_offset, int32_t nkinds,
                          double alpha,
                          const int32_t dims[3], const double size[3], const double shift[3], const double delta[3]);
CEG_API int ceg_plan_num_probes(const ceg_plan_t* plan);
CEG_API int ceg_grids_multi(const double* pos, const int64_t* atomkind, const double* charge, int64_t natoms,
                    const double mat[9], const double invmat[9], int32_t ortho, double safemin2, double cutoff2,
                    int32_t nprobes, const ceg_rule_t* const* rules, const int32_t* const* rule_offset, int32_t nkinds, double alpha,
                    const int32_t dims[3], const double size[3], const double shift[3], const double delta[3],
                    double lambda_vdw, double threshold_vdw, double lambda_coulomb, double threshold_coulomb,
                    float* const* grids_vdw, float* grid_coulomb, int32_t ngpus);
CEG_API int ceg_plan_build_multi(ceg_plan_t* plan,
                         double lambda_vdw, double threshold_vdw,
                         double lambda_coulomb, double threshold_coulomb,
                         int32_t i_begin, int32_t i_end,
                         float* const* d_out_vdw, float* d_out_coulomb,
                         int64_t channel_stride, int32_t i_origin, void* stream);

CEG_API int ceg_plan_eval_points(ceg_plan_t* plan, int32_t which, int32_t algo,
                         const double* points, int64_t npoints, double* out);

typedef struct ceg_interp ceg_interp_t;

typedef struct ceg_grid_header {
    double  spacing;
    int32_t dims[3];
    int32_t has_mat;
    double  size[3], shift[3], delta[3], unitcell[3];
    int32_t num_unitcell[3];
    int32_t _pad;
    double  ewald_precision;
    double  mat[9];
} ceg_grid_header_t;

CEG_API int ceg_interp_create(ceg_interp_t** handle, int32_t device,
                              const float* grid, int32_t grid_on_device,
                              const int32_t dims[3], const double size[3], const double shift[3],
                              const double mat[9], const double invmat[9], int32_t is_vdw);
CEG_API int ceg_interp_create_from_file(ceg_interp_t** handle, int32_t device, const char* path, int32_t iscoulomb, double scale,
                                const double* mat, const double* invmat, ceg_grid_header_t* header_out);
CEG_API int ceg_interp_set_higherorder(ceg_interp_t* handle, int32_t higherorder);
CEG_API int ceg_interp_destroy(ceg_interp_t* handle);
CEG_API int ceg_interp_points(ceg_interp_t* handle, const double* points, int64_t npoints, double* out);
CEG_API int ceg_interp_points_device(ceg_interp_t* handle, const double* d_points, int64_t npoints,
                                     double* d_out, void* stream);
CEG_API int ceg_scale_grid_device(float* d_grid, int64_t nfloats, double scale, int32_t device, void* stream);

typedef struct ceg_recip ceg_recip_t;

CEG_API int ceg_recip_create(ceg_recip_t** handle, int32_t device, const int32_t* kvec_ijk,
                             const double* kfactors, const double* sf_re, const double* sf_im, int64_t nk,
                             const int32_t ks[3], const double invmat[9]);
CEG_API int ceg_recip_destroy(ceg_recip_t* handle);
CEG_API int ceg_recip_layout(const int32_t* kvec_ijk, int64_t nk, const int32_t ks[3], int32_t* nrounds, int32_t* nslots,
                             int64_t* slot_of, int32_t* desc);
CEG_API int ceg_recip_energy(ceg_recip_t* handle, const double* positions, const double* charges,
                             int32_t natoms, int64_t n, double energy_net_charges,
                             double static_contribution, double* out);
CEG_API int ceg_recip_energy_device(ceg_recip_t* handle, const double* d_positions, const double* charges,
                                    int32_t natoms, int64_t n, double energy_net_charges,
                                    double static_contribution, double* d_out, void* stream);

CEG_API int ceg_recip_set_structure_factor(ceg_recip_t* handle, const double* sf_re, const double* sf_im);

CEG_API int ceg_energy_grid(ceg_interp_t* const* vdw_grids, ceg_interp_t* coulomb_grid, ceg_recip_t* recip,
                            const double* base, const double* charges, int32_t natoms,
                            const double* rotations, int32_t nrot, const double steps[9], const int32_t num[3],
                            const uint8_t* block, const int32_t block_dims[3], const double block_size[3], const double block_shift[3],
                            const double block_mat[9], const double block_invmat[9],
                            double energy_net_charges, double static_contribution,
                            double* out, int32_t out_on_device, void* stream);

#define CEG_EGRID_MAX_TEMPS 8
CEG_API int ceg_energy_grid_reduced(ceg_interp_t* const* vdw_grids, ceg_interp_t* coulomb_grid, ceg_recip_t* recip,
                                    const double* base, const double* charges, int32_t natoms,
                                    const double* rotations, int32_t nrot, const double steps[9], const int32_t num[3],
                                    const uint8_t* block, const int32_t block_dims[3], const double block_size[3], const double block_shift[3],
                                    const double block_mat[9], const double block_invmat[9],
                                    double energy_net_charges, double static_contribution,
                                    const double* temperatures, int32_t ntemps, const double* weights,
                                    double* out_mean, double* out_min, int32_t* out_argmin,
                                    int32_t out_on_device, void* stream);

typedef struct ceg_pairs ceg_pairs_t;

CEG_API int ceg_pairs_create(ceg_pairs_t** handle, int32_t device, const double mat[9], const double invmat[9],
                             double cutoff2, const ceg_rule_t* rules, const int32_t* rule_offset,
                             int32_t nkinds, double coulombic);
CEG_API int ceg_pairs_destroy(ceg_pairs_t* handle);
CEG_API int ceg_pairs_set_atoms(ceg_pairs_t* handle, const double* positions, const int32_t* kinds,
                                const int32_t* molecule, int64_t natoms);
CEG_API int ceg_pairs_energy(ceg_pairs_t* handle, const double* trial, const int32_t* trial_kinds, int32_t m,
                             int64_t n, int32_t exclude_molecule, double* out);
CEG_API int ceg_pairs_energy_device(ceg_pairs_t* handle, const double* d_trial, const int32_t* trial_kinds,
                                    int32_t m, int64_t n, int32_t exclude_molecule, double* d_out, void* stream);
CEG_API int ceg_pairs_neighbour_cells(ceg_pairs_t* handle, int32_t nb[3]);

typedef struct ceg_mc ceg_mc_t;

CEG_API int ceg_mc_create(ceg_mc_t** handle, int32_t device, ceg_interp_t* const* vdw_grids, ceg_interp_t* coulomb_grid,
                          const double* kind_charge, int32_t nkinds, const double mat[9], const double invmat[9],
                          double cutoff2, const ceg_rule_t* rules, const int32_t* rule_offset, double coulombic,
                          const int32_t* kvec_ijk, const double* kfactors, const double* sf_re, const double* sf_im,
                          int64_t nk, const int32_t ks[3], const double ewald_invmat[9]);
CEG_API int ceg_mc_destroy(ceg_mc_t* handle);
CEG_API int ceg_mc_set_guests(ceg_mc_t* handle, const double* positions, const int32_t* kinds,
                              const int32_t* mol_first, int32_t nmol);
CEG_API int ceg_mc_trial(ceg_mc_t* handle, int32_t molecule, const double* trial, int64_t n, double* out);
CEG_API int ceg_mc_trial_device(ceg_mc_t* handle, int32_t molecule, const double* d_trial, int64_t n, double* d_out, void* stream);
CEG_API int ceg_mc_trial_insert_device(ceg_mc_t* handle, const int32_t* kinds, int32_t m, const double* d_trial, int64_t n, double* d_out, void* stream);
CEG_API int ceg_mc_accept(ceg_mc_t* handle, int32_t molecule, const double* positions);
CEG_API int ceg_mc_trial_insert(ceg_mc_t* handle, const int32_t* kinds, int32_t m, const double* trial, int64_t n, double* out);
CEG_API int ceg_mc_insert(ceg_mc_t* handle, const int32_t* kinds, int32_t m, const double* positions, int32_t* molecule_out);
CEG_API int ceg_mc_remove(ceg_mc_t* handle, int32_t molecule, int32_t* moved_out);
CEG_API int ceg_mc_get_state(ceg_mc_t* handle, double* positions, double* sf_total_re, double* sf_total_im);
CEG_API int ceg_mc_neighbour_cells(ceg_mc_t* handle, int32_t nb[3], int32_t* capacity);
#define CEG_MC_GROUP_MAX 256
typedef struct ceg_mc_group ceg_mc_group_t;

CEG_API int ceg_mc_group_create(ceg_mc_group_t** group, ceg_mc_t* const* chains, int32_t k);
CEG_API int ceg_mc_group_destroy(ceg_mc_group_t* group);
CEG_API int ceg_mc_group_trial(ceg_mc_group_t* group, const int32_t* molecule, const int32_t* n,
                               const int32_t* insert_kinds, int32_t insert_m, const double* trial, double* out);
CEG_API int ceg_mc_group_accept(ceg_mc_group_t* group, const int32_t* molecule, const double* positions);

typedef struct ceg_mc_sweep_params {
    uint64_t seed, first_step;
    const uint32_t* stream_id;
    const double *temperature, *dmax, *thetamax, *p_rotation;
    const int32_t* bead;
} ceg_mc_sweep_params_t;
typedef struct ceg_mc_sweep_stats {
    int64_t translation_trials, translation_accepted, rotation_trials, rotation_accepted, blocked;
    double delta;
} ceg_mc_sweep_stats_t;
typedef struct ceg_mc_sweep_record {
    int32_t molecule, kind, accepted, _pad;
    double u;
    double rows[2][4];
    double positions[16][3];
} ceg_mc_sweep_record_t;

CEG_API int ceg_mc_group_sweep(ceg_mc_group_t* group, const ceg_mc_sweep_params_t* params, int64_t nsteps,
                               ceg_mc_sweep_stats_t* stats_out, ceg_mc_sweep_record_t* log_out);

#define CEG_MC_GCMC_MAX_SPECIES 8
typedef struct ceg_mc_gcmc_species {
    int32_t m, bead;
    int32_t kinds[16];
    double model[16][3];
    double cumulative[5];
    double phiPV_div_k, self_reciprocal, tail_framework;
    double tail_cross[CEG_MC_GCMC_MAX_SPECIES];
} ceg_mc_gcmc_species_t;
typedef struct ceg_mc_gcmc_params {
    uint64_t seed, first_step;
    const uint32_t* stream_id;
    const double *temperature, *dmax, *thetamax;
    int32_t nspecies, _pad;
    const ceg_mc_gcmc_species_t* species;
    const int32_t* molecule_species;
    const int32_t* max_molecules;
    int32_t* molecule_species_out;
} ceg_mc_gcmc_params_t;
typedef struct ceg_mc_gcmc_stats {
    int64_t trials[7], accepted[7];
    int64_t blocked, capacity, spent;
    double delta_moves, delta_swaps;
    int32_t count[CEG_MC_GCMC_MAX_SPECIES];
    int32_t nmol, _pad;
} ceg_mc_gcmc_stats_t;
typedef struct ceg_mc_gcmc_record {
    int32_t species, molecule, kind, accepted;
    int32_t n_species, flags;
    double u, tc;
    double rows[2][4];
    double positions[16][3];
} ceg_mc_gcmc_record_t;

CEG_API int ceg_mc_group_sweep_gcmc(ceg_mc_group_t* group, const ceg_mc_gcmc_params_t* params, int64_t nsteps,
                                    ceg_mc_gcmc_stats_t* stats_out, ceg_mc_gcmc_record_t* log_out);

CEG_API int ceg_block_from_grid(int32_t device, const float* value, int32_t value_on_device,
                                const int32_t dims[3], double threshold, uint8_t* block);
CEG_API int ceg_block_spheres(int32_t device, const int32_t dims[3], const double delta[3], const double shift[3],
                              const double mat[9], const double invmat[9], int32_t ortho, double safemin2,
                              const double* centers, const double* radius2, int32_t nspheres, uint8_t* block);

#ifdef __cplusplus
}
#endif
#endif
```

Baseline: 1.254 billion grid-points/s.

## Specialize culled kernel for frameworks with uniform LJ parameters and charges

At plan creation the host checks whether every framework atom that interacts by van der Waals shares one Lennard-Jones parameter set, and whether those atoms also share one charge. If so, the culled kernel runs a new variant. That variant drops per-pair parameter loads and the square root, works with unit-scaled polynomial terms, and counts pairs so the shift correction is applied once. Epsilon, sigma and charge factors are multiplied in at the end. This saves per-pair register traffic and arithmetic, at the cost of more template instantiations, an environment cap for the feature, and an extra code path whose rescaling must match the general one.

```diff
diff --git a/crystalenergygrids.jl_amd/ceg_hip/_abi.py b/crystalenergygrids.jl_amd/ceg_hip/_abi.py
--- a/crystalenergygrids.jl_amd/ceg_hip/_abi.py
+++ b/crystalenergygrids.jl_amd/ceg_hip/_abi.py
@@ -107,6 +107,8 @@
     "ceg_plan_destroy": (C.c_int, [C.c_void_p]),
     "ceg_image_cache_stats": (C.c_int, [c_int64_p, c_int64_p, c_int64_p]),
     "ceg_plan_can_cull": (C.c_int, [C.c_void_p]),
+    "ceg_plan_uniform_class": (C.c_int, [C.c_void_p]),
+    "ceg_uniform_class": (C.c_int, [c_int64_p, c_double_p, C.c_int64, C.c_void_p, c_int32_p, C.c_int32, C.c_double, c_double_p]),
     "ceg_plan_num_images": (C.c_int64, [C.c_void_p]),
     "ceg_plan_copy_images": (C.c_int, [C.c_void_p, c_double_p, c_int32_p, c_int32_p, c_int32_p, c_int32_p]),
     "ceg_plan_build_vdw": (C.c_int, [
diff --git a/crystalenergygrids.jl_amd/ceg_hip/plan.py b/crystalenergygrids.jl_amd/ceg_hip/plan.py
--- a/crystalenergygrids.jl_amd/ceg_hip/plan.py
+++ b/crystalenergygrids.jl_amd/ceg_hip/plan.py
@@ -31,6 +31,10 @@
         lc, tc = coulomb_scaling()
         _abi.check(self._lib, self._lib.ceg_plan_build_fused(self._h, lv, tv, lc, tc, i_begin, i_end, d_vdw,
                                                              d_coulomb, channel_stride, i_origin, algo, stream))
+
+    @property
+    def uniform_class(self) -> int:
+        return int(self._lib.ceg_plan_uniform_class(self._h))
 
     def eval_points(self, which: str, points, algo: int = _abi.ALGO_AUTO) -> np.ndarray:
         pts = np.ascontiguousarray(points, dtype=np.float64).reshape(-1, 3)
diff --git a/crystalenergygrids.jl_amd/csrc/ceg_api.hip b/crystalenergygrids.jl_amd/csrc/ceg_api.hip
--- a/crystalenergygrids.jl_amd/csrc/ceg_api.hip
+++ b/crystalenergygrids.jl_amd/csrc/ceg_api.hip
@@ -48,6 +48,39 @@
         return 0;
     }
     return n;
+}
+
+namespace ceg {
+UniformClass detect_uniform_class(const FastVdw* fast, int32_t nkinds, const int32_t* kind, const double* charge, int64_t natoms)
+{
+    UniformClass u;
+    std::vector<char> present((size_t)std::max(nkinds, 1), 0);
+    for (int64_t a = 0; a < natoms; ++a)
+        if (kind[a] >= 0 && kind[a] < nkinds) present[kind[a]] = 1;
+    const FastVdw* first = nullptr;
+    for (int32_t k = 0; k < nkinds; ++k) {
+        const FastVdw& f = fast[k];
+        if (!present[k] || f.cls == 0) continue;
+        if (f.cls != 1) return u;
+        if (!first) first = &f;
+        else if (memcmp(&first->p0, &f.p0, 4 * sizeof(double)) != 0) return u;
+    }
+    if (!first) return u;
+    const double e4 = first->p0, s6 = first->p2, sh = first->shift;
+    if (!(std::fabs(e4) >= 1e-9 && std::fabs(e4) <= 1e9) || !(s6 >= 1e-9 && s6 <= 1e9) || !std::isfinite(sh)) return u;
+    u.cls = 1; u.eps4 = e4; u.s6 = s6; u.shift = sh;
+    if (!charge) return u;
+    bool have = false;
+    double q = 0.0;
+    for (int64_t a = 0; a < natoms; ++a) {
+        const int32_t k = kind[a];
+        if (k < 0 || k >= nkinds || fast[k].cls == 0) continue;
+        if (!have) { q = charge[a]; have = true; }
+        else if (memcmp(&q, &charge[a], sizeof(double)) != 0) return u;
+    }
+    if (have && std::fabs(q) >= 1e-6 && std::fabs(q) <= 1e6) { u.cls = 2; u.q = q; }
+    return u;
+}
 }
 
 struct ceg_plan {
@@ -81,6 +114,7 @@
     bool single_buck = false;
     double bk[4] = {0, 0, 0, 0};
     double* d_bk2 = nullptr;
+    UniformClass uni;
     double r_exact2 = CEG_R_EXACT2;
     std::vector<FastVdw> h_fast;
     FastVdw* d_fast = nullptr;
@@ -99,6 +133,7 @@
         bool single_buck = false;
         double bk[4] = {0, 0, 0, 0};
         double* d_bk2 = nullptr;
+        UniformClass uni;
         int32_t* d_imgkind = nullptr;
     };
     int nprobes = 0;
@@ -214,6 +249,26 @@
     p->r_exact2 = std::max(CEG_R_EXACT2, hs_max2 * (1.0 + 1e-9) + 1e-9);
     if (p->r_exact2 >= p->g.cutoff2) p->vdwk = 0, p->r_exact2 = CEG_R_EXACT2;
     return CEG_OK;
+}
+
+void set_uniform_class(ceg_plan* p)
+{
+    p->uni = UniformClass{};
+    if (p->vdwk != 1 || p->natoms <= 0) return;
+    p->uni = detect_uniform_class(p->h_fast.data(), p->nkinds, p->h_kind.data(), p->h_charge.empty() ? nullptr : p->h_charge.data(), p->natoms);
+}
+
+void fill_uniform_class(PlanConst& c, const UniformClass& u)
+{
+    c.uni_class = u.cls;
+    if (u.cls == 0) return;
+    const double unit = u.eps4 * u.s6;
+    c.uni_unit = unit; c.uni_s6 = u.s6; c.uni_shift = u.shift;
+    c.uni_k1 = 2.0 * u.s6; c.uni_k2 = 3.5 * u.s6; c.uni_k3 = 5.6 * u.s6;
+    c.uni_sv = 1.0 / unit; c.uni_s1 = -1.0 / (6.0 * unit); c.uni_s2 = 1.0 / (48.0 * unit); c.uni_s3 = -1.0 / (480.0 * unit);
+    if (u.cls == 2) {
+        c.uni_q = u.q; c.uni_inv_q = 1.0 / u.q; c.uni_qs2 = 1.0 / (3.0 * u.q); c.uni_qs3 = 1.0 / (15.0 * u.q);
+    }
 }
 
 struct BlockCache {
@@ -935,6 +990,8 @@
                 ceg_plan::ProbeTab& t = p->probes[q];
                 t.rules = p->h_rules; t.offset = p->h_offset; t.fast = p->h_fast;
                 t.vdwk = p->vdwk; t.single_buck = p->single_buck;
+                set_uniform_class(p);
+                t.uni = p->uni;
                 for (int c = 0; c < 4; ++c) t.bk[c] = p->bk[c];
                 r_exact2 = std::max(r_exact2, p->r_exact2);
                 for (int32_t k = 0; k < nkinds; ++k) any[k] |= (t.offset[k + 1] > t.offset[k]) ? 1 : 0;
@@ -950,6 +1007,15 @@
             p->h_offset_union.assign(nkinds + 1, 0);
             for (int32_t k = 0; k < nkinds; ++k) p->h_offset_union[k + 1] = p->h_offset_union[k] + any[k];
             p->h_offset = p->probes[0].offset;
+            p->uni = UniformClass{};
+        } else {
+            set_uniform_class(p);
+        }
+        if (const char* e = std::getenv("CEG_HIP_UNIFORM_CLASS")) {
+            const int cap = std::max(0, atoi(e));
+            auto limit = [cap](UniformClass& u) { if (u.cls > cap) u.cls = cap; if (u.cls == 0) u = UniformClass{}; };
+            limit(p->uni);
+            for (auto& t : p->probes) limit(t.uni);
         }
     }
     double w[3];
@@ -999,6 +1065,7 @@
         if (p->h_fast.empty()) p->h_fast.assign(1, FastVdw{});
         rc = upload(&p->d_fast, p->h_fast.data(), p->h_fast.size());
         hc.fastvdw = p->d_fast;
+        fill_uniform_class(hc, p->uni);
         p->fast_ewald = false;
         bool any_vdwk2 = p->vdwk == 2;
         for (const auto& t : p->probes) any_vdwk2 = any_vdwk2 || t.vdwk == 2;
@@ -1065,6 +1132,7 @@
                 PlanConst hq = hc;
                 hq.rt = hc.rtm[q];
                 hq.fastvdw = hc.fastm[q];
+                fill_uniform_class(hq, t.uni);
                 setup_bk2(t.vdwk, t.single_buck, t.bk, &t.d_bk2, hq);
                 if (!rc && p->nprobes > 1) {
                     std::vector<int32_t> has((size_t)p->nkinds);
@@ -1156,6 +1224,31 @@
 
 extern "C" int ceg_plan_can_cull(const ceg_plan_t* p) { return (p && p->can_cull) ? 1 : 0; }
 
+extern "C" int ceg_plan_uniform_class(const ceg_plan_t* p)
+{
+    if (!p) return 0;
+    return p->nprobes > 0 ? p->probes[0].uni.cls : p->uni.cls;
+}
+
+extern "C" int ceg_uniform_class(const int64_t* atomkind, const double* charge, int64_t natoms, const ceg_rule_t* rules,
+                                 const int32_t* rule_offset, int32_t nkinds, double cutoff2, double constants[4])
+{
+    if (!atomkind || natoms <= 0 || !rules || !rule_offset || nkinds <= 0) return fail(CEG_ERR_INVALID, "atom / rule tables missing");
+    ceg_plan tmp;
+    tmp.natoms = natoms;
+    tmp.g.cutoff2 = cutoff2;
+    tmp.h_kind.resize((size_t)natoms);
+    for (int64_t a = 0; a < natoms; ++a) {
+        if (atomkind[a] < 1 || atomkind[a] > nkinds) return fail(CEG_ERR_INVALID, "atomkind[%lld] outside 1..%d", (long long)a, nkinds);
+        tmp.h_kind[a] = (int32_t)(atomkind[a] - 1);
+    }
+    if (charge) tmp.h_charge.assign(charge, charge + natoms);
+    if (int rc = convert_rules(&tmp, rules, rule_offset, nkinds)) return rc;
+    set_uniform_class(&tmp);
+    if (constants) { constants[0] = tmp.uni.eps4; constants[1] = tmp.uni.s6; constants[2] = tmp.uni.shift; constants[3] = tmp.uni.q; }
+    return tmp.uni.cls;
+}
+
 extern "C" int64_t ceg_plan_num_images(const ceg_plan_t* p) { return (p && p->images_built) ? p->ib.nimages : 0; }
 
 extern "C" int ceg_plan_copy_images(const ceg_plan_t* p, double* xyzq, int32_t* kind, int32_t* atom, int32_t* bin_start, int32_t nb[3])
@@ -1200,7 +1293,7 @@
     if (culled) {
         const bool probe0 = p->nprobes > 0 && mode != MODE_COULOMB;
         e = launch_culled(mode, probe0 ? p->probes[0].d_pc : p->d_pc, p->g, probe0 ? p->probes[0].vdwk : p->vdwk,
-                          p->ew2 ? 2 : (p->fast_ewald ? 1 : 0), out, pts, stream);
+                          p->ew2 ? 2 : (p->fast_ewald ? 1 : 0), out, pts, stream, probe0 ? p->probes[0].uni.cls : p->uni.cls);
     } else {
         AtomTable at{p->d_atoms, p->has_rules ? p->d_kind : nullptr, p->natoms};
         e = launch_bruteforce(mode, p->g, at, rt, out, pts, stream);
diff --git a/crystalenergygrids.jl_amd/csrc/ceg_internal.h b/crystalenergygrids.jl_amd/csrc/ceg_internal.h
--- a/crystalenergygrids.jl_amd/csrc/ceg_internal.h
+++ b/crystalenergygrids.jl_amd/csrc/ceg_internal.h
@@ -102,6 +102,12 @@
     double bk_B, bk_C, bk_invC;
     double bk_nshift, bk_c1, bk_c2, bk_c3, bk_c4;
     double bk_s1, bk_s2, bk_s3;
+    int32_t uni_class, _pad_uni;
+    double uni_unit, uni_s6, uni_shift, uni_q;
+    double uni_k1, uni_k2, uni_k3;
+    double uni_inv_q;
+    double uni_sv, uni_s1, uni_s2, uni_s3;
+    double uni_qs2, uni_qs3;
     int32_t all_simple;
     int32_t nprobes;
     RuleTable rtm[CEG_MAX_PROBES];
@@ -131,7 +137,13 @@
 hipError_t launch_bruteforce(int mode, const Geom& g, const AtomTable& atoms, const RuleTable& rt,
                              const Output& out, const Points& pts, hipStream_t stream);
 hipError_t launch_culled(int mode, const PlanConst* d_pc, const Geom& g, int vdwk, int ewk,
-                         const Output& out, const Points& pts, hipStream_t stream);
+                         const Output& out, const Points& pts, hipStream_t stream, int uni = 0);
+
+struct UniformClass {
+    int cls = 0;
+    double eps4 = 0, s6 = 0, shift = 0, q = 0;
+};
+UniformClass detect_uniform_class(const FastVdw* fast, int32_t nkinds, const int32_t* kind, const double* charge, int64_t natoms);
 constexpr int CEG_MAX_PROBES_FUSED = 2;
 hipError_t launch_culled_multi(int mode, int np, const PlanConst* d_pc, const Geom& g, const Output& out, hipStream_t stream);
 
diff --git a/crystalenergygrids.jl_amd/csrc/ceg_kernels.hip b/crystalenergygrids.jl_amd/csrc/ceg_kernels.hip
--- a/crystalenergygrids.jl_amd/csrc/ceg_kernels.hip
+++ b/crystalenergygrids.jl_amd/csrc/ceg_kernels.hip
@@ -310,8 +310,10 @@
 #ifndef CEG_NW_MULTI_FUSED
 #define CEG_NW_MULTI_FUSED 8
 #endif
-constexpr int culled_waves(int mode, int vdwk, int ewk, int np = 1)
-{
+constexpr bool vdwk_uniform(int vdwk) { return vdwk == 4 || vdwk == 5; }
+constexpr int culled_waves(int mode, int vdwk_, int ewk, int np = 1)
+{
+    const int vdwk = vdwk_uniform(vdwk_) ? 1 : vdwk_;
     return np > 1 ? (mode == 2 ? CEG_WAVES_MULTI_FUSED : (np == 2 ? CEG_WAVES_MULTI_VDW : 3))
            : (mode == 2 && vdwk >= 2 && ewk) ? CEG_WAVES_FUSED_BUCK
            : (mode == 2 && vdwk == 1 && ewk) ? CEG_WAVES_FUSED_LJ
@@ -344,7 +346,7 @@
     int32_t _pad[2];
 };
 
-template <int MODE, bool FASTEW, bool LJSLOW, bool EWSCALED, bool BKSCALED, int NP, bool DOV = true, bool DOC = true, typename Rec>
+template <int MODE, bool FASTEW, bool LJSLOW, bool EWSCALED, bool BKSCALED, int NP, int UNI = 0, bool DOV = true, bool DOC = true, typename Rec>
 __device__ __forceinline__ void slow_pairs(const PlanConst* __restrict__ pc, unsigned long long cands, int lane,
                                            double px, double py, double pz,
                                            const Rec* s_rec,
@@ -379,7 +381,9 @@
             const int kd = mt & META_KINDMASK;
             double v, p1, p2, p3;
             vdw_terms<LJSLOW, true>(pc->rt.rules, pc->rt.offset[kd], pc->rt.offset[kd + 1], r2, v, p1, p2, p3);
-            if (LJSLOW) {
+            if (UNI) {
+                v *= pc->uni_sv; p1 *= pc->uni_s1; p2 *= pc->uni_s2; p3 *= pc->uni_s3;
+            } else if (LJSLOW) {
                 p1 *= -1.0 / 6.0; p2 *= 1.0 / 48.0; p3 *= -1.0 / 480.0;
             }
             if (BKSCALED) {
@@ -397,7 +401,9 @@
                 ewald_terms_poly(g.alpha, O.w, r2, v, p1, p2, p3);
             else
                 ewald_terms(g.alpha, O.w, r2, v, p1, p2, p3);
-            if (EWSCALED) {
+            if (UNI == 2) {
+                v *= pc->uni_inv_q; p1 *= pc->uni_inv_q; p2 *= pc->uni_qs2; p3 *= pc->uni_qs3;
+            } else if (EWSCALED) {
                 p2 *= 1.0 / 3.0; p3 *= 1.0 / 15.0;
             }
             accum_add(ac, v, p1, p2, p3, dx, dy, dz);
@@ -467,6 +473,9 @@
     constexpr bool EW2 = EWK == 2 && MODE != MODE_VDW;
     constexpr int WG = 64 * culled_nw(MODE, VDWK, EWK, NP);
     constexpr bool BK2 = VDWK == 3 && MODE != MODE_COULOMB;
+    constexpr bool UNI = vdwk_uniform(VDWK) && MODE != MODE_COULOMB;
+    constexpr bool UNIQ = VDWK == 5 && MODE == MODE_FUSED && EWK == 2;
+    static_assert(!vdwk_uniform(VDWK) || (NP == 1 && MODE != MODE_COULOMB && (VDWK == 4 || UNIQ)), "uniform variants");
     constexpr int NW = WG / 64;
     constexpr bool HAS_LJ = !MULTI && (VDWK == 1 || VDWK == 2) && MODE != MODE_COULOMB;
     using Rec = std::conditional_t<MULTI, CandRecM<NP>, std::conditional_t<HAS_LJ, CandRec, CandRecS>>;
@@ -592,6 +601,11 @@
     const int bk2_off = BK2 ? __builtin_amdgcn_readfirstlane(-pc->bk2_base * (CEG_BK2_STRIDE * 8)) : 0;
     int bk2_stride = CEG_BK2_STRIDE * 8;
     asm volatile("" : "+v"(bk2_stride));
+    const double uni_s6 = UNI ? uniform(pc->uni_s6) : 0.0, uni_k1 = UNI ? uniform(pc->uni_k1) : 0.0;
+    const double uni_k2 = UNI ? uniform(pc->uni_k2) : 0.0, uni_k3 = UNI ? uniform(pc->uni_k3) : 0.0;
+    const double uni_inv_q = UNIQ ? uniform(pc->uni_inv_q) : 0.0;
+    int uni_count = 0;
+    int uni_count_all = 0;
     const double bk_B = pc->bk_B, bk_nshift = pc->bk_nshift, bk_c1 = pc->bk_c1, bk_c2 = pc->bk_c2, bk_c3 = pc->bk_c3, bk_c4 = pc->bk_c4;
 
     for (int rbase = 0; rbase < nrows; rbase += 64) {
@@ -668,7 +682,7 @@
                                 LJM[p] = make_double4(F.p0, F.p1, F.p2, F.shift);
                             }
                         }
-                    } else if (FASTVDW && VDWK != 3 && hasvdw && keep) {
+                    } else if (FASTVDW && VDWK != 3 && !UNI && hasvdw && keep) {
                         const FastVdw F = pc->fastvdw[kd];
                         LJ = make_double4(F.p0, F.p1, F.p2, F.shift);
                         vclass = F.cls;
@@ -708,7 +722,7 @@
                 const unsigned long long mine = !simple_c ? mask_x : (withv ? (interior ? mask_vi : mask_vb) : (interior ? mask_ni : mask_nb));
                 const int first = !simple_c ? nreg : (withv ? (interior ? 0 : nvi) : (interior ? nv : nni));
                 const int slot = first + __builtin_amdgcn_mbcnt_hi((unsigned)(mine >> 32), __builtin_amdgcn_mbcnt_lo((unsigned)mine, 0));
-                s_rec[slot].xyzq = Quad{P.x, P.y, P.z, P.w};
+                s_rec[slot].xyzq = Quad{P.x, P.y, P.z, (UNIQ && !withv) ? mul_sc(P.w, uni_inv_q) : P.w};
                 if constexpr (MULTI) {
 #pragma unroll
                     for (int p = 0; p < NP; ++p) set_lj_record(s_rec[slot], p, Quad{LJM[p].x, LJM[p].y, LJM[p].z, LJM[p].w});
@@ -739,7 +753,7 @@
                 const double dxy = dx * dy, dxz = dx * dz, dyz = dy * dz;
                 const double dxyz = dxz * dy;
                 double rr = 0.0, rinv = 0.0, inv = 0.0;
-                constexpr bool NEED_SQRT = (VDWK >= 2 && MODE != MODE_COULOMB) || (EWK == 1 && MODE != MODE_VDW);
+                constexpr bool NEED_SQRT = ((VDWK == 2 || VDWK == 3) && MODE != MODE_COULOMB) || (EWK == 1 && MODE != MODE_VDW);
                 if (NEED_SQRT) {
                     fast_sqrt_rsqrt(r2, rr, rinv);
                     inv = rinv * rinv;
@@ -779,7 +793,16 @@
                     }
                 } else if constexpr (WITH_VDW) {
                     double v, p1, p2, p3;
-                    if constexpr (VDWK == 3) {
+                    if constexpr (UNI) {
+                        const double inv2 = inv * inv;
+                        const double z = inv2 * inv;
+                        const double a = z * z;
+                        v = fms_vsv(a, uni_s6, z);
+                        p1 = fms_vsv(a, uni_k1, z) * inv;
+                        p2 = fms_vsv(a, uni_k2, z) * inv2;
+                        p3 = fms_vsv(a, uni_k3, z) * (inv2 * inv2);
+                        if constexpr (!INTERIOR) ++uni_count;
+                    } else if constexpr (VDWK == 3) {
                         const double2* rec = reinterpret_cast<const double2*>(
                             reinterpret_cast<const char*>(s_bk2) + mad_u24(key, bk2_stride, bk2_off));
                         const double2 g01 = rec[0], g23 = rec[1], g45 = rec[2], g67 = rec[3];
@@ -865,7 +888,7 @@
                         cc = __builtin_fma(cc, t, c12.x);
                         b0 = __builtin_fma(b0, t, a01.x);
                         cc = __builtin_fma(cc, t, a6c0.y);
-                        const double qb0 = A.w * b0, qc = A.w * cc;
+                        const double qb0 = (UNIQ && WITH_VDW) ? b0 : A.w * b0, qc = (UNIQ && WITH_VDW) ? cc : A.w * cc;
                         const double b1 = (qb0 + qc) * inv;
                         const double b2 = fma_vsv(qc, ew_k3, b1) * inv;
                         const double b3 = fma_vsv(qc, ew_k15, b2) * inv;
@@ -902,6 +925,7 @@
 #endif
             if (MODE != MODE_COULOMB) {
                 for (int q = 0; q < nvi; ++q) pair_body(q, std::true_type{}, std::true_type{});
+                if (UNI) uni_count_all += nvi;
                 for (int q = nvi; q < nv; ++q) pair_body(q, std::true_type{}, std::false_type{});
             }
             if (MODE != MODE_VDW) {
@@ -924,10 +948,10 @@
             if (slow != 0ull) {
                 __builtin_amdgcn_wave_barrier();
                 if constexpr (MULTI && MODE == MODE_FUSED) {
-                    slow_pairs<MODE, FASTEW, true, EW2, false, NP, true, false>(pc, slow, lane, px, py, pz, s_rec, s_odd, avm, out.probe_idx, ac, smallest_d2);
-                    slow_pairs<MODE, FASTEW, true, EW2, false, NP, false, true>(pc, slow, lane, px, py, pz, s_rec, s_odd, avm, out.probe_idx, ac, smallest_d2);
+                    slow_pairs<MODE, FASTEW, true, EW2, false, NP, 0, true, false>(pc, slow, lane, px, py, pz, s_rec, s_odd, avm, out.probe_idx, ac, smallest_d2);
+                    slow_pairs<MODE, FASTEW, true, EW2, false, NP, 0, false, true>(pc, slow, lane, px, py, pz, s_rec, s_odd, avm, out.probe_idx, ac, smallest_d2);
                 } else
-                    slow_pairs<MODE, FASTEW, VDWK == 1, EW2, VDWK == 3 && MODE != MODE_COULOMB, NP>(pc, slow, lane, px, py, pz, s_rec, s_odd, avm, out.probe_idx, ac, smallest_d2);
+                    slow_pairs<MODE, FASTEW, VDWK == 1 || UNI, EW2, VDWK == 3 && MODE != MODE_COULOMB, NP, UNIQ ? 2 : (UNI ? 1 : 0)>(pc, slow, lane, px, py, pz, s_rec, s_odd, avm, out.probe_idx, ac, smallest_d2);
             }
         }
     }
@@ -939,6 +963,17 @@
             a.d2xy *= 48.0; a.d2xz *= 48.0; a.d2yz *= 48.0;
             a.d3 *= -480.0;
         }
+    }
+    if (UNI) {
+        const double e4 = pc->uni_unit;
+        av.v = __builtin_fma(av.v, e4, -((double)(uni_count + uni_count_all) * pc->uni_shift));
+        av.d1x *= -6.0 * e4; av.d1y *= -6.0 * e4; av.d1z *= -6.0 * e4;
+        av.d2xy *= 48.0 * e4; av.d2xz *= 48.0 * e4; av.d2yz *= 48.0 * e4;
+        av.d3 *= -480.0 * e4;
+    }
+    if (UNIQ) {
+        const double q = pc->uni_q;
+        ac.v *= q; ac.d1x *= q; ac.d1y *= q; ac.d1z *= q; ac.d2xy *= q; ac.d2xz *= q; ac.d2yz *= q; ac.d3 *= q;
     }
     if (VDWK == 3 && MODE != MODE_COULOMB) {
         const double C = pc->bk_C;
@@ -1073,22 +1108,29 @@
 }
 
 template <int MODE, bool POINTS>
-static hipError_t launch_cull_flags(int vdwk, int ewk, hipStream_t stream, const PlanConst* pc, const Output& out, const Points& pts,
+static hipError_t launch_cull_flags(int vdwk, int ewk, int uni, hipStream_t stream, const PlanConst* pc, const Output& out, const Points& pts,
                                     int tj, int tk, int64_t ntiles)
 {
     if (MODE == MODE_VDW) ewk = 1;
     if (MODE == MODE_COULOMB) vdwk = 1;
     if (ewk == 2 && vdwk == 0) ewk = 1;
     if (vdwk == 3 && MODE == MODE_FUSED && ewk != 2) vdwk = 2;
+    if (vdwk == 1 && uni > 0 && MODE == MODE_VDW) vdwk = 4;
+    if (vdwk == 1 && uni > 0 && MODE == MODE_FUSED && ewk == 2) vdwk = uni == 2 ? 5 : 4;
     const int nw = culled_nw(MODE, vdwk, ewk);
     const int64_t nblocks = (ntiles + nw - 1) / nw;
     if (nblocks > 0x7fffffffLL) return hipErrorInvalidValue;
     const dim3 grid((unsigned)nblocks), block(64 * nw);
 #define CEG_LAUNCH(V, F) hipLaunchKernelGGL((k_culled<MODE, POINTS, V, F>), grid, block, 0, stream, pc, out, pts, tj, tk, ntiles)
     if (ewk == 2 && MODE != MODE_VDW) {
-        if (vdwk == 1) CEG_LAUNCH(1, 2); else if (vdwk == 3) CEG_LAUNCH(3, 2); else CEG_LAUNCH(2, 2);
+        if (vdwk == 1) CEG_LAUNCH(1, 2); else if (vdwk == 3) CEG_LAUNCH(3, 2);
+        else if (vdwk == 4) { if constexpr (MODE == MODE_FUSED) CEG_LAUNCH(4, 2); }
+        else if (vdwk == 5) { if constexpr (MODE == MODE_FUSED) CEG_LAUNCH(5, 2); }
+        else CEG_LAUNCH(2, 2);
     } else if (ewk) {
-        if (vdwk == 1) CEG_LAUNCH(1, 1); else if (vdwk == 2) CEG_LAUNCH(2, 1); else if (vdwk == 3) CEG_LAUNCH(3, 1); else CEG_LAUNCH(0, 1);
+        if (vdwk == 1) CEG_LAUNCH(1, 1); else if (vdwk == 2) CEG_LAUNCH(2, 1); else if (vdwk == 3) CEG_LAUNCH(3, 1);
+        else if (vdwk == 4) { if constexpr (MODE == MODE_VDW) CEG_LAUNCH(4, 1); }
+        else CEG_LAUNCH(0, 1);
     } else {
         if (vdwk == 1) CEG_LAUNCH(1, 0); else if (vdwk == 2) CEG_LAUNCH(2, 0); else if (vdwk == 3) CEG_LAUNCH(2, 0); else CEG_LAUNCH(0, 0);
     }
@@ -1097,14 +1139,14 @@
 }
 
 template <bool POINTS>
-static hipError_t launch_cull_t(int mode, const PlanConst* pc, int vdwk, int ewk, const Output& out,
+static hipError_t launch_cull_t(int mode, const PlanConst* pc, int vdwk, int ewk, int uni, const Output& out,
                                 const Points& pts, int64_t ntiles, int tj, int tk, hipStream_t stream)
 {
     if (ntiles <= 0) return hipSuccess;
     switch (mode) {
-    case MODE_VDW: return launch_cull_flags<MODE_VDW, POINTS>(vdwk, ewk, stream, pc, out, pts, tj, tk, ntiles);
-    case MODE_COULOMB: return launch_cull_flags<MODE_COULOMB, POINTS>(vdwk, ewk, stream, pc, out, pts, tj, tk, ntiles);
-    default: return launch_cull_flags<MODE_FUSED, POINTS>(vdwk, ewk, stream, pc, out, pts, tj, tk, ntiles);
+    case MODE_VDW: return launch_cull_flags<MODE_VDW, POINTS>(vdwk, ewk, uni, stream, pc, out, pts, tj, tk, ntiles);
+    case MODE_COULOMB: return launch_cull_flags<MODE_COULOMB, POINTS>(vdwk, ewk, uni, stream, pc, out, pts, tj, tk, ntiles);
+    default: return launch_cull_flags<MODE_FUSED, POINTS>(vdwk, ewk, uni, stream, pc, out, pts, tj, tk, ntiles);
     }
 }
 
@@ -1139,12 +1181,12 @@
 }
 
 hipError_t launch_culled(int mode, const PlanConst* d_pc, const Geom& g, int vdwk, int ewk,
-                         const Output& out, const Points& pts, hipStream_t stream)
-{
-    if (pts.xyz) return launch_cull_t<true>(mode, d_pc, vdwk, ewk, out, pts, (pts.n + 63) / 64, 1, 1, stream);
+                         const Output& out, const Points& pts, hipStream_t stream, int uni)
+{
+    if (pts.xyz) return launch_cull_t<true>(mode, d_pc, vdwk, ewk, uni, out, pts, (pts.n + 63) / 64, 1, 1, stream);
     const int ni = out.i_end - out.i_begin;
     const int ti = (ni + 3) / 4, tj = (g.dims[1] + 1 + 3) / 4, tk = (g.dims[2] + 1 + 3) / 4;
-    return launch_cull_t<false>(mode, d_pc, vdwk, ewk, out, pts, (int64_t)ti * tj * tk, tj, tk, stream);
-}
-
-}
+    return launch_cull_t<false>(mode, d_pc, vdwk, ewk, uni, out, pts, (int64_t)ti * tj * tk, tj, tk, stream);
+}
+
+}
diff --git a/include/ceg_hip.h b/include/ceg_hip.h
--- a/include/ceg_hip.h
+++ b/include/ceg_hip.h
@@ -117,6 +117,10 @@
 CEG_API int ceg_image_cache_stats(int64_t* hits, int64_t* misses, int64_t* entries);
 
 CEG_API int ceg_plan_can_cull(const ceg_plan_t* plan);
+
+CEG_API int ceg_plan_uniform_class(const ceg_plan_t* plan);
+CEG_API int ceg_uniform_class(const int64_t* atomkind, const double* charge, int64_t natoms, const ceg_rule_t* rules,
+                              const int32_t* rule_offset, int32_t nkinds, double cutoff2, double constants[4]);
 
 CEG_API int64_t ceg_plan_num_images(const ceg_plan_t* plan);
 CEG_API int ceg_plan_copy_images(const ceg_plan_t* plan, double* xyzq, int32_t* kind, int32_t* atom, int32_t* bin_start, int32_t nb[3]);
```

Result: faster. 1.307 billion grid-points/s, median of 6 (+4.3%).
